# o1-labs/proof-systems

Hardware: AMD Instinct MI355X
Metric: MSM Mscalar/s at 2^20 (Vesta) (higher is better)
Workload: dtype u29x9 / u32x8 (255-bit Montgomery integers); 1 GPU; msm_2^20_vesta_srs; points_per_gpu=1048576, points_total=1048576, bases=SRS::<Vesta>::create, scalars=uniform 254-bit, seed 1234+rank, parallelism=point-range x1, world_size_seen=1

## Files before the change

### include/kimchi_hip.h

```cpp
#ifndef KIMCHI_HIP_H
#define KIMCHI_HIP_H

#include <stddef.h>
#include <stdint.h>

#ifdef __cplusplus
extern "C" {
#endif

#define KH_OK 0
#define KH_E_INVALID (-1)
#define KH_E_DEVICE (-2)
#define KH_E_NOTFOUND (-3)
#define KH_E_NOMEM (-4)

#define KH_CURVE_VESTA 0
#define KH_CURVE_PALLAS 1
#define KH_FIELD_FP 0
#define KH_FIELD_FQ 1
#define KH_BASIS_G (-1)

typedef struct kh_srs kh_srs_t;
typedef struct kh_sponge kh_sponge_t;

int kh_device_count(void);
int kh_init(int device_id);
int kh_set_device(int device_id);
int kh_get_device(void);
int kh_private_context_begin(void);
int kh_private_context_end(void);
int kh_private_context_active(void);
int kh_set_phase_timers(int on);
int kh_trim(void);
const char *kh_last_error(void);

int kh_srs_create(int curve, const uint64_t *g_xy , size_t n, kh_srs_t **out);
int kh_msm_set_wide_min_n(size_t n);
int kh_msm_set_sort_staging(unsigned entries, unsigned max_passes);
int kh_srs_set_wide_tables(kh_srs_t *srs, int on);
int kh_srs_has_wide_tables(const kh_srs_t *srs);
void kh_srs_free(kh_srs_t *srs);
size_t kh_srs_size(const kh_srs_t *srs);
int kh_srs_curve(const kh_srs_t *srs);
int kh_srs_device(const kh_srs_t *srs);

int kh_srs_generate(int curve, size_t start, size_t count, uint64_t *out_xy, int threads);
int kh_srs_h(int curve, uint64_t out_xy[8]);
int kh_group_map_to_group(int curve, const uint64_t t[4], uint64_t out_xy[8]);

int kh_srs_create_device(int curve, size_t depth, kh_srs_t **out);
int kh_srs_create_device_range(int curve, size_t start, size_t count, kh_srs_t **out);
int kh_srs_get_g(kh_srs_t *srs, size_t offset, size_t count, uint64_t *out_xy);

int kh_srs_set_lagrange(kh_srs_t *srs, unsigned log2_domain, unsigned chunk,
                        const uint64_t *xy, const uint8_t *inf, size_t n);
int kh_srs_compute_lagrange(kh_srs_t *srs, unsigned log2_domain);
int kh_srs_get_lagrange(kh_srs_t *srs, unsigned log2_domain, unsigned chunk,
                        uint64_t *out_xy, uint8_t *out_inf);
int kh_srs_lagrange_chunks(const kh_srs_t *srs, unsigned log2_domain);

int kh_msm(kh_srs_t *srs, int basis, unsigned chunk, size_t offset,
           const uint64_t *scalars, size_t n, int scalars_are_montgomery,
           uint64_t out_xy[8], uint8_t *out_is_inf);

int kh_msm_batch(kh_srs_t *srs, int basis, unsigned chunk, size_t offset,
                 const uint64_t *scalars, size_t n, size_t k, int scalars_are_montgomery,
                 uint64_t *out_xy , uint8_t *out_is_inf );

int kh_msm_points(int curve, const uint64_t *xy , const uint8_t *inf ,
                  const uint64_t *scalars, size_t n, int scalars_are_montgomery,
                  uint64_t out_xy[8], uint8_t *out_is_inf);

int kh_msm_points_batch(int curve, const uint64_t *xy, const uint8_t *inf, const uint64_t *scalars,
                        size_t n, size_t k, int scalars_are_montgomery,
                        uint64_t *out_xy , uint8_t *out_is_inf );

int kh_points_sum(int curve, const uint64_t *xy, const uint8_t *inf, size_t n, uint64_t out_xy[8], uint8_t *out_is_inf);
int kh_points_add(int curve, const uint64_t *a_xy, const uint8_t *a_inf, const uint64_t *b_xy, const uint8_t *b_inf, size_t n,
                  uint64_t *out_xy , uint8_t *out_is_inf );

int kh_msm_sharded(kh_srs_t *const *shards, size_t R, const uint64_t *scalars, size_t n, int scalars_are_montgomery,
                   uint64_t out_xy[8], uint8_t *out_is_inf);
int kh_msm_sharded_dev(kh_srs_t *const *shards, size_t R, const uint64_t *const *scalars_dev, const size_t *counts,
                       int scalars_are_montgomery, uint64_t out_xy[8], uint8_t *out_is_inf);

int kh_ipa_fold_scalars(int field, const uint64_t *lo, const uint64_t *hi, const uint64_t u[4], size_t n, uint64_t *out);
int kh_inner_product(int field, const uint64_t *a, const uint64_t *b, size_t n, uint64_t out[4]);
int kh_ipa_fold_points(int curve, const uint64_t *g_lo_xy, const uint64_t *g_hi_xy, const uint64_t u[4], size_t n,
                       uint64_t *out_xy, uint8_t *out_inf);
int kh_ipa_fold_points_endo(int curve, const uint64_t *g_lo_xy, const uint64_t *g_hi_xy, const uint64_t chal[2], size_t n,
                            uint64_t *out_xy, uint8_t *out_inf);
int kh_endos(int curve, uint64_t endo_q[4], uint64_t endo_r[4]);
int kh_scalar_challenge_to_field(int curve, const uint64_t chal[2], uint64_t out[4]);
// ... 450 lines not shown
```

### proof_systems_amd/csrc/api_internal.hpp

```cpp
#pragma once
#include <atomic>
#include <map>
#include <memory>

#include "common.hpp"
#include "host_ec.hpp"
#include "msm.hpp"

namespace kh {
struct LagrangeChunk { DevBuf pts; DevBuf inf; bool has_inf = false; size_t n = 0; int precomp_c = 0; };
}

namespace kh {
struct IpaWorkspace {
    int index = 0;
    bool live = false;
    std::thread::id owner;
    DevBuf a[2], b[2], coef[2], sc, partial, sg;
    hipEvent_t ev = nullptr;
    DevBuf rb_tab, rb_B, rb_part, rb_lists, rb_scratch;
    hipStream_t rb_stream = nullptr;
    hipEvent_t rb_go = nullptr, rb_snap = nullptr, rb_done = nullptr;
    uint32_t* rb_fail = nullptr;
    ~IpaWorkspace() {
        if (ev) (void)hipEventDestroy(ev);
        if (rb_go) (void)hipEventDestroy(rb_go);
        if (rb_snap) (void)hipEventDestroy(rb_snap);
        if (rb_done) (void)hipEventDestroy(rb_done);
        if (rb_stream) { (void)hipStreamSynchronize(rb_stream); (void)hipStreamDestroy(rb_stream); }
        if (rb_fail) (void)hipHostFree(rb_fail);
    }
};
}

struct kh_srs {
    int curve = 0;
    int device = -1;
    size_t n = 0;
    kh::DevBuf g;
    size_t g_stride = 0;
    int g_precomp_c = 0;
    kh::DevBuf g_wide; int g_wide_c = 0;
    std::shared_ptr<std::atomic<int>> jobs = std::make_shared<std::atomic<int>>(0);
    std::mutex wide_mu;
    std::unique_ptr<kh::IpaWorkspace> ipa_ws[KH_IPA_OPENINGS];
    uint64_t h[8];
    std::vector<khost::xyzz> h_table;
    std::vector<uint64_t> h_multiples;
    bool h_in_tables = false;
    std::mutex h_mu;
    std::mutex map_mu;
    std::mutex ipa_mu; std::condition_variable ipa_cv;
    std::map<unsigned, std::vector<std::unique_ptr<kh::LagrangeChunk>>> lagrange;
};
#define KH_ON_DEVICE_OF(srs) kh::DeviceScope dev_scope_((srs) ? (srs)->device : -1)

namespace kh {
int resolve_basis(kh_srs_t* srs, int basis, unsigned chunk, MsmBasis& out);
void xyzz_to_affine_batch(const khost::Crv& crv, const std::vector<khost::xyzz>& acc, uint64_t* out_xy, uint8_t* out_inf);
hipStream_t thread_copy_stream();
hipEvent_t thread_upload_event();
int acquire_slot(std::unique_lock<std::mutex>* lk, Context& C, bool side_first = false);
const char* slot_error(int si);
int wait_then_finish(std::unique_lock<std::mutex>& lk, Context& C, MsmSlot& S, uint64_t* out_xy, uint8_t* out_inf);
double last_wait_us();
void xfer_trim(int d);
struct PoolBlock {
    void* p = nullptr;
    ~PoolBlock() { if (p) (void)kh_dev_free(p); }
    template <class T> T* as() const { return (T*)p; }
};
struct WitnessPlace {
    const uint32_t* rows;
    size_t row0, row_stride;
    uint64_t* witness;
    size_t col_stride;
    __host__ __device__ size_t start_row(size_t i) const { return rows ? (size_t)rows[i] : row0 + i * row_stride; }
    __host__ __device__ size_t offset(size_t r, size_t c) const { return 4 * (c * col_stride + r); }
    __host__ __device__ uint64_t* cell(size_t r, size_t c) const { return witness + offset(r, c); }
};
static constexpr int WAVE_BLOCK = 64;
static constexpr size_t WAVE_BLOCK_MAX_N = (size_t)1 << 36;
inline dim3 blocks_of(size_t n, size_t per) { return dim3((unsigned)((n + per - 1) / per)); }
int poseidon_permute(Context& C, int field, uint64_t* states_dev, size_t n);
int poseidon_hash(Context& C, int field, const uint64_t* msgs_dev, size_t msg_len, size_t n, const uint64_t* init, uint64_t* digests_dev);
int poseidon_gate_rows(Context& C, int field, const uint64_t* states_dev, size_t n, const WitnessPlace& at, uint64_t* out_states_dev);
void poseidon_set_split_max_n(size_t n);
int complete_add_rows(Context& C, int field, const uint64_t* p1_dev, const uint64_t* p2_dev, size_t n, const WitnessPlace& at, uint64_t* out_dev);
int endomul_scalar_rows(Context& C, int field, const uint64_t* chals_dev, unsigned num_bits, size_t n, const WitnessPlace& at, const uint64_t* endo_scalar,
                        uint64_t* out_dev);
size_t chain_slice(bool is_endo, unsigned num_bits, size_t n);
size_t chain_scratch_bytes(bool is_endo, unsigned num_bits, size_t n);
int chain_rows(Context& C, int field, bool is_endo, const uint64_t* endo, const uint64_t* base_dev, const uint64_t* acc0_dev, const uint64_t* scalars_dev,
               unsigned num_bits, size_t n, const WitnessPlace& at, uint64_t* out_acc_dev, uint64_t* out_n_dev, uint32_t* flags_dev, unsigned bit,
// ... 100 lines not shown
```

### proof_systems_amd/csrc/common.hpp

```cpp
#pragma once
#include <hip/hip_runtime.h>
#include <stdarg.h>
#include <stdint.h>
#include <stdio.h>
#include <atomic>
#include <chrono>
#include <condition_variable>
#include <initializer_list>
#include <map>
#include <memory>
#include <mutex>
#include <set>
#include <string>
#include <thread>
#include <vector>

#include "../../include/kimchi_hip.h"
#include "msm_plan.hpp"

namespace kh {

void set_error(const char* fmt, ...);

#define KH_HIP(expr)                                                                         \
// ... 17 lines not shown
    void* p = nullptr;
    size_t cap = 0;
    DevBuf() = default;
    DevBuf(const DevBuf&) = delete;
    DevBuf& operator=(const DevBuf&) = delete;
    DevBuf(DevBuf&& o) noexcept : p(o.p), cap(o.cap) { o.p = nullptr; o.cap = 0; }
    DevBuf& operator=(DevBuf&& o) noexcept { if (this != &o) { release(); p = o.p; cap = o.cap; o.p = nullptr; o.cap = 0; } return *this; }
    ~DevBuf() { release(); }
    int reserve(size_t bytes) {
        if (bytes <= cap) return KH_OK;
        if (p) { hipError_t e = hipFree(p); (void)e; p = nullptr; cap = 0; }
        size_t want = bytes + bytes / 8;
        hipError_t e = hipMalloc(&p, want);
        if (e != hipSuccess) { set_error("hipMalloc(%zu) failed: %s", want, hipGetErrorString(e)); p = nullptr; return KH_E_NOMEM; }
        cap = want;
        return KH_OK;
    }
    void release() { if (p) { hipError_t e = hipFree(p); (void)e; } p = nullptr; cap = 0; }
    template <class T> T* as() const { return (T*)p; }
};

struct PhaseTimer {
    static constexpr int MAXP = 24;
    hipEvent_t k0 = nullptr, k1 = nullptr;
    const char* kname = nullptr;
    hipEvent_t ev[MAXP + 1];
    const char* names[MAXP];
    int n = 0;
    bool created = false;
    bool enabled = false;
    int init() {
        if (created) return KH_OK;
        for (int i = 0; i <= MAXP; i++) KH_HIP(hipEventCreate(&ev[i]));
        KH_HIP(hipEventCreate(&k0)); KH_HIP(hipEventCreate(&k1));
        created = true;
        return KH_OK;
    }
    void begin(hipStream_t s) { n = 0; kname = nullptr; if (enabled && created) (void)hipEventRecord(ev[0], s); }
    void mark(const char* name, hipStream_t s) {
        if (!enabled || !created || n >= MAXP) return;
        names[n] = name; n++;
        (void)hipEventRecord(ev[n], s);
    }
};

struct MsmBasis {
    const void* pts = nullptr;
    const uint8_t* inf = nullptr;
    size_t n = 0;
    int precomp_c = 0;
    size_t stride = 0;
    size_t batch_stride = 0;
    const void* wide_pts = nullptr;
    int wide_c = 0;
    bool glv = false;
};

struct MsmJob {
    MsmBasis basis;
    size_t offset = 0;
    const uint64_t* scalars = nullptr;
    size_t n = 0, k = 0;
    int mont = 0, curve = 0;
    MsmPlan plan;
    bool done_by_flag = false;
    bool spread_rerun = false;
};

struct MsmSlot {
    hipStream_t stream = nullptr;
    PhaseTimer timer;
    DevBuf ws_scalars, ws_digits, ws_hist, ws_cnt, ws_off, ws_ntask, ws_toff, ws_entries, ws_partial,
        ws_buckets, ws_seg, ws_out, ws_scan_tmp, ws_biglist, ws_points, ws_order, ws_chunks, ws_handed, ws_sync, ws_mid,
        ws_b29, ws_a1, ws_l2, ws_a2, ws_xlist;
    void* pinned = nullptr; size_t pinned_cap = 0;
    hipEvent_t done = nullptr;
    bool busy = false;
    std::thread::id owner;
    uint64_t ticket = 0;
    MsmJob job;
    std::shared_ptr<std::atomic<int>> handle_jobs;
    volatile uint32_t* host_abort = nullptr;
    volatile uint32_t* spread_abort = nullptr;
    bool flag_unavailable = false;
    bool pinned_coherent = false;
    volatile uint32_t* done_flag = nullptr;
    DevBuf ws_done;
    uint32_t done_expect = 0;
};
static constexpr int MSM_SLOTS = 4;

struct Context {
    std::mutex mu;
    std::condition_variable cv;
    int sync_inflight = 0;
    std::multiset<std::thread::id> blocked_owners;
    int device = -1;
    bool ready = false;
    hipStream_t stream = nullptr;
    bool main_dirty = false;
    hipEvent_t order_ev = nullptr;
    int num_cus = 256;
    size_t lds_per_cu = (size_t)160 << 10, lds_per_block = (size_t)64 << 10;
    bool fused_disabled = false;
    PhaseTimer timer;
    std::vector<std::pair<const char*, float>> last;
    MsmSlot slot[MSM_SLOTS];
// ... 45 lines not shown
```

### proof_systems_amd/csrc/msm.hip

```cpp
#include <hip/hip_ext.h>
#include <math.h>
#include "common.hpp"
#include "env.hpp"
#include "block_sum.cuh"
#include "coop.cuh"
#include "field29.cuh"
#include "host_ec.hpp"
#include "msm.hpp"
#include "msm_plan.hpp"
#include <condition_variable>
#include <functional>
#include <memory>
#include <thread>

namespace kh {

#define KH_HIGH_PRIO() __builtin_amdgcn_s_setprio(3)

class HostHelper {
    std::thread th_; std::mutex m_; std::condition_variable cv_, done_cv_;
    std::function<void()> job_; bool has_job_ = false, busy_ = false, stop_ = false;
    void loop() {
        std::unique_lock<std::mutex> lk(m_);
        for (;;) {
// ... 231 lines not shown
    }
    __syncthreads();
    size_t q; int Sq, sigma; geom_ids(g, s, w, j, q, Sq, sigma);
    u32* out = H + (q * Sq + sigma) * g.nb;
    for (u32 b = threadIdx.x; b < g.nb; b += blockDim.x) out[b] = h[b];
}
__global__ void k_key_totals(u32* __restrict__ H, u32 nb, int Sq, size_t nkeys, u32* __restrict__ cnt) {
    KH_HIGH_PRIO();
    size_t key = (size_t)blockIdx.x * blockDim.x + threadIdx.x;
    if (key >= nkeys) { if (key == nkeys) cnt[key] = 0; return; }
    size_t q = key / nb; u32 b = (u32)(key % nb);
    u32* p = H + q * Sq * nb + b;
    u32 run = 0;
    for (int s = 0; s < Sq; s++) { u32 v = p[(size_t)s * nb]; p[(size_t)s * nb] = run; run += v; }
    cnt[key] = run;
}
__global__ void k_scatter(const int32_t* __restrict__ digits, SortGeom g, const u32* __restrict__ H,
                          const u32* __restrict__ off, u32* __restrict__ entries) {
    KH_HIGH_PRIO();
    extern __shared__ u32 pos[];
    int s = blockIdx.x, w = blockIdx.y, j = blockIdx.z;
    size_t q; int Sq, sigma; geom_ids(g, s, w, j, q, Sq, sigma);
    const u32* hin = H + (q * Sq + sigma) * g.nb;
    const u32* o = off + q * g.nb;
    for (u32 b = threadIdx.x; b < g.nb; b += blockDim.x) pos[b] = o[b] + hin[b];
    __syncthreads();
    size_t lo = g.n * (size_t)s / g.S, hi = g.n * (size_t)(s + 1) / g.S;
    const int32_t* d = digits + ((size_t)j * g.W + w) * g.n;
    u32 pbase = (u32)(g.pt_offset + (g.precomp ? (size_t)w * g.pt_stride : 0) + (size_t)j * g.pt_batch);
    for (size_t i = lo + threadIdx.x; i < hi; i += blockDim.x) {
        int32_t v = d[i];
        if (v) {
            u32 b = (u32)(v < 0 ? -v : v) - 1u;
            u32 slot = atomicAdd(&pos[b], 1u);
            entries[slot] = (pbase + (u32)i) | (v < 0 ? 0x80000000u : 0u);
        }
    }
}
__device__ __forceinline__ u32 lds_inc_agg(u32* ctr, u32 key, bool active) {
    const u64 act = __ballot(active);
    if (!act) return 0;
    const int leader = __ffsll((long long)act) - 1;
    const u32 k0 = __shfl(key, leader, 64);
    if (__ballot(active && key == k0) == act) {
        const int lane = (int)(threadIdx.x & 63u);
        u32 b = 0;
        if (lane == leader) b = atomicAdd(&ctr[k0], (u32)__popcll(act));
        b = __shfl(b, leader, 64);
        return b + (u32)__popcll(act & ((1ull << lane) - 1ull));
    }
    return active ? atomicAdd(&ctr[key], 1u) : 0u;
}
__global__ void __launch_bounds__(PART_T)
k_part_hist(const int32_t* __restrict__ digits, u32 tot_e, u32 nblk, u32 shift, u32* __restrict__ PH) {
    KH_HIGH_PRIO();
    __shared__ u32 cnt[PART_P];
    const u32 blk = blockIdx.x, j = blockIdx.y, tid = threadIdx.x;
    if (tid < PART_P) cnt[tid] = 0;
    __syncthreads();
    const u32 e_lo = (u32)((u64)tot_e * blk / nblk), e_hi = (u32)((u64)tot_e * (blk + 1) / nblk);
    const int32_t* d = digits + (size_t)j * tot_e;
    for (u32 e0 = e_lo + tid; e0 < e_hi; e0 += 8 * PART_T) {
        int32_t v[8];
#pragma unroll
        for (int u = 0; u < 8; u++) { const u32 e = e0 + u * PART_T; v[u] = d[e < e_hi ? e : e_hi - 1]; if (e >= e_hi) v[u] = 0; }
#pragma unroll
        for (int u = 0; u < 8; u++) (void)lds_inc_agg(cnt, (((u32)(v[u] < 0 ? -v[u] : v[u]) - 1u) >> shift) & (PART_P - 1u), v[u] != 0);
    }
    __syncthreads();
    if (tid < PART_P) PH[((size_t)j * PART_P + tid) * nblk + blk] = cnt[tid];
    if (blk == 0 && j == 0 && tid == 0) PH[(size_t)gridDim.y * PART_P * nblk] = 0;
}
__global__ void __launch_bounds__(PART_T)
k_part_scatter(const int32_t* __restrict__ digits, u32 tot_e, u32 n, u32 nblk, const u32* __restrict__ PO, u32* __restrict__ mid) {
    KH_HIGH_PRIO();
    __shared__ u32 cur[PART_P];
    const u32 blk = blockIdx.x, j = blockIdx.y, tid = threadIdx.x;
    if (tid < PART_P) cur[tid] = PO[((size_t)j * PART_P + tid) * nblk + blk];
    __syncthreads();
    const u32 e_lo = (u32)((u64)tot_e * blk / nblk), e_hi = (u32)((u64)tot_e * (blk + 1) / nblk);
    const int32_t* d = digits + (size_t)j * tot_e;
    u32 w = (e_lo + tid) / n, i = (e_lo + tid) - w * n;
    for (u32 e0 = e_lo + tid; e0 < e_hi; e0 += 8 * PART_T) {
        int32_t v[8];
#pragma unroll
        for (int u = 0; u < 8; u++) { const u32 e = e0 + u * PART_T; v[u] = d[e < e_hi ? e : e_hi - 1]; if (e >= e_hi) v[u] = 0; }
#pragma unroll
        for (int u = 0; u < 8; u++) {
            const u32 b = (u32)(v[u] < 0 ? -v[u] : v[u]) - 1u;
            const u32 pos = lds_inc_agg(cur, b >> PART_LOW, v[u] != 0);
            if (v[u]) mid[pos] = ((b & ((1u << PART_LOW) - 1u)) << 25) | (v[u] < 0 ? 1u << 24 : 0u) | (w << 20) | i;
            i += PART_T;
            while (i >= n) { i -= n; w++; }
        }
    }
}
__global__ void __launch_bounds__(PART_T)
k_part_sort(const u32* __restrict__ mid, const u32* __restrict__ PO, u32 nblk, u32 nb, size_t pt_stride, size_t pt_offset, size_t pt_batch,
            u32 last_group, u32* __restrict__ off, u32* __restrict__ entries) {
    KH_HIGH_PRIO();
    __shared__ u32 hist[1u << PART_LOW], cur[1u << PART_LOW];
    const u32 pidx = blockIdx.x, j = blockIdx.y, tid = threadIdx.x;
    const size_t q = (size_t)j * PART_P + pidx;
    const u32 base = PO[q * nblk], end = PO[(q + 1) * nblk];
    if (tid < (1u << PART_LOW)) hist[tid] = 0;
    __syncthreads();
    for (u32 x0 = base + tid; x0 < end; x0 += 8 * PART_T) {
        u32 m[8];
#pragma unroll
        for (int u = 0; u < 8; u++) { const u32 x = x0 + u * PART_T; m[u] = mid[x < end ? x : end - 1]; }
#pragma unroll
        for (int u = 0; u < 8; u++) (void)lds_inc_agg(hist, m[u] >> 25, x0 + u * PART_T < end);
    }
    __syncthreads();
    if (tid < 64) {
        const u32 a = hist[2 * tid], b = hist[2 * tid + 1];
        u32 inc = a + b;
#pragma unroll
        for (int d = 1; d < 64; d <<= 1) { const u32 o = __shfl_up(inc, d, 64); if (tid >= (u32)d) inc += o; }
        const u32 ex = base + inc - (a + b);
// ... 236 lines not shown
    KH_TS(5);
    if (!grid_barrier(sync, 3 * G, abort_dev, abort_host, spin_limit)) return;
    KH_TS(6);
    const u32* o = off + (size_t)j * g.nb + b_lo;
    {
        u32 a[FUSED_C], hh[FUSED_C];
#pragma unroll
        for (int u = 0; u < FUSED_C; u++) { const u32 b = tid + u * FUSED_T, bc = b < g.sub ? b : 0u; a[u] = coh_load(o + bc); hh[u] = coh_load(hout + bc); }
        u32 total2;
        lane_sums(bsums + FUSED_B, G, blk, &base, &total2);
#pragma unroll
        for (int u = 0; u < FUSED_C; u++) { const u32 b = tid + u * FUSED_T; if (b < g.sub) lds[b] = a[u] + hh[u]; }
    }
    run = base + ex2;
#pragma unroll
    for (int i = 0; i < FUSED_KPT; i++) {
        const u32 key = key0 + i;
        if ((u32)i < g.kpt && key <= g.nkeys) toff[key] = run;
        run += nt[i];
    }
    __syncthreads();
    KH_TS(7);
    const u32 pb0 = (u32)(g.pt_offset + (size_t)j * g.pt_batch);
    const u32 e_first = 4 * (q_lo + tid);
    u32 w = e_first / g.n, i = e_first - w * g.n;
#pragma unroll
    for (int t = 0; t < FUSED_V; t++) asm volatile("" : "+v"(dv[t][0]), "+v"(dv[t][1]));
#pragma unroll
    for (int t = 0; t < FUSED_V; t++) {
#pragma unroll
        for (int l = 0; l < 4; l++) {
            const u32 c = (dv[t][l >> 1] >> (16 * (l & 1))) & 0xffffu, b = (c & 0x7fffu) - b_lo;
            if (c != 0xffffu && b < g.sub) {
                u32 ii = i + l, ww = w;
                if (ii >= g.n) { ii -= g.n; ww++; }
                const u32 slot = atomicAdd(&lds[b], 1u);
                entries[slot] = (pb0 + (u32)(ww * g.pt_stride) + ii) | ((c & 0x8000u) << 16);
            }
        }
        i += 4 * FUSED_T;
        while (i >= g.n) { i -= g.n; w++; }
    }
    __syncthreads();
    KH_TS(8);
    if (tid == 0) {
        const u32 out = __hip_atomic_fetch_add(sync + 1, 1u, __ATOMIC_RELAXED, __HIP_MEMORY_SCOPE_AGENT);
        if (out == G - 1) {
            __hip_atomic_store(sync, 0u, __ATOMIC_RELAXED, __HIP_MEMORY_SCOPE_AGENT);
            __hip_atomic_store(sync + 1, 0u, __ATOMIC_RELAXED, __HIP_MEMORY_SCOPE_AGENT);
        }
    }
}
__global__ void __launch_bounds__(PART_T)
k_part2_scatter(const int32_t* __restrict__ digits, u32 tot_e, u32 nblk, u32 low, const u32* __restrict__ PO, u32* __restrict__ mid, u32* __restrict__ xlist, u32* __restrict__ big) {
    KH_HIGH_PRIO();
    __shared__ u32 cur[PART_P];
    const u32 blk = blockIdx.x, j = blockIdx.y, tid = threadIdx.x;
    if (blk == 0 && j == 0 && tid == 0) { xlist[0] = 0; xlist[1] = 0; big[0] = 0; }
    if (tid < PART_P) cur[tid] = PO[((size_t)j * PART_P + tid) * nblk + blk];
    __syncthreads();
    const u32 e_lo = (u32)((u64)tot_e * blk / nblk), e_hi = (u32)((u64)tot_e * (blk + 1) / nblk);
    const int32_t* d = digits + (size_t)j * tot_e;
    for (u32 e0 = e_lo + tid; e0 < e_hi; e0 += 8 * PART_T) {
        int32_t v[8];
#pragma unroll
        for (int u = 0; u < 8; u++) { const u32 e = e0 + u * PART_T; v[u] = d[e < e_hi ? e : e_hi - 1]; if (e >= e_hi) v[u] = 0; }
#pragma unroll
        for (int u = 0; u < 8; u++) {
            const u32 b = (u32)(v[u] < 0 ? -v[u] : v[u]) - 1u;
            const u32 pos = lds_inc_agg(cur, b & (PART_P - 1u), v[u] != 0);
            if (v[u]) mid[pos] = ((b >> 8) << 17) | (v[u] < 0 ? 1u << 16 : 0u) | (e0 + u * PART_T - e_lo);
        }
    }
}
__global__ void __launch_bounds__(PART_T)
k_part2_sort(const u32* __restrict__ mid, const u32* __restrict__ PO, u32 nblk, u32 low, u32 nb, u32 tot_e, u32 n, size_t pt_stride, size_t pt_offset,
             size_t pt_batch, u32 last_group, size_t total_idx, WideTasks ta, u32* __restrict__ off, u32* __restrict__ entries,
             u32* __restrict__ toff, u32* __restrict__ order, u32* __restrict__ ptot, u32* __restrict__ xlist, u32* __restrict__ slist,
             uint8_t* __restrict__ buckets29, u32 og, u32 stage_cap, u32 max_pass, u32* __restrict__ big, u32 bigcap, u32 hot_nt) {
    KH_HIGH_PRIO();
    __shared__ u32 cur[1u << PART2_MAXLOW], pstart[1025], bi0[1024], bw0[1024], lh[MAX_K + 2], sh[PART_T / 64 + 1];
    __shared__ u32 xl_n, pfirst[PART2_MAXPASS], plast[PART2_MAXPASS];
    extern __shared__ u32 stage[];
    u32* const xl_key = stage; u32* const xl_nt = stage + (1u << PART2_MAXLOW); u32* const xl_base = stage + (2u << PART2_MAXLOW);
    const u32 pidx = blockIdx.x, j = blockIdx.y, tid = threadIdx.x;
    const size_t q = (size_t)j * PART_P + pidx;
    const u32 nparts = gridDim.x * gridDim.y;
    const u32 nbl = 1u << low;
    for (u32 i = tid; i <= nblk; i += PART_T) pstart[i] = PO[q * nblk + i];
    for (u32 i = tid; i < nblk; i += PART_T) {
        const u32 est = (u32)((u64)tot_e * i / nblk), w0 = est / n;
        bw0[i] = w0; bi0[i] = est - w0 * n;
    }
    for (u32 i = tid; i < nbl; i += PART_T) cur[i] = 0;
    for (u32 i = tid; i < MAX_K + 2; i += PART_T) lh[i] = 0;
    if (tid == 0) xl_n = 0;
    __syncthreads();
    const u32 base = pstart[0], end = pstart[nblk];
    for (u32 x0 = base + tid; x0 < end; x0 += 8 * PART_T) {
        u32 m[8];
#pragma unroll
        for (int u = 0; u < 8; u++) { const u32 x = x0 + u * PART_T; m[u] = mid[x < end ? x : end - 1]; }
#pragma unroll
        for (int u = 0; u < 8; u++) (void)lds_inc_agg(cur, m[u] >> 17, x0 + u * PART_T < end);
    }
    __syncthreads();
    {
        const u32 i0 = 2 * tid, a = i0 < nbl ? cur[i0] : 0u, b = i0 + 1 < nbl ? cur[i0 + 1] : 0u;
        u32 btot;
        const u32 ex = base + block_scan_1024(a + b, sh, &btot);
        __syncthreads();
        const size_t key0 = (size_t)j * nb + (size_t)pidx * nbl + i0;
        if (i0 < nbl) { off[key0] = ex; cur[i0] = ex; }
        if (i0 + 1 < nbl) { off[key0 + 1] = ex + a; cur[i0 + 1] = ex + a; }
        if (tid == 0 && pidx == PART_P - 1 && j == last_group) off[(size_t)(j + 1) * nb] = end;
        const u32 K = pick_K(PO[total_idx], ta.room, ta.kmin, ta.ktab, ta.nkeys);
        const u32 nta = (a + K - 1) / K, ntb = (b + K - 1) / K;
        const u32 la = nta ? (a + nta - 1) / nta : 0u, lb = ntb ? (b + ntb - 1) / ntb : 0u;
        const u32 tex = block_scan_1024(nta + ntb, sh, &btot);
        if (i0 < nbl) toff[key0] = tex;
        if (i0 + 1 < nbl) toff[key0 + 1] = tex + nta;
        if (tid == 0) ptot[q] = btot;
        if (i0 < nbl) atomicAdd(&lh[la], 1u);
        if (i0 + 1 < nbl) atomicAdd(&lh[lb], 1u);
        if (nta > 1) { const u32 sl = atomicAdd(&xl_n, 1u); xl_key[sl] = (u32)key0; xl_nt[sl] = nta; xl_base[sl] = atomicAdd(&xlist[0], nta - 1u); slist[atomicAdd(&xlist[1], 1u)] = (u32)key0; }
        if (ntb > 1) { const u32 sl = atomicAdd(&xl_n, 1u); xl_key[sl] = (u32)key0 + 1u; xl_nt[sl] = ntb; xl_base[sl] = atomicAdd(&xlist[0], ntb - 1u); slist[atomicAdd(&xlist[1], 1u)] = (u32)key0 + 1u; }
        if (nta > hot_nt) { const u32 sl = atomicAdd(&big[0], 1u); big[2 + sl] = (u32)key0; big[2 + bigcap + sl] = 0u; }
        if (ntb > hot_nt) { const u32 sl = atomicAdd(&big[0], 1u); big[2 + sl] = (u32)key0 + 1u; big[2 + bigcap + sl] = 0u; }
        if (i0 < nbl && a == 0) { uint4* rec = (uint4*)(buckets29 + ((size_t)j * nb + ((size_t)i0 << 8 | pidx)) * B29_BYTES); _Pragma("unroll") for (int t = 0; t < 9; t++) rec[t] = make_uint4(0u, 0u, 0u, 0u); }
        if (i0 + 1 < nbl && b == 0) { uint4* rec = (uint4*)(buckets29 + ((size_t)j * nb + ((size_t)(i0 + 1) << 8 | pidx)) * B29_BYTES); _Pragma("unroll") for (int t = 0; t < 9; t++) rec[t] = make_uint4(0u, 0u, 0u, 0u); }
        __syncthreads();
        const u32 L = MAX_K - (tid <= MAX_K ? tid : MAX_K), hv = tid <= MAX_K ? lh[L] : 0u;
        const u32 above = block_scan_1024(hv, sh, &btot);
        __syncthreads();
        if (tid <= MAX_K) lh[L] = above;
        __syncthreads();
        if (i0 < nbl) { const u32 r = atomicAdd(&lh[la], 1u); order[(size_t)(r / og) * nparts * og + q * og + (r % og)] = (u32)key0; }
        if (i0 + 1 < nbl) { const u32 r = atomicAdd(&lh[lb], 1u); order[(size_t)(r / og) * nparts * og + q * og + (r % og)] = (u32)key0 + 1u; }
        const u32 nx = xl_n;
        for (u32 it = 0; it < nx; it++) {
            const u32 key = xl_key[it], ntx = xl_nt[it], xb = xl_base[it];
            for (u32 jt = 1 + tid; jt < ntx; jt += PART_T) { xlist[2 + 2 * (size_t)(xb + jt - 1)] = key; xlist[3 + 2 * (size_t)(xb + jt - 1)] = jt; }
        }
    }
    __syncthreads();
    const u32 pb0 = (u32)(pt_offset + (size_t)j * pt_batch);
    const u32 lane = tid & 63u, wv = tid >> 6;
    const u32 S_eff = stage_cap > 2048u ? stage_cap - 1024u : 0u;
    const u32 npass = S_eff ? (end - base + S_eff - 1u) / S_eff : 0u;
    const bool staged = S_eff != 0u && npass >= 1u && npass <= max_pass;
    uint8_t* const bpass = (uint8_t*)(stage + stage_cap);
    if (staged) {
        if (tid < PART2_MAXPASS) { pfirst[tid] = 0xffffffffu; plast[tid] = 0u; }
        __syncthreads();
        for (u32 b = tid; b < nbl; b += PART_T) {
            const u32 o = cur[b], oe = b + 1 < nbl ? cur[b + 1] : end, pb = (o - base) / S_eff;
            bpass[b] = (uint8_t)pb;
            if (oe > o) { atomicMin(&pfirst[pb], o); atomicMax(&plast[pb], oe); }
        }
        __syncthreads();
    }
    for (u32 pass = 0; pass < (staged ? npass : 1u); pass++) {
        const u32 p0 = staged ? pfirst[pass] : 0u, p1 = staged ? plast[pass] : 0u;
        if (staged && p0 == 0xffffffffu) continue;
        for (u32 blk = wv; blk < nblk; blk += PART_T / 64) {
            const u32 rs = pstart[blk], re = pstart[blk + 1];
            const u32 w0 = bw0[blk], i0 = bi0[blk];
            for (u32 x0 = rs; x0 < re; x0 += 256) {
                u32 m[4];
#pragma unroll
                for (int u = 0; u < 4; u++) { const u32 x = x0 + u * 64 + lane; m[u] = mid[x < re ? x : re - 1]; }
#pragma unroll
                for (int u = 0; u < 4; u++) {
                    if (x0 + u * 64 >= re) break;
                    const u32 bk = m[u] >> 17;
                    const bool live = x0 + u * 64 + lane < re && (!staged || bpass[bk] == pass);
                    const u32 pos = lds_inc_agg(cur, bk, live);
                    if (live) {
                        u32 w = w0, i = i0 + (m[u] & 0xffffu);
                        while (i >= n) { i -= n; w++; }
                        const u32 val = (pb0 + (u32)(w * pt_stride) + i) | ((m[u] & (1u << 16)) << 15);
                        if (staged && pos - p0 < stage_cap) stage[pos - p0] = val;
                        else entries[pos] = val;
                    }
                }
            }
        }
        if (staged) {
            __syncthreads();
            const u32 cnt = p1 - p0 < stage_cap ? p1 - p0 : stage_cap;
            for (u32 k = tid; k < cnt; k += PART_T) entries[p0 + k] = stage[k];
            __syncthreads();
        }
    }
}
__global__ void __launch_bounds__(256)
k_wide_fixup(u32* __restrict__ toff, const u32* __restrict__ ptot, u32 nparts, u32 low, u32 nkeys, u32* __restrict__ handed, u32* __restrict__ big) {
    KH_HIGH_PRIO();
    __shared__ u32 sh[4];
    const u32 key = blockIdx.x * 256 + threadIdx.x, q = (blockIdx.x * 256) >> low;
    u32 v = 0;
    for (u32 t = threadIdx.x; t < q && t < nparts; t += 256) v += ptot[t];
#pragma unroll
    for (int d = 32; d >= 1; d >>= 1) v += __shfl_xor(v, d, 64);
    if ((threadIdx.x & 63u) == 0) sh[threadIdx.x >> 6] = v;
    __syncthreads();
    const u32 bs = sh[0] + sh[1] + sh[2] + sh[3];
    if (key < nkeys) toff[key] += bs;
    else if (key == nkeys) toff[key] = bs;
    if (key == 0) handed[0] = 0;
}
template <class BF>
__global__ void __launch_bounds__(256) __attribute__((amdgpu_num_vgpr(112), amdgpu_waves_per_eu(4, 4)))
k_accumulate29(const u32* __restrict__ entries, const u32* __restrict__ off, const u32* __restrict__ toff,
               const u32* __restrict__ roff, const u32* __restrict__ order,
               size_t nkeys, const uint8_t* __restrict__ pts, uint8_t* __restrict__ partial, u32* __restrict__ handed, const u32* __restrict__ abort_dev, u32 hi_prio) {
    if (hi_prio) __builtin_amdgcn_s_setprio(2);
    if (sort_gave_up(abort_dev)) return;
    const size_t t0 = (size_t)blockIdx.x * blockDim.x + threadIdx.x;
    u32 NT = roff[nkeys];
    if (t0 >= NT) return;
    size_t lo = 0, hi = nkeys;
    while (hi - lo > 1) {
        size_t mid = (lo + hi) >> 1;
        if (roff[mid] <= (u32)t0) lo = mid; else hi = mid;
    }
    size_t key = order ? order[lo] : lo;
    u32 jt = (u32)t0 - roff[lo];
    const size_t t = (size_t)toff[key] + jt;
    u32 o0 = off[key], cnt = off[key + 1] - o0, nt = toff[key + 1] - toff[key];
    u32 start = o0 + (u32)(((u64)jt * cnt) / nt);
    u32 end = o0 + (u32)(((u64)(jt + 1) * cnt) / nt);
    u32 e = entries[start];
    Aff<BF> p = Aff<BF>::load(pts + (size_t)(e & 0x7fffffffu) * 64);
    if (e >> 31) p.y = neg<BF>(p.y);
    typedef typename C29<BF>::T K29;
    Acc29<BF> acc;
    bool ok = true;
    u32 k = start + 1;
    if (k < end) {
        const Fe29<BF> x1 = pack29<BF, 5>(p.x), y1 = pack29<BF, 5>(p.y);
        e = entries[k];
        p = Aff<BF>::load(pts + (size_t)(e & 0x7fffffffu) * 64);
        if (e >> 31) p.y = neg<BF>(p.y);
        ok = aadd29<BF>(acc, x1, y1, pack29<BF, 5>(p.x), pack29<BF, 5>(p.y));
        k = ok ? k + 1 : end;
    } else {
        acc.x = to29<BF>(p.x); acc.y = to29<BF>(p.y);
#pragma unroll
        for (int i = 0; i < 9; i++) { acc.zz.v[i] = K29::one(i); acc.zzz.v[i] = K29::one(i); }
    }
    for (; k < end; k++) {
        e = entries[k];
        p = Aff<BF>::load(pts + (size_t)(e & 0x7fffffffu) * 64);
        if (e >> 31) p.y = neg<BF>(p.y);
        ok = madd29<BF, false>(acc, pack29<BF, 5>(p.x), pack29<BF, 5>(p.y));
        if (!ok) break;
    }
    Xyzz<BF> r;
    if (__builtin_expect(!ok, 0)) {
        e = entries[start];
        p = Aff<BF>::load(pts + (size_t)(e & 0x7fffffffu) * 64);
        if (e >> 31) p.y = neg<BF>(p.y);
        r = Xyzz<BF>::from_affine(p);
        for (u32 k = start + 1; k < end; k++) {
            e = entries[k];
            p = Aff<BF>::load(pts + (size_t)(e & 0x7fffffffu) * 64);
            r = madd<BF>(r, p, (e >> 31) != 0);
        }
    } else {
        r.x = from29<BF>(acc.x); r.y = from29<BF>(acc.y); r.zz = from29<BF>(acc.zz); r.zzz = from29<BF>(acc.zzz);
    }
    r.store(partial + t * 128);
}
__device__ __forceinline__ u32 wide_true_bucket(u32 key, u32 low) {
    const u32 nbl = 1u << low, grp = key >> (low + 8), kk = key & ((nbl << 8) - 1u);
    return (grp << (low + 8)) | ((kk & (nbl - 1u)) << 8) | (kk >> low);
}
template <class BF>
__device__ __forceinline__ bool wide_task29(u32 key, u32 jt, const u32* __restrict__ entries, const u32* __restrict__ off, const u32* __restrict__ toff,
                                            const uint8_t* __restrict__ pts, uint8_t* __restrict__ partial, uint8_t* __restrict__ buckets29, u32 low, u32* __restrict__ handed) {
    const u32 o0 = off[key], cnt = off[key + 1] - o0;
    if (cnt == 0) return true;
    const u32 t0 = toff[key], nt = toff[key + 1] - t0;
    u32 start = o0, end = o0 + cnt;
    if (nt != 1) { start = o0 + (u32)(((u64)jt * cnt) / nt); end = o0 + (u32)(((u64)(jt + 1) * cnt) / nt); }
    u32 e = entries[start];
    Aff<BF> p = Aff<BF>::load(pts + (size_t)(e & 0x7fffffffu) * 64);
    if (e >> 31) p.y = neg<BF>(p.y);
    typedef typename C29<BF>::T K29;
    Acc29<BF> acc;
    bool ok = true;
    u32 k = start + 1;
    if (k < end) {
        const Fe29<BF> x1 = pack29<BF, 5>(p.x), y1 = pack29<BF, 5>(p.y);
        e = entries[k];
        p = Aff<BF>::load(pts + (size_t)(e & 0x7fffffffu) * 64);
        if (e >> 31) p.y = neg<BF>(p.y);
        ok = aadd29<BF>(acc, x1, y1, pack29<BF, 5>(p.x), pack29<BF, 5>(p.y));
        k = ok ? k + 1 : end;
    } else {
        acc.x = to29<BF>(p.x); acc.y = to29<BF>(p.y);
#pragma unroll
        for (int i = 0; i < 9; i++) { acc.zz.v[i] = K29::one(i); acc.zzz.v[i] = K29::one(i); }
    }
    for (; k < end; k++) {
        e = entries[k];
        p = Aff<BF>::load(pts + (size_t)(e & 0x7fffffffu) * 64);
        if (e >> 31) p.y = neg<BF>(p.y);
        ok = madd29<BF, false>(acc, pack29<BF, 5>(p.x), pack29<BF, 5>(p.y));
        if (!ok) break;
    }
    if (!ok) { if (!handed) return false; const u32 slot = atomicAdd(&handed[0], 1u); handed[2 + 2 * slot] = key; handed[3 + 2 * slot] = jt; return true; }
    if (nt == 1) { store_b29<BF>(buckets29 + (size_t)wide_true_bucket(key, low) * B29_BYTES, acc); return true; }
    Xyzz<BF> r;
    r.x = from29<BF>(acc.x); r.y = from29<BF>(acc.y); r.zz = from29<BF>(acc.zz); r.zzz = from29<BF>(acc.zzz);
    r.store(partial + (size_t)(t0 + jt) * 128);
    return true;
}
template <class BF>
__device__ __forceinline__ void wide_task_exact(u32 key, u32 jt, const u32* __restrict__ entries, const u32* __restrict__ off, const u32* __restrict__ toff,
                                                const uint8_t* __restrict__ pts, uint8_t* __restrict__ partial, uint8_t* __restrict__ buckets29, u32 low) {
    const u32 o0 = off[key], cnt = off[key + 1] - o0, t0 = toff[key], nt = toff[key + 1] - t0;
    if (cnt == 0) return;
    const u32 start = o0 + (u32)(((u64)jt * cnt) / nt), end = o0 + (u32)(((u64)(jt + 1) * cnt) / nt);
    u32 e = entries[start];
    Aff<BF> p = Aff<BF>::load(pts + (size_t)(e & 0x7fffffffu) * 64);
    if (e >> 31) p.y = neg<BF>(p.y);
    Xyzz<BF> acc = Xyzz<BF>::from_affine(p);
    for (u32 k = start + 1; k < end; k++) {
        e = entries[k];
        p = Aff<BF>::load(pts + (size_t)(e & 0x7fffffffu) * 64);
        acc = madd<BF>(acc, p, (e >> 31) != 0);
    }
    if (nt == 1) {
        uint8_t* const rec = buckets29 + (size_t)wide_true_bucket(key, low) * B29_BYTES;
        if (acc.is_identity()) store_b29_identity<BF>(rec); else store_b29<BF>(rec, xyzz_to29<BF>(acc));
    } else acc.store(partial + (size_t)(t0 + jt) * 128);
}
template <class BF>
__global__ void __launch_bounds__(256) __attribute__((amdgpu_num_vgpr(112), amdgpu_waves_per_eu(4, 4)))
k_acc_wide29(const u32* __restrict__ entries, const u32* __restrict__ off, const u32* __restrict__ toff, const u32* __restrict__ order, u32 nkeys,
             const uint8_t* __restrict__ pts, uint8_t* __restrict__ partial, uint8_t* __restrict__ buckets29, u32 low, u32* __restrict__ handed) {
    const u32 g = blockIdx.x * blockDim.x + threadIdx.x;
    if (g < nkeys) (void)wide_task29<BF>(order[g], 0u, entries, off, toff, pts, partial, buckets29, low, handed);
}
template <class BF>
__global__ void __launch_bounds__(256)
k_acc_wide_rest(const u32* __restrict__ entries, const u32* __restrict__ off, const u32* __restrict__ toff, const u32* __restrict__ xlist, const u32* __restrict__ handed,
                const uint8_t* __restrict__ pts, uint8_t* __restrict__ partial, uint8_t* __restrict__ buckets29, u32 low) {
    KH_HIGH_PRIO();
    const u32 nx = xlist[0], nh = handed[0];
    for (u32 it = blockIdx.x * blockDim.x + threadIdx.x; it < nx; it += gridDim.x * blockDim.x) {
        const u32 key = xlist[2 + 2 * it], jt = xlist[3 + 2 * it];
        if (!wide_task29<BF>(key, jt, entries, off, toff, pts, partial, buckets29, low, nullptr))
            wide_task_exact<BF>(key, jt, entries, off, toff, pts, partial, buckets29, low);
    }
    for (u32 it = blockIdx.x * blockDim.x + threadIdx.x; it < nh; it += gridDim.x * blockDim.x)
        wide_task_exact<BF>(handed[2 + 2 * it], handed[3 + 2 * it], entries, off, toff, pts, partial, buckets29, low);
}
__device__ __forceinline__ size_t hot_key(u32 slot) { return 2 + (size_t)slot; }
__device__ __forceinline__ size_t hot_cbase(size_t cap, u32 slot) { return 2 + cap + slot; }
__device__ __forceinline__ size_t item_key(size_t cap, u32 it) { return 2 + 2 * cap + it; }
__device__ __forceinline__ size_t item_chunk(size_t cap, u32 it) { return 2 + 3 * cap + it; }
__device__ __forceinline__ void list_hot_bucket(u32* __restrict__ big, size_t cap, u32 key, u32 nt) {
    u32 nch = (nt + CHUNK - 1) / CHUNK;
    u32 slot = atomicAdd(&big[0], 1u);
    u32 cbase = atomicAdd(&big[1], nch);
    big[hot_key(slot)] = key; big[hot_cbase(cap, slot)] = cbase;
    for (u32 j = 0; j < nch; j++) { big[item_key(cap, cbase + j)] = key; big[item_chunk(cap, cbase + j)] = j; }
}
template <class BF>
__global__ void __launch_bounds__(256)
k_bucket_sum(const u32* __restrict__ toff, size_t nkeys, const uint8_t* __restrict__ partial,
             uint8_t* __restrict__ buckets, u32* __restrict__ big, size_t cap, u32 SMALL_NT, const u32* __restrict__ abort_dev) {
    KH_HIGH_PRIO();
    if (sort_gave_up(abort_dev)) return;
    size_t key = (size_t)blockIdx.x * blockDim.x + threadIdx.x;
    if (key >= nkeys) return;
    u32 t0 = toff[key], nt = toff[key + 1] - t0;
    Xyzz<BF> acc = Xyzz<BF>::identity();
    if (nt > SMALL_NT) {
        list_hot_bucket(big, cap, (u32)key, nt);
    } else if (nt > 0) {
        acc = Xyzz<BF>::load(partial + (size_t)t0 * 128);
        for (u32 k = 1; k < nt; k++) acc = add<BF>(acc, Xyzz<BF>::load(partial + (size_t)(t0 + k) * 128));
    }
    acc.store(buckets + key * 128);
}
template <class BF>
__global__ void __launch_bounds__(64)
k_bucket_chunk(const u32* __restrict__ toff, const uint8_t* __restrict__ partial, const u32* __restrict__ big, size_t cap,
               uint8_t* __restrict__ chunk_out, const u32* __restrict__ abort_dev) {
    KH_HIGH_PRIO();
    if (sort_gave_up(abort_dev)) return;
    u32 nitems = big[1];
    const u32 quad = threadIdx.x >> 2;
    for (u32 it = blockIdx.x; it < nitems; it += gridDim.x) {
        u32 key = big[item_key(cap, it)], j = big[item_chunk(cap, it)];
        u32 t0 = toff[key], nt = toff[key + 1] - t0;
        u32 lo = j * CHUNK, hi = lo + CHUNK < nt ? lo + CHUNK : nt;
        const Fe<BF> acc = quad_chunk_sum<BF>(partial + (size_t)t0 * 128, lo + quad, hi, 16);
        if (threadIdx.x < 4) quad_store<BF>(chunk_out + (size_t)it * 128, acc);
    }
}
template <class BF>
__global__ void __launch_bounds__(256)
k_bucket_big(const u32* __restrict__ toff, const uint8_t* __restrict__ chunk_out, uint8_t* __restrict__ buckets,
             const u32* __restrict__ big, size_t cap, const u32* __restrict__ abort_dev) {
    KH_HIGH_PRIO();
    if (sort_gave_up(abort_dev)) return;
    __shared__ u32 sh[4 * 32];
// ... 169 lines not shown
__global__ void __launch_bounds__(128)
k_marginal_fin_q(const uint8_t* __restrict__ marg, MargGeom g, uint8_t* __restrict__ out, u32* __restrict__ done_ws, u32* __restrict__ done_flag) {
    KH_HIGH_PRIO();
    __shared__ u32 sh[32 * 32];
    const u32 j = blockIdx.x; const size_t q = blockIdx.y;
    const u32 v = threadIdx.x >> 2, role = threadIdx.x & 3u, f = g.wd[j];
    Fe<BF> r = Fe<BF>::zero();
    if (v < (1u << f)) r = quad_load<BF>(marg + ((q * 3 + j) * 32 + v) * 128);
    auto put = [&](const Fe<BF>& x) {
#pragma unroll
        for (int k = 0; k < 8; k++) sh[(v * 4 + role) * 8 + k] = x.v[k];
    };
    auto get = [&](u32 from) {
        Fe<BF> o = Fe<BF>::zero();
        if (from < 32) {
#pragma unroll
            for (int k = 0; k < 8; k++) o.v[k] = sh[(from * 4 + role) * 8 + k];
        }
        return o;
    };
    for (u32 d = 1; d < 32; d <<= 1) {
        put(r); __syncthreads();
        const Fe<BF> o = get(v + d);
        __syncthreads();
        r = quad_add<BF>(r, o);
    }
    if (v == 0 && j != 0) r = Fe<BF>::zero();
    for (u32 d = 16; d >= 1; d >>= 1) {
        put(r); __syncthreads();
        const Fe<BF> o = v < d ? get(v + d) : Fe<BF>::zero();
        __syncthreads();
        r = quad_add<BF>(r, o);
    }
    if (threadIdx.x < 4) quad_store<BF>(out + (q * 3 + j) * 128, r);
    if (done_ws) {
        __threadfence_system();
        __syncthreads();
        if (threadIdx.x == 0) {
            const u32 blocks = gridDim.x * gridDim.y;
            if (__hip_atomic_fetch_add(done_ws, 1u, __ATOMIC_ACQ_REL, __HIP_MEMORY_SCOPE_AGENT) == blocks - 1) {
                __hip_atomic_store(done_ws, 0u, __ATOMIC_RELAXED, __HIP_MEMORY_SCOPE_AGENT);
                const u32 e = done_ws[1] + 1;
                done_ws[1] = e;
                __threadfence_system();
                __hip_atomic_store(done_flag, e, __ATOMIC_RELEASE, __HIP_MEMORY_SCOPE_SYSTEM);
            }
        }
    }
}

template <class BF>
__global__ void __launch_bounds__(256)
k_bucket_sum_wide(const u32* __restrict__ toff, const u32* __restrict__ xlist, const u32* __restrict__ slist, const uint8_t* __restrict__ partial,
                  uint8_t* __restrict__ buckets29, u32 low, u32 SMALL_NT, u32* __restrict__ big, u32 cap, uint8_t* __restrict__ chunk_out) {
    KH_HIGH_PRIO();
    __shared__ __attribute__((aligned(16))) uint8_t total[4 * 128];
    const u32 count = xlist[1], nhot = big[0];
    for (u32 it = blockIdx.x * blockDim.x + threadIdx.x; it < count; it += gridDim.x * blockDim.x) {
        const u32 key = slist[it];
        const u32 t0 = toff[key], nt = toff[key + 1] - t0;
        if (nt > SMALL_NT) continue;
        Xyzz<BF> acc = Xyzz<BF>::load(partial + (size_t)t0 * 128);
        for (u32 k = 1; k < nt; k++) acc = add<BF>(acc, Xyzz<BF>::load(partial + (size_t)(t0 + k) * 128));
        uint8_t* const rec = buckets29 + (size_t)wide_true_bucket(key, low) * B29_BYTES;
        if (acc.is_identity()) store_b29_identity<BF>(rec); else store_b29<BF>(rec, xyzz_to29<BF>(acc));
    }
    if (nhot == 0) return;
    const u32 wave = threadIdx.x >> 6, lane = threadIdx.x & 63u, quad = lane >> 2;
    const u32 gw = blockIdx.x * (blockDim.x >> 6) + wave, GW = gridDim.x * (blockDim.x >> 6);
    u32 cbase = 0;
    for (u32 h = 0; h < nhot; h++) {
        const u32 key = big[2 + h];
        const u32 t0 = toff[key], nt = toff[key + 1] - t0, nch = (nt + CHUNK - 1) / CHUNK;
        for (u32 c = (gw + GW - cbase % GW) % GW; c < nch; c += GW) {
            const u32 lo = c * CHUNK, hi = lo + CHUNK < nt ? lo + CHUNK : nt;
            const Fe<BF> acc = quad_chunk_sum<BF>(partial + (size_t)t0 * 128, lo + quad, hi, 16);
            if (lane < 4) quad_store<BF>(chunk_out + (size_t)(cbase + c) * 128, acc);
            __threadfence();
            u32 arrived = 0;
            if (lane == 0) arrived = __hip_atomic_fetch_add(&big[2 + cap + h], 1u, __ATOMIC_ACQ_REL, __HIP_MEMORY_SCOPE_AGENT) + 1u;
            arrived = __shfl(arrived, 0, 64);
            if (arrived == nch) {
                __threadfence();
                const Fe<BF> o = quad_chunk_sum<BF>(chunk_out + (size_t)cbase * 128, quad, nch, 16);
                if (lane < 4) quad_store<BF>(total + 128 * wave, o);
                __builtin_amdgcn_wave_barrier();
                if (lane == 0) {
                    const Xyzz<BF> v = Xyzz<BF>::load(total + 128 * wave);
                    uint8_t* const rec = buckets29 + (size_t)wide_true_bucket(key, low) * B29_BYTES;
                    if (v.is_identity()) store_b29_identity<BF>(rec); else store_b29<BF>(rec, xyzz_to29<BF>(v));
                }
                __builtin_amdgcn_wave_barrier();
            }
        }
        cbase += nch;
    }
}
template <class F>
__device__ __forceinline__ bool is_marker29(const Acc29<F>& a) { return a.zz.v[0] == 0xffffffffu; }
template <class BF>
__device__ __forceinline__ void wide_sum29(const uint8_t* __restrict__ in, size_t stride, u32 n, uint8_t* __restrict__ o) {
    Acc29<BF> acc;
    bool have = false, ok = true;
#pragma unroll 1
    for (u32 i = 0; i < n; i++) {
        const Acc29<BF> b = load_b29<BF>(in + (size_t)i * stride);
        if (is_identity29<BF>(b)) continue;
        if (!have) { acc = b; have = true; ok = !is_marker29<BF>(b); }
        else ok = !is_marker29<BF>(b) && add29<BF>(acc, b);
        if (!ok) break;
    }
    if (!ok) { acc.zz.v[0] = 0xffffffffu; store_b29<BF>(o, acc); return; }
    if (have) store_b29<BF>(o, acc); else store_b29_identity<BF>(o);
}
template <class BF>
__global__ void __launch_bounds__(256)
k_wide_a1(const uint8_t* __restrict__ buckets29, WideGeom g, u32 ngroups, uint8_t* __restrict__ out29) {
    KH_HIGH_PRIO();
    const u32 per = g.nb >> g.rlog, items = 2u * per;
    const u32 gid = blockIdx.x * blockDim.x + threadIdx.x;
    if (gid >= items * ngroups) return;
    const u32 q = gid / items, u = gid - q * items;
    u32 out = u;
    if (u >= per) { const u32 v = u - per, b = v & ((1u << g.lo) - 1u), sc = v >> g.lo; out = per + b * ((1u << g.hi) >> g.rlog) + sc; }
    u32 t0, ts;
    wide_a1_item(g, out, t0, ts);
    wide_sum29<BF>(buckets29 + ((size_t)q * g.nb + t0) * B29_BYTES, (size_t)ts * B29_BYTES, 1u << g.rlog, out29 + ((size_t)q * items + out) * B29_BYTES);
}
template <class BF>
__global__ void __launch_bounds__(256)
k_wide_l2(const uint8_t* __restrict__ in29, u32 flog, u32 nrec, uint8_t* __restrict__ out29) {
    KH_HIGH_PRIO();
    const u32 gid = blockIdx.x * blockDim.x + threadIdx.x;
    if (gid >= nrec) return;
    wide_sum29<BF>(in29 + ((size_t)gid << flog) * B29_BYTES, B29_BYTES, 1u << flog, out29 + (size_t)gid * B29_BYTES);
}
template <class BF>
__device__ __attribute__((noinline)) Xyzz<BF> wide_chunk_exact(const uint8_t* __restrict__ buckets29g, WideGeom g, u32 out) {
    u32 t0, ts;
    wide_a1_item(g, out, t0, ts);
    Xyzz<BF> acc = Xyzz<BF>::identity();
    const u32 r = 1u << g.rlog;
    for (u32 i = 0; i < r; i++) {
        const Acc29<BF> b = load_b29<BF>(buckets29g + ((size_t)t0 + (size_t)i * ts) * B29_BYTES);
        if (!is_identity29<BF>(b)) acc = add<BF>(acc, xyzz_from29<BF>(b));
    }
    return acc;
}
template <class BF>
__device__ __attribute__((noinline)) Xyzz<BF> wide_run_exact(const uint8_t* __restrict__ chunks29g, const uint8_t* __restrict__ buckets29g, WideGeom g, u32 run) {
    Xyzz<BF> acc = Xyzz<BF>::identity();
    const u32 f = 1u << g.flog, c0 = run << g.flog;
    for (u32 i = 0; i < f; i++) {
        const Acc29<BF> b = load_b29<BF>(chunks29g + (size_t)(c0 + i) * B29_BYTES);
        if (is_marker29<BF>(b)) acc = add<BF>(acc, wide_chunk_exact<BF>(buckets29g, g, c0 + i));
        else if (!is_identity29<BF>(b)) acc = add<BF>(acc, xyzz_from29<BF>(b));
    }
    return acc;
}
template <class BF>
__global__ void __launch_bounds__(64)
k_wide_a2(const uint8_t* __restrict__ runs29, const uint8_t* __restrict__ chunks29, const uint8_t* __restrict__ buckets29, WideGeom g, uint8_t* __restrict__ outw) {
    KH_HIGH_PRIO();
    __shared__ u32 stage[32][16];
    const u32 q = blockIdx.y, lane = threadIdx.x, role = lane & 3u, quad = lane >> 2;
    const u32 per = g.nb >> g.rlog, per2 = per >> g.flog;
    const u32 r0 = blockIdx.x * 16u, plane = r0 >= per2 ? 1u : 0u;
    const u32 s = ((1u << (plane ? g.hi : g.lo)) >> g.rlog) >> g.flog;
    uint8_t* const og = outw + ((size_t)q * 2 + plane) * (1u << g.lo) * 128;
    if (lane < 16) {
        const u32 run = r0 + lane;
        const Acc29<BF> b = load_b29<BF>(runs29 + ((size_t)q * 2 * per2 + run) * B29_BYTES);
        Xyzz<BF> a = Xyzz<BF>::identity();
        if (__builtin_expect(is_marker29<BF>(b), 0)) a = wide_run_exact<BF>(chunks29 + (size_t)q * 2 * per * B29_BYTES, buckets29 + (size_t)q * g.nb * B29_BYTES, g, run);
        else if (!is_identity29<BF>(b)) a = xyzz_from29<BF>(b);
#pragma unroll
        for (int k = 0; k < 8; k++) { stage[k][lane] = a.x.v[k]; stage[8 + k][lane] = a.y.v[k]; stage[16 + k][lane] = a.zz.v[k]; stage[24 + k][lane] = a.zzz.v[k]; }
    }
    __syncthreads();
    Fe<BF> acc;
#pragma unroll
    for (int k = 0; k < 8; k++) acc.v[k] = stage[role * 8 + k][quad];
    for (u32 d = s >> 1; d >= 1; d >>= 1) acc = quad_add<BF>(acc, quad_shfl_down<BF>(acc, (int)d));
    if ((quad & (s - 1u)) == 0u) {
        const u32 m = (r0 - plane * per2 + quad) / s;
        if (plane || m) quad_store<BF>(og + (size_t)(m - (plane ? 0u : 1u)) * 128, acc);
    }
    if (plane == 0 && lane < 4)
        for (u32 p = (1u << g.hi) - 1u + blockIdx.x; p < (1u << g.lo); p += per2 / 16u) quad_store<BF>(og + (size_t)p * 128, Fe<BF>::zero());
}

template <class BF>
__global__ void __launch_bounds__(256)
k_precompute(uint8_t* __restrict__ tables, const uint8_t* __restrict__ inf, size_t n, int c, int W, uint8_t* __restrict__ scratch) {
    size_t i = (size_t)blockIdx.x * blockDim.x + threadIdx.x;
    if (i >= n) return;
    if (inf && inf[i]) {
        for (int w = 1; w < W; w++) { Fe<BF> z = Fe<BF>::zero(); z.store(tables + ((size_t)w * n + i) * 64); z.store(tables + ((size_t)w * n + i) * 64 + 32); }
        return;
    }
    Xyzz<BF> P = Xyzz<BF>::from_affine(Aff<BF>::load(tables + i * 64));
    Fe<BF> prod = Fe<BF>::one();
    for (int w = 1; w < W; w++) {
        for (int k = 0; k < c; k++) P = dbl<BF>(P);
        P.store(scratch + ((size_t)(w - 1) * n + i) * 128);
        prod = mul<BF>(prod, P.zzz);
        prod.store(tables + ((size_t)w * n + i) * 64);
    }
    Fe<BF> iv = inv<BF>(prod);
    for (int w = W - 1; w >= 1; w--) {
        Xyzz<BF> Q = Xyzz<BF>::load(scratch + ((size_t)(w - 1) * n + i) * 128);
        Fe<BF> izzz = iv;
        if (w > 1) izzz = mul<BF>(iv, Fe<BF>::load(tables + ((size_t)(w - 1) * n + i) * 64));
        iv = mul<BF>(iv, Q.zzz);
        Fe<BF> izz = sqr<BF>(mul<BF>(izzz, Q.zz));
        Fe<BF> x = mul<BF>(Q.x, izz), y = mul<BF>(Q.y, izzz);
        x.store(tables + ((size_t)w * n + i) * 64);
        y.store(tables + ((size_t)w * n + i) * 64 + 32);
    }
}

struct VestaCfg { typedef FqParams Base; typedef FpParams Scalar; };
struct PallasCfg { typedef FpParams Base; typedef FqParams Scalar; };

static std::atomic<size_t>& wide_min_n_cell() {
    static std::atomic<size_t> v{(size_t)env_int("KH_WIDE_MIN_N", 1 << 19)};
    return v;
}
static std::atomic<u32>& sort_staging_cell(int i) {
    static std::atomic<u32> v[2] = {{(u32)env_int("KH_PART2_STAGE", 28672)}, {(u32)env_int("KH_PART2_MAXPASS", 2)}};
    return v[i];
}
void msm_set_sort_staging(unsigned entries, unsigned max_passes) { sort_staging_cell(0).store(entries); sort_staging_cell(1).store(max_passes); }
size_t msm_wide_min_n() { const size_t v = wide_min_n_cell().load(); return v ? v : ~(size_t)0; }
void msm_set_wide_min_n(size_t n) { wide_min_n_cell().store(n); }
static int msm_reserve(Context& Ctx, MsmSlot& C, const MsmPlan& P, bool& flag_on) {
    hipStream_t s = C.stream;
    const size_t nkeys = P.nkeys, M = P.M, max_tasks = P.max_tasks, ngroups = P.ngroups;
    int rc;
    if ((rc = C.ws_digits.reserve(M * sizeof(int32_t)))) return rc;
    if ((rc = C.ws_hist.reserve(nkeys * P.Sq * sizeof(u32)))) return rc;
    if ((rc = C.ws_cnt.reserve((nkeys + 2) * sizeof(u32)))) return rc;
    if ((rc = C.ws_off.reserve((nkeys + 2) * sizeof(u32)))) return rc;
    if ((rc = C.ws_ntask.reserve((nkeys + 2) * sizeof(u32)))) return rc;
    if ((rc = C.ws_toff.reserve((nkeys + 2) * sizeof(u32)))) return rc;
    if ((rc = C.ws_entries.reserve((M + 1) * sizeof(u32)))) return rc;
    if ((rc = C.ws_partial.reserve(max_tasks * 128))) return rc;
    if ((rc = C.ws_handed.reserve((max_tasks + 2) * sizeof(u32)))) return rc;
    if ((rc = C.ws_buckets.reserve(nkeys * 128))) return rc;
    if ((rc = C.ws_biglist.reserve((2 + 4 * P.bigcap) * sizeof(u32)))) return rc;
    if ((rc = C.ws_chunks.reserve(P.bigcap * 128))) return rc;
    if ((rc = C.ws_order.reserve((2 * (MAX_K + 1) + 3 * (nkeys + 2)) * sizeof(u32)))) return rc;
    if (P.wide) {
        if ((rc = C.ws_xlist.reserve((3 * max_tasks + 8) * sizeof(u32)))) return rc;
        if ((rc = C.ws_handed.reserve((2 * max_tasks + 4) * sizeof(u32)))) return rc;
        if ((rc = C.ws_b29.reserve(nkeys * B29_BYTES))) return rc;
        if ((rc = C.ws_a1.reserve(ngroups * 2 * (size_t)(P.nb >> P.wg.rlog) * B29_BYTES))) return rc;
        if ((rc = C.ws_l2.reserve(ngroups * 2 * (size_t)(P.nb >> (P.wg.rlog + P.wg.flog)) * B29_BYTES))) return rc;
        if ((rc = C.ws_a2.reserve(ngroups * 2 * ((size_t)1 << P.wg.lo) * 128))) return rc;
    }
    if ((rc = C.ws_seg.reserve(std::max(ngroups * (size_t)(P.nseg + P.nblk1), P.nout * (size_t)32) * 128))) return rc;
    if ((rc = C.ws_out.reserve(P.nout * 128))) return rc;
    if (C.pinned_cap < P.nout * 128) {
        if (C.pinned) (void)hipHostFree(C.pinned);
        C.pinned = nullptr; C.pinned_cap = 0;
        C.pinned_coherent = hipHostMalloc(&C.pinned, P.nout * 128 + 4096, hipHostMallocCoherent | hipHostMallocMapped) == hipSuccess;
        if (!C.pinned_coherent) { (void)hipGetLastError(); C.pinned = nullptr; KH_HIP(hipHostMalloc(&C.pinned, P.nout * 128 + 4096, hipHostMallocDefault)); }
        C.pinned_cap = P.nout * 128 + 4096;
    }
    if (Ctx.once("msm_attr")) {
        KH_HIP(hipFuncSetAttribute((const void*)k_hist, hipFuncAttributeMaxDynamicSharedMemorySize, 131072));
        KH_HIP(hipFuncSetAttribute((const void*)k_scatter, hipFuncAttributeMaxDynamicSharedMemorySize, 131072));
        KH_HIP(hipFuncSetAttribute((const void*)k_sort_fused, hipFuncAttributeMaxDynamicSharedMemorySize, 131072));
    }
    if (P.sort == SORT_PARTITIONED) {
        if ((rc = C.ws_hist.reserve((P.part_size + 1) * sizeof(u32)))) return rc;
        if ((rc = C.ws_cnt.reserve((P.part_size + 1) * sizeof(u32)))) return rc;
        if ((rc = C.ws_mid.reserve(M * sizeof(u32)))) return rc;
    }
    if (P.sort == SORT_FUSED) {
        if ((rc = C.ws_hist.reserve((size_t)P.fg.k * P.fg.bpg * P.nb * sizeof(u32)))) return rc;
        if (!C.ws_sync.p) {
            if ((rc = C.ws_sync.reserve((2 + 2 * FUSED_B + 32 + 2) * sizeof(u32)))) return rc;
            KH_HIP(hipMemsetAsync(C.ws_sync.p, 0, (2 + 2 * FUSED_B + 32 + 2) * sizeof(u32), s));
        }
        if (!C.host_abort) {
            void* hp = nullptr;
            KH_HIP(hipHostMalloc(&hp, 64, hipHostMallocCoherent | hipHostMallocMapped));
// ... 59 lines not shown
        return;
    }
    if (T.kind == TAIL_MARGINALS_H)
        hipLaunchKernelGGL((k_marginals_h<BF>), dim3(32, 3, ngroups), dim3(256), 0, s, buckets, T.mg, seg);
    else if (T.kind == TAIL_MARGINALS_Q)
        hipLaunchKernelGGL((k_marginals_q<BF>), dim3(32, 3, ngroups), dim3(256), 0, s, buckets, T.mg, seg);
    else
        hipLaunchKernelGGL((k_marginals<BF>), dim3(32, 3, ngroups), dim3(64), 0, s, buckets, T.mg, seg);
    if (T.fin_quad)
        hipLaunchKernelGGL((k_marginal_fin_q<BF>), dim3(3, ngroups), dim3(128), 0, s, seg, T.mg, out, done_ws, done_flag);
    else
        hipLaunchKernelGGL((k_marginal_fin<BF>), dim3(3, ngroups), dim3(64), 0, s, seg, T.mg, out);
}

struct SortViews { u32 *len_hist, *cursor, *order, *rnt, *roff, *slist; };
static SortViews sort_views(const MsmSlot& C, const MsmPlan& P) {
    SortViews v;
    v.len_hist = C.ws_order.as<u32>();
    v.cursor = v.len_hist + (MAX_K + 1);
    v.order = v.cursor + (MAX_K + 1);
    v.rnt = v.order + (P.nkeys + 2);
    v.roff = v.rnt + (P.nkeys + 2);
    v.slist = C.ws_xlist.as<u32>() + P.slist_off;
    return v;
}
template <class CFG>
static int msm_launch_sort(MsmSlot& C, const uint8_t* inf, const u64* scalars_dev, int mont, const MsmShape& sh, const MsmPlan& P, u32*& order, u32*& roff) {
    typedef typename CFG::Scalar SF;
    hipStream_t s = C.stream;
    const size_t n = sh.n, k = sh.k, nkeys = P.nkeys;
    const bool wide = P.wide, fused = P.sort == SORT_FUSED;
    int rc;
    if (P.glv)
    hipLaunchKernelGGL((k_digits_glv<SF>), dim3((unsigned)((n + 255) / 256), (unsigned)k), dim3(256), 0, s,
                       scalars_dev, inf, sh.offset, sh.batch_stride, n, mont, P.c, P.W, C.ws_digits.as<int32_t>());
    else
    hipLaunchKernelGGL((k_digits<SF>), dim3((unsigned)((n + 255) / 256), (unsigned)k), dim3(256), 0, s,
                       scalars_dev, inf, sh.offset, sh.batch_stride, n, mont, P.c, P.W, C.ws_digits.as<int32_t>(), (size_t)0, n);
    C.timer.mark("digits", s);
    const SortViews v = sort_views(C, P);
    u32 *const len_hist = v.len_hist, *const cursor = v.cursor, *const rnt = v.rnt, *const slist = v.slist;
    order = v.order; roff = v.roff;
    if (fused) {
        static const unsigned long long fused_spin_ticks = 100ull * (unsigned long long)env_int("KH_FUSED_SPIN_US", 20000);
        order = nullptr; roff = C.ws_toff.as<u32>();
        u32* sy = C.ws_sync.as<u32>();
        hipLaunchKernelGGL(k_sort_fused, dim3(P.fg.bpg * P.fg.k * P.fg.split), dim3(FUSED_T), (size_t)P.fg.sub * sizeof(u32), s, C.ws_digits.as<int32_t>(), P.fg,
                           C.ws_hist.as<u32>(), C.ws_off.as<u32>(), C.ws_toff.as<u32>(), C.ws_entries.as<u32>(), C.ws_handed.as<u32>(),
                           C.ws_biglist.as<u32>(), sy, sy + 2, C.host_abort, fused_spin_ticks);
        C.timer.mark("sort", s);
    } else if (P.sort == SORT_PARTITIONED) {
        const u32 tot_e = (u32)P.tot_e, part_nblk = P.part_nblk, part_low = P.part_low;
        const dim3 pgrid(part_nblk, (unsigned)k);
        hipLaunchKernelGGL(k_part_hist, pgrid, dim3(PART_T), 0, s, C.ws_digits.as<int32_t>(), tot_e, part_nblk, wide ? 0u : part_low, C.ws_hist.as<u32>());
        C.timer.mark("histogram", s);
        if ((rc = exclusive_scan_u32(C.ws_hist.as<u32>(), C.ws_cnt.as<u32>(), P.part_size + 1, C.ws_scan_tmp, s))) return rc;
        C.timer.mark("scan", s);
        if (wide) {
            hipLaunchKernelGGL(k_part2_scatter, pgrid, dim3(PART_T), 0, s, C.ws_digits.as<int32_t>(), tot_e, part_nblk, part_low, C.ws_cnt.as<u32>(), C.ws_mid.as<u32>(), C.ws_xlist.as<u32>(), C.ws_biglist.as<u32>());
            const WideTasks wt{P.room, P.kmin, (u32)nkeys, P.ktab};
            u32* const ptot = C.ws_ntask.as<u32>();
            hipLaunchKernelGGL(k_part2_sort, dim3(PART_P, (unsigned)k), dim3(PART_T), P.part2_lds, s, C.ws_mid.as<u32>(), C.ws_cnt.as<u32>(), part_nblk, part_low, P.nb, tot_e, (u32)n,
                               P.g.pt_stride, sh.offset, sh.batch_stride, (u32)(k - 1), P.part_size, wt, C.ws_off.as<u32>(), C.ws_entries.as<u32>(),
                               C.ws_toff.as<u32>(), order, ptot, C.ws_xlist.as<u32>(), slist, C.ws_b29.as<uint8_t>(), wide_og, P.stage_now, P.part2_maxpass, C.ws_biglist.as<u32>(), (u32)P.bigcap, WIDE_HOT_NT);
            hipLaunchKernelGGL(k_wide_fixup, dim3((unsigned)(nkeys / 256 + 1)), dim3(256), 0, s, C.ws_toff.as<u32>(), ptot, (u32)(k * PART_P), part_low, (u32)nkeys,
                               C.ws_handed.as<u32>(), C.ws_biglist.as<u32>());
        } else {
        hipLaunchKernelGGL(k_part_scatter, pgrid, dim3(PART_T), 0, s, C.ws_digits.as<int32_t>(), tot_e, (u32)n, part_nblk, C.ws_cnt.as<u32>(), C.ws_mid.as<u32>());
        hipLaunchKernelGGL(k_part_sort, dim3(PART_P, (unsigned)k), dim3(PART_T), 0, s, C.ws_mid.as<u32>(), C.ws_cnt.as<u32>(), part_nblk, P.nb,
                           P.g.pt_stride, sh.offset, sh.batch_stride, (u32)(k - 1), C.ws_off.as<u32>(), C.ws_entries.as<u32>());
        }
        C.timer.mark("scatter", s);
    } else {
        size_t lds = (size_t)P.nb * sizeof(u32);
        dim3 sgrid((unsigned)P.S, (unsigned)P.W, (unsigned)k);
        hipLaunchKernelGGL(k_hist, sgrid, dim3(1024), lds, s, C.ws_digits.as<int32_t>(), P.g, C.ws_hist.as<u32>());
        hipLaunchKernelGGL(k_key_totals, dim3((unsigned)((nkeys + 1 + 255) / 256)), dim3(256), 0, s,
                           C.ws_hist.as<u32>(), P.nb, P.Sq, nkeys, C.ws_cnt.as<u32>());
        C.timer.mark("histogram", s);
        if ((rc = exclusive_scan_u32(C.ws_cnt.as<u32>(), C.ws_off.as<u32>(), nkeys + 1, C.ws_scan_tmp, s))) return rc;
        C.timer.mark("scan", s);
        hipLaunchKernelGGL(k_scatter, sgrid, dim3(1024), lds, s, C.ws_digits.as<int32_t>(), P.g, C.ws_hist.as<u32>(),
                           C.ws_off.as<u32>(), C.ws_entries.as<u32>());
        C.timer.mark("scatter", s);
    }
    if (!fused && !wide) {
        hipLaunchKernelGGL(k_task_reset, dim3(1), dim3(320), 0, s, len_hist, C.ws_biglist.as<u32>());
        hipLaunchKernelGGL(k_ntask, dim3((unsigned)((nkeys + 1 + 1023) / 1024)), dim3(1024), 0, s, C.ws_off.as<u32>(), nkeys, P.room, P.kmin, P.ktab, C.ws_ntask.as<u32>(), len_hist, C.ws_handed.as<u32>());
        if ((rc = exclusive_scan_u32(C.ws_ntask.as<u32>(), C.ws_toff.as<u32>(), nkeys + 1, C.ws_scan_tmp, s))) return rc;
        if (P.M >= ((size_t)1 << 22)) {
            hipLaunchKernelGGL(k_len_starts, dim3(1), dim3(320), 0, s, len_hist, cursor);
            hipLaunchKernelGGL(k_len_rank, dim3((unsigned)((nkeys + 1 + 1023) / 1024)), dim3(1024), 0, s, C.ws_off.as<u32>(), C.ws_ntask.as<u32>(), nkeys, cursor, order, rnt);
            if ((rc = exclusive_scan_u32(rnt, roff, nkeys + 1, C.ws_scan_tmp, s))) return rc;
        } else {
            order = nullptr; roff = C.ws_toff.as<u32>();
        }
        C.timer.mark("tasks", s);
    }
    return KH_OK;
}

template <class CFG>
static int msm_launch(MsmSlot& C, const MsmBasis& basis, const u64* scalars_dev, int mont, const MsmShape& sh, const MsmPlan& P, bool flag_on) {
    typedef typename CFG::Base BF;
    hipStream_t s = C.stream;
    const size_t nkeys = P.nkeys, ngroups = P.ngroups;
    const bool wide = P.wide, fused = P.sort == SORT_FUSED;
    const void* const tab_pts = wide ? basis.wide_pts : basis.pts;
    int rc;
    C.timer.begin(s);
    u32 *order = nullptr, *roff = nullptr;
    if ((rc = msm_launch_sort<CFG>(C, basis.inf, scalars_dev, mont, sh, P, order, roff))) return rc;
    u32* const slist = sort_views(C, P).slist;
    const u32* abort_dev = fused ? C.ws_sync.as<u32>() + 2 + 2 * FUSED_B + 32 : nullptr;
    uint8_t* const b29 = wide ? C.ws_b29.as<uint8_t>() : nullptr;
    if (wide) {
        launch_timed(C.timer, "k_acc_wide29", k_acc_wide29<BF>, dim3(P.acc_blocks), dim3(256), P.wide_acc_lds, s, C.ws_entries.as<u32>(), C.ws_off.as<u32>(),
                     C.ws_toff.as<u32>(), order, (u32)nkeys, (const uint8_t*)tab_pts, C.ws_partial.as<uint8_t>(), b29, P.part_low, C.ws_handed.as<u32>());
        const unsigned xgrid = P.M / nkeys >= 64 ? 2048u : WIDE_XB;
        hipLaunchKernelGGL((k_acc_wide_rest<BF>), dim3(xgrid), dim3(256), 0, s, C.ws_entries.as<u32>(), C.ws_off.as<u32>(), C.ws_toff.as<u32>(), C.ws_xlist.as<u32>(),
                           C.ws_handed.as<u32>(), (const uint8_t*)tab_pts, C.ws_partial.as<uint8_t>(), b29, P.part_low);
    } else
        launch_timed(C.timer, "k_accumulate29", k_accumulate29<BF>, dim3(P.acc_blocks), dim3(256), 0, s, C.ws_entries.as<u32>(), C.ws_off.as<u32>(),
                     C.ws_toff.as<u32>(), roff, order, nkeys, (const uint8_t*)tab_pts, C.ws_partial.as<uint8_t>(), C.ws_handed.as<u32>(), abort_dev, P.acc_prio);
    C.timer.mark("accumulate", s);
    if (wide)
        hipLaunchKernelGGL((k_bucket_sum_wide<BF>), dim3(256), dim3(256), 0, s, C.ws_toff.as<u32>(), C.ws_xlist.as<u32>(), slist,
                           C.ws_partial.as<uint8_t>(), b29, P.part_low, WIDE_HOT_NT, C.ws_biglist.as<u32>(), (u32)P.bigcap, C.ws_chunks.as<uint8_t>());
    else
        launch_bucket_sums<BF>(s, P.quad_sum, P.quad_sum ? (P.spread ? SPREAD_MAX_NT : 16u) : (nkeys <= 16384 ? 4u : 16u), P.spread ? (u32*)C.spread_abort : nullptr,
                               C.ws_toff.as<u32>(), nkeys, C.ws_partial.as<uint8_t>(), C.ws_buckets.as<uint8_t>(), C.ws_biglist.as<u32>(), P.bigcap,
                               C.ws_chunks.as<uint8_t>(), abort_dev);
    C.timer.mark("bucket_sum", s);
    u32* const done_ws = flag_on ? C.ws_done.as<u32>() : nullptr; u32* const done_flag = flag_on ? (u32*)C.done_flag : nullptr;
    if (flag_on) C.done_expect++;
    const MargGeom& mg = P.mg;
    if (wide) {
        hipLaunchKernelGGL((k_wide_a1<BF>), dim3((P.wide_items + 255) / 256), dim3(256), 0, s, b29, P.wg, (u32)ngroups, C.ws_a1.as<uint8_t>());
        C.timer.mark("reduce_a1", s);
        hipLaunchKernelGGL((k_wide_l2<BF>), dim3((P.wide_runs + 63) / 64), dim3(64), 0, s, C.ws_a1.as<uint8_t>(), P.wg.flog, P.wide_runs, C.ws_l2.as<uint8_t>());
        hipLaunchKernelGGL((k_wide_a2<BF>), dim3(P.wide_runs / (u32)ngroups / 16u, (unsigned)ngroups), dim3(64), 0, s, C.ws_l2.as<uint8_t>(), C.ws_a1.as<uint8_t>(), b29, P.wg,
                           C.ws_a2.as<uint8_t>());
        hipLaunchKernelGGL((k_marginals_q<BF>), dim3(32, 3, (unsigned)P.tail_groups), dim3(256), 0, s, C.ws_a2.as<uint8_t>(), mg, C.ws_seg.as<uint8_t>());
        hipLaunchKernelGGL((k_marginal_fin_q<BF>), dim3(3, (unsigned)P.tail_groups), dim3(128), 0, s, C.ws_seg.as<uint8_t>(), mg, (uint8_t*)C.pinned, done_ws, done_flag);
    } else {
        NarrowTail T;
        T.kind = !P.planes ? TAIL_SEGMENTS : ((mg.nb >> mg.wd[0]) >= 256 ? TAIL_MARGINALS_H : (P.few_groups ? TAIL_MARGINALS_Q : TAIL_MARGINALS));
        T.fin_quad = P.direct_out; T.mg = mg; T.nb = P.nb; T.m = P.m; T.nseg = P.nseg; T.nblk1 = P.nblk1; T.ngroups = ngroups;
        launch_narrow_tail<BF>(s, T, C.ws_buckets.as<uint8_t>(), C.ws_seg.as<uint8_t>(), P.direct_out ? (uint8_t*)C.pinned : C.ws_out.as<uint8_t>(), done_ws, done_flag);
    }
    C.timer.mark("reduce", s);
    KH_HIP(hipGetLastError());
    if (!P.direct_out) KH_HIP(hipMemcpyAsync(C.pinned, C.ws_out.p, P.nout * 128, hipMemcpyDeviceToHost, s));
    KH_HIP(hipEventRecord(C.done, s));
    return KH_OK;
}

int msm_enqueue(Context& C, MsmSlot& S, int curve, const MsmBasis& basis, size_t offset, const uint64_t* scalars_dev, size_t n, size_t k, int mont,
                int flags) {
    MsmJob job;
    job.basis = basis; job.offset = offset; job.scalars = scalars_dev; job.n = n; job.k = k; job.mont = mont; job.curve = curve;
    if (n == 0 || k == 0) {
        S.busy = true; S.owner = std::this_thread::get_id(); S.ticket = C.next_ticket++;
        S.job = job;
        KH_HIP(hipEventRecord(S.done, S.stream));
        return KH_OK;
    }
    static const bool fused_off = env_flag("KH_NO_FUSED_SORT", false), flag_off = env_flag("KH_NO_DONE_FLAG", false), fin_quad = !env_flag("KH_NO_FIN_QUAD", false);
    MsmShape sh;
    sh.n = n; sh.k = k; sh.offset = offset; sh.flags = flags;
    sh.precomp_c = basis.precomp_c; sh.has_wide = basis.wide_pts != nullptr; sh.wide_c = basis.wide_c; sh.glv = basis.glv;
    sh.stride = basis.stride; sh.basis_n = basis.n; sh.batch_stride = basis.batch_stride;
    sh.num_cus = C.num_cus; sh.lds_per_cu = C.lds_per_cu; sh.lds_per_block = C.lds_per_block;
    sh.wide_min_n = msm_wide_min_n(); sh.stage_entries = sort_staging_cell(0).load(); sh.stage_maxpass = sort_staging_cell(1).load();
    sh.fused_off = fused_off || C.fused_disabled; sh.flag_off = flag_off; sh.fin_quad = fin_quad;
    const char* why = nullptr;
    KH_REQUIRE(msm_plan(sh, job.plan, &why) == 0, "%s (n=%zu k=%zu)", why, n, k);
    bool flag_on = false;
    int rc = msm_reserve(C, S, job.plan, flag_on);
    if (rc) return rc;
    rc = curve == KH_CURVE_VESTA ? msm_launch<VestaCfg>(S, basis, scalars_dev, mont, sh, job.plan, flag_on)
                                 : msm_launch<PallasCfg>(S, basis, scalars_dev, mont, sh, job.plan, flag_on);
    if (rc) return rc;
    job.done_by_flag = job.plan.direct_out && flag_on;
    S.busy = true; S.owner = std::this_thread::get_id(); S.ticket = C.next_ticket++;
    S.job = job;
    return KH_OK;
}

static int msm_rerun(Context& C, MsmSlot& S) {
    const MsmJob j = S.job;
    const uint64_t ticket = S.ticket; const auto owner = S.owner;
    int rc = msm_enqueue(C, S, j.curve, j.basis, j.offset, j.scalars, j.n, j.k, j.mont);
    S.ticket = ticket; S.owner = owner; C.next_ticket--;
    if (rc) { S.busy = false; return rc; }
    KH_HIP(hipEventSynchronize(S.done));
    return KH_OK;
}

int msm_finish(Context& C, MsmSlot& S, uint64_t* out_xy, uint8_t* out_inf, bool flag_seen) {
    if (!(flag_seen && S.job.done_by_flag && S.timer.n == 0)) KH_HIP(hipEventSynchronize(S.done));
    if (S.job.plan.sort == SORT_FUSED && S.host_abort && *S.host_abort) {
        *S.host_abort = 0;
        if (!C.fused_disabled) fprintf(stderr, "libkimchi_hip: k_sort_fused could not get its blocks co-resident (shared GPU?): using the multi-launch sort from now on\n");
        C.fused_disabled = true;
        counter(CNT_FUSED_RETRY)++;
        KH_HIP(hipMemsetAsync(S.ws_sync.p, 0, (2 + 2 * FUSED_B + 32 + 2) * sizeof(u32), S.stream));
        if (int rc = msm_rerun(C, S)) return rc;
    }
    if (S.job.plan.spread && S.spread_abort && *S.spread_abort) {
        *S.spread_abort = 0;
        counter(CNT_SPREAD_RETRY)++;
        if (int rc = msm_rerun(C, S)) return rc;
        S.job.spread_rerun = true;
    }
    S.busy = false;
    static const bool fused_dbg = env_flag("KH_FUSED_DEBUG", false);
    if (fused_dbg && S.ws_sync.p) {
        unsigned long long ts[12]; (void)hipMemcpy(ts, S.ws_sync.as<u32>() + 2 + 2 * FUSED_B, sizeof(ts), hipMemcpyDeviceToHost);
        fprintf(stderr, "k_sort_fused phases (us):"); for (int i = 1; i < 9; i++) fprintf(stderr, " %.1f", (double)(ts[i] - ts[i - 1]) / 100.0);
        fprintf(stderr, " | p3: %.1f %.1f %.1f %.1f\n", (double)(ts[9] - ts[4]) / 100.0, (double)(ts[10] - ts[9]) / 100.0, (double)(ts[11] - ts[10]) / 100.0, (double)(ts[5] - ts[11]) / 100.0);
    }
    collect_timings(C, S.timer);
    const MsmJob& J = S.job;
// ... 13 lines not shown
        if (Pp->wide) {
            for (int g2 = 0; g2 < 2; g2++) {
                const khost::xyzz* r3 = res + (j * 2 + g2) * 3;
                khost::xyzz f = r3[2];
                for (int t = 0; t < (int)Pp->mg.wd[1]; t++) f = crv.dbl(f);
                f = crv.add(f, r3[1]);
                for (int t = 0; t < (int)Pp->mg.wd[0]; t++) f = crv.dbl(f);
                f = crv.add(f, r3[0]);
                if (g2 == 0) { for (int t = 0; t < (int)Pp->wg.lo; t++) f = crv.dbl(f); total = f; }
                else total = crv.add(total, f);
            }
        } else if (Pp->precomp && Pp->planes) {
            total = res[j * 3 + 2];
            for (int t = 0; t < (int)Pp->mg.wd[1]; t++) total = crv.dbl(total);
            total = crv.add(total, res[j * 3 + 1]);
            for (int t = 0; t < (int)Pp->mg.wd[0]; t++) total = crv.dbl(total);
            total = crv.add(total, res[j * 3]);
        } else if (Pp->precomp) total = res[j];
        else {
            total = crv.identity();
            for (int w = Pp->W - 1; w >= 0; w--) {
                for (int t = 0; t < Pp->c; t++) total = crv.dbl(total);
                total = crv.add(total, res[j * Pp->W + w]);
            }
        }
    };
    if ((!P.precomp && J.k >= 2) || (P.planes && J.k >= 16)) {
        const size_t half = J.k / 2, kk = J.k;
        HostHelper& hh = host_helper(&C);
        hh.run([finish_one, half, kk] { for (size_t j = half; j < kk; j++) finish_one(j); });
        for (size_t j = 0; j < half; j++) finish_one(j);
        hh.wait();
    } else {
        for (size_t j = 0; j < J.k; j++) finish_one(j);
    }
    khost::Crv crv(J.curve); const khost::Fld& F = crv.F;
    static thread_local std::vector<khost::fe> pre;
    pre.resize(J.k + 1);
    pre[0] = F.f.one;
    for (size_t j = 0; j < J.k; j++) pre[j + 1] = crv.is_identity(tot[j]) ? pre[j] : F.mul(pre[j], tot[j].zzz);
    khost::fe inv = F.inv(pre[J.k]);
    for (size_t j = J.k; j-- > 0;) {
        if (crv.is_identity(tot[j])) { memset(out_xy + 8 * j, 0, 64); out_inf[j] = 1; continue; }
        const khost::fe izzz = F.mul(inv, pre[j]);
        inv = F.mul(inv, tot[j].zzz);
        const khost::fe izz = F.sqr(F.mul(izzz, tot[j].zz));
        const khost::fe x = F.mul(tot[j].x, izz), y = F.mul(tot[j].y, izzz);
        memcpy(out_xy + 8 * j, &x, 32); memcpy(out_xy + 8 * j + 4, &y, 32);
        out_inf[j] = 0;
    }
    return KH_OK;
}

int msm_precompute(Context& C, int curve, void* tables, const uint8_t* inf, size_t n, int c) {
    const int W = windows_of(c);
    DevBuf& scratch = C.scratch("precompute");
    int rc = scratch.reserve((size_t)(W - 1) * n * 128); if (rc) return rc;
    dim3 grid((unsigned)((n + 255) / 256));
    KH_CURVE_LAUNCH(curve, k_precompute<F>, grid, dim3(256), 0, C.stream, (uint8_t*)tables, inf, n, c, W, scratch.as<uint8_t>());
    KH_HIP(hipStreamSynchronize(C.stream));
    if (scratch.cap > ((size_t)1 << 30)) scratch.release();
    return KH_OK;
}

template <class F>
__global__ void k_debug_field(int op, const u64* a, const u64* b, u64* out, size_t n) {
    size_t i = (size_t)blockIdx.x * blockDim.x + threadIdx.x;
    if (i >= n) return;
    Fe<F> x = Fe<F>::load(a + 4 * i), y = Fe<F>::zero(), r;
    if (b) y = Fe<F>::load(b + 4 * i);
    switch (op) {
        case 0: r = mul<F>(x, y); break;
        case 1: r = add<F>(x, y); break;
        case 2: r = sub<F>(x, y); break;
        case 3: r = to_mont<F>(x); break;
        case 4: r = from_mont<F>(x); break;
        case 5: r = sqr<F>(x); break;
        case 7: r = from29<F>(mul29<F>(to29<F>(x), to29<F>(y))); break;
        case 8: r = from29<F>(sqr29<F>(to29<F>(x))); break;
        case 9: r = unpack29<F>(pack29<F, 0>(x)); break;
        case 10: r = from29<F>(mul29<F>(pack29<F, 5>(x), to29<F>(y))); break;
        default: r = neg<F>(x); break;
    }
    r.store(out + 4 * i);
}
template <class F>
__global__ void k_debug_field29(int op, int spread, const u32* a, const u32* b, const u32* c, u32* out, size_t n) {
    const size_t i = (size_t)blockIdx.x * blockDim.x + threadIdx.x;
    if (i >= n) return;
    typedef typename C29<F>::T K;
    Fe29<F> x, y, z, r;
#pragma unroll
    for (int k = 0; k < 9; k++) { x.v[k] = a[9 * i + k]; y.v[k] = op == 0 ? b[9 * i + k] : 0u; z.v[k] = c[9 * i + k]; }
    if (op == 0) r = spread == 0 ? mulsub29<F, K::s71>(x, y, z) : (spread == 1 ? mulsub29<F, K::s51>(x, y, z) : mulsub29<F, K::s44>(x, y, z));
    else r = spread == 0 ? sqrsub29<F, K::s71>(x, z) : (spread == 1 ? sqrsub29<F, K::s51>(x, z) : sqrsub29<F, K::s44>(x, z));
#pragma unroll
    for (int k = 0; k < 9; k++) out[9 * i + k] = r.v[k];
}
int debug_field29_op(Context& C, int field, int op, int spread, const u32* a, const u32* b, const u32* c, u32* out, size_t n) {
    dim3 grid((unsigned)((n + 255) / 256));
    KH_FIELD_LAUNCH(field, k_debug_field29<F>, grid, dim3(256), 0, C.stream, op, spread, a, b, c, out, n);
    return KH_OK;
}
int debug_field_op(Context& C, int field, int op, const u64* a, const u64* b, u64* out, size_t n) {
    dim3 grid((unsigned)((n + 255) / 256));
    KH_FIELD_LAUNCH(field, k_debug_field<F>, grid, dim3(256), 0, C.stream, op, a, b, out, n);
    return KH_OK;
}
template <class F>
__global__ void k_debug_point(int op, const u64* p, const uint8_t* pinf, const u64* q, const uint8_t* qinf, uint8_t* out, size_t n) {
    size_t i = (size_t)blockIdx.x * blockDim.x + threadIdx.x;
    if (i >= n) return;
// ... 185 lines not shown
```

### proof_systems_amd/csrc/msm.hpp

```cpp
#pragma once
#include "common.hpp"
#include "host_ec.hpp"
#include "gate_batch.hpp"
#include "witness_lookup.hpp"

namespace kh {

int msm_precompute(Context& C, int curve, void* tables, const uint8_t* inf, size_t n, int c);
int rebase_points(hipStream_t s, int curve, const uint64_t* coef, size_t Q, const void* tables, size_t stride, size_t N, void* B, void* part, void* lists,
                  hipEvent_t after_plan = nullptr);
int rebase_tables(hipStream_t s, int curve, const void* part, size_t N, const void* extra_affine_host, size_t extra, int c, void* scratch, void* tables, uint32_t* fail,
                  const uint64_t* glv_beta = nullptr);
int msm_debug_glv_split(hipStream_t s, int field, const uint64_t* scalars_dev, size_t n, uint32_t* out_dev);
const uint32_t* msm_glv_lambda(int scalar_field);
size_t rebase_bucket_bytes(size_t N);
size_t rebase_part_bytes(size_t N);
size_t rebase_list_bytes(size_t Q);
static constexpr int MSM_PRECOMP_C = 16;
static constexpr int MSM_WIDE_C = 20;
void msm_set_wide_min_n(size_t n);
void msm_set_sort_staging(unsigned entries, unsigned max_passes);
size_t msm_wide_min_n();
static constexpr size_t MSM_PRECOMP_MIN_N = 1024;
int msm_enqueue(Context& C, MsmSlot& S, int curve, const MsmBasis& basis, size_t offset, const uint64_t* scalars_dev, size_t n, size_t k, int mont,
                int flags = 0);
int msm_finish(Context& C, MsmSlot& S, uint64_t* out_xy, uint8_t* out_inf, bool flag_seen = false);
int debug_field_op(Context& C, int field, int op, const uint64_t* a, const uint64_t* b, uint64_t* out, size_t n);
int debug_field29_op(Context& C, int field, int op, int spread, const uint32_t* a, const uint32_t* b, const uint32_t* c, uint32_t* out, size_t n);
int debug_point_op(Context& C, int curve, int op, const uint64_t* p, const uint8_t* pinf, const uint64_t* q, const uint8_t* qinf, uint8_t* out, size_t n);
int debug_bucket_tail_sizes(int tail, int fin, unsigned c_or_nb, unsigned m, size_t groups, size_t* in_records, size_t* seg_records, size_t* out_records);
int debug_bucket_tail(Context& C, int curve, int tail, int fin, unsigned c_or_nb, unsigned m, size_t groups, const uint8_t* buckets, uint8_t* seg, uint8_t* out);
size_t debug_bucket_sums_cap(size_t nkeys, size_t ntasks);
int debug_bucket_sums(Context& C, int curve, int kind, size_t nkeys, const uint32_t* toff, const uint8_t* partial, uint8_t* buckets, uint32_t* big, size_t bigcap,
                      uint8_t* chunks);
int debug_msm_sort_plan(Context& C, const kh_msm_sort_args_t& a, MsmShape& sh, MsmPlan& P, kh_msm_sort_echo_t* echo);
int debug_msm_sort_run(Context& C, MsmSlot& S, const kh_msm_sort_args_t& a, const MsmShape& sh, const MsmPlan& P, const kh_msm_sort_echo_t& echo, const kh_msm_sort_out_t& out);

int ntt_build_twiddles(Context& C, int field, unsigned logn, int inverse, uint64_t* tab);
void ntt_trim(Context& C);
int ipa_fold_scalars(Context& C, int field, const uint64_t* lo, const uint64_t* hi, const uint64_t u[4], size_t n, uint64_t* out);
int ipa_inner_product(Context& C, int field, const uint64_t* a, const uint64_t* b, size_t n, uint64_t out[4]);
int ipa_fold_points_endo(Context& C, int curve, const uint64_t* g_lo, const uint64_t* g_hi, const uint64_t chal[2], size_t n, uint64_t* out_xy, uint8_t* out_inf);
int ipa_round_step(hipStream_t s, int field, int has_fold, const uint64_t* a, const uint64_t* b, const uint64_t* coef, size_t n, size_t cur2, size_t ncoef,
                   const uint64_t u[4], const uint64_t uinv[4], uint64_t* a2, uint64_t* b2, uint64_t* coef2,
                   const uint64_t rand_l[4], const uint64_t rand_r[4], uint64_t* sc, uint64_t* partial, unsigned* counter, unsigned extra, unsigned uslot);
int ipa_round_fold(hipStream_t s, int field, const uint64_t* a, const uint64_t* b, const uint64_t* coef, size_t Nj, size_t ncoef,
                   const uint64_t u[4], const uint64_t uinv[4], uint64_t* a2, uint64_t* b2, uint64_t* coef2);
int ipa_sg_split(hipStream_t s, int field, const uint64_t* coef, size_t n, int has_fold, const uint64_t u[4], uint64_t* out);
int bpoly_run(hipStream_t s, int field, const uint64_t* chals_dev, unsigned rounds, size_t k, const uint64_t* rs_dev, uint64_t* out_dev);
int poly_lincomb(Context& C, int field, const uint64_t* const* segs_dev, const size_t* lens, const uint64_t* scales, size_t m, uint64_t* out_dev, size_t out_len);
int poly_b_init(Context& C, int field, const uint64_t* elm, const uint64_t* scales, size_t k, size_t n, uint64_t* out_dev);
int poly_eval_chunks(Context& C, int field, const uint64_t* const* polys_dev, const size_t* lens, const size_t* num_chunks, size_t m, size_t chunk,
                     const uint64_t* points, size_t npts, uint64_t* out);
int poly_div_vanishing(Context& C, int field, const uint64_t* f_dev, size_t len, size_t n, uint64_t* q_dev, uint64_t* r_dev);
int poly_coset_ntt(Context& C, int field, const uint64_t* coeffs_dev, unsigned log2_n, const uint64_t shift[4], uint64_t* out_dev, size_t batch);
int poly_scan(Context& C, int field, int op, int rev, uint64_t* data_dev, size_t n);
int poly_batch_inversion(Context& C, int field, uint64_t* v_dev, size_t n);
int poly_divide_by_linear(Context& C, int field, const uint64_t* f_dev, size_t len, const uint64_t a[4], uint64_t* q_dev, uint64_t rem[4], uint64_t* rem_dev = nullptr);
int poly_check_equal(Context& C, const uint64_t* v_dev, size_t n, const uint64_t* expect, uint32_t* flags_dev, unsigned bit);
int poly_index_columns(Context& C, int field, const uint8_t* selcol_dev, const uint32_t* wires_dev, const uint64_t* coeffs_dev, size_t n_gates,
                       size_t n, size_t zk_rows, const uint64_t* shifts, size_t ncol, uint64_t* d1_dev);
int lookup_selector_columns(Context& C, int field, const uint8_t* code_dev, size_t n_gates, size_t n, const int* patterns, size_t npat, uint64_t* out_dev);
int lookup_table_columns(Context& C, int field, const uint64_t* segs_dev, const uint64_t* seg_starts , size_t nseg, const uint64_t* data_dev, size_t n, size_t width,
                         uint64_t* tcols_dev, uint64_t* ids_dev, uint64_t* rtsel_dev, size_t rt_offset, size_t rt_len, size_t zk_rows);
int lookup_atom_denominators(Context& C, int field, const uint64_t* x8_dev, size_t n, size_t zk_rows, const uint64_t a[4], const uint64_t omega[4],
                             uint64_t* atoms_dev);
int lookup_atom_finish(Context& C, int field, size_t n, size_t zk_rows, const uint64_t zh8[32], const uint64_t lim0[4], const uint64_t limf[4],
                       uint64_t* atoms_dev);
size_t lookup_sorted_scratch_words(size_t L);
size_t lookup_sorted_status_offset(size_t L);
int lookup_sorted_run(Context& C, const uint64_t* table_dev, size_t L, const uint64_t* values_dev, size_t value_stride, size_t mpr, uint64_t* out_dev,
                      size_t out_stride, uint32_t* scratch_dev);
int gate_count();
// ... 30 lines not shown
```

### proof_systems_amd/csrc/msm_api.cpp

```cpp
#include <stdlib.h>
#include <algorithm>
#include <chrono>

#include "api_internal.hpp"
#include "env.hpp"

using namespace kh;

static int free_slot(Context& C) {
    for (int i = 0; i < MSM_SLOTS; i++) if (!C.slot[i].busy) return i;
    return -1;
}
int kh::acquire_slot(std::unique_lock<std::mutex>* lk, Context& C, bool side_first) {
    const auto me = std::this_thread::get_id();
    auto t_start = std::chrono::steady_clock::now();
    uint64_t seen = ~(uint64_t)0;
    for (;;) {
        uint64_t sig = C.next_ticket;
        for (int i = 0; i < MSM_SLOTS; i++) sig = sig * 1315423911ull + (C.slot[i].busy ? C.slot[i].ticket + 1 : 0);
        if (sig != seen) { seen = sig; t_start = std::chrono::steady_clock::now(); }
        int si = -1;
        if (side_first) for (int i = MSM_SLOTS - 1; i >= 1; i--) if (!C.slot[i].busy) { si = i; break; }
        if (si < 0) si = free_slot(C);
        if (si >= 0 || !lk) return si;
// ... 132 lines not shown
    auto& groups = coalesce_groups(C);
    for (auto& g : groups)
        if (!g->closed && g->members.size() < COALESCE_MAX && g->srs == srs && g->basis == basis && g->chunk == chunk && g->offset == offset && g->n == n && g->mont == mont) {
            std::shared_ptr<CoalesceGroup> grp = g;
            grp->members.push_back({scalars, out_xy, out_inf});
            grp->cv.notify_all();
            grp->cv.wait(lk, [&] { return grp->done; });
            if (grp->rc) set_error("%s", grp->err.c_str());
            return grp->rc;
        }
    std::shared_ptr<CoalesceGroup> grp(new CoalesceGroup);
    grp->srs = srs; grp->basis = basis; grp->chunk = chunk; grp->offset = offset; grp->n = n; grp->mont = mont;
    grp->members.push_back({scalars, out_xy, out_inf});
    groups.push_back(grp);
    if (burst) {
        const auto deadline = now + std::chrono::microseconds(400);
        size_t seen = 1;
        for (;;) {
            grp->cv.wait_for(lk, std::chrono::microseconds(40));
            if (grp->members.size() == seen || grp->members.size() >= COALESCE_MAX || std::chrono::steady_clock::now() >= deadline) break;
            seen = grp->members.size();
        }
    }
    grp->closed = true;
    groups.erase(std::find(groups.begin(), groups.end(), grp));
    const size_t kk = grp->members.size();
    std::vector<uint64_t> res(8 * kk); std::vector<uint8_t> rinf(kk);
    auto run = [&]() -> int {
        MsmBasis b; int r;
        int si = acquire_slot(&lk, C);
        KH_REQUIRE(si >= 0, "%s", slot_error(si));
        MsmSlot& S = C.slot[si];
        if ((r = resolve_counted(srs, basis, chunk, b, S))) return r;
        HandleJobGuard counted{S};
        if ((r = S.ws_scalars.reserve(kk * n * 32))) return r;
        for (size_t j = 0; j < kk; j++)
            KH_HIP(hipMemcpyAsync((char*)S.ws_scalars.p + j * n * 32, grp->members[j].scalars, n * 32, hipMemcpyHostToDevice, S.stream));
        if ((r = msm_enqueue(C, S, srs->curve, b, offset, S.ws_scalars.as<uint64_t>(), n, kk, mont))) return r;
        counted.keep = true;
        return wait_then_finish(lk, C, S, res.data(), rinf.data());
    };
    rc = run();
    if (rc == KH_OK)
        for (size_t j = 0; j < kk; j++) { memcpy(grp->members[j].out_xy, &res[8 * j], 64); *grp->members[j].out_inf = rinf[j]; }
    else grp->err = kh_last_error();
    grp->rc = rc; grp->done = true;
    grp->cv.notify_all();
    return rc;
}

extern "C" {

int kh_msm_set_wide_min_n(size_t n) { msm_set_wide_min_n(n); return KH_OK; }
int kh_msm_set_sort_staging(unsigned entries, unsigned max_passes) {
    if (max_passes > 8) { set_error("kh_msm_set_sort_staging: at most 8 passes (got %u)", max_passes); return KH_E_INVALID; }
    msm_set_sort_staging(entries, max_passes); return KH_OK;
}
int kh_msm_submit(kh_srs_t* srs, int basis, unsigned chunk, size_t offset, const uint64_t* scalars_dev, size_t n, size_t k,
                  int scalars_are_montgomery, uint64_t* ticket) {
    KH_ON_DEVICE_OF(srs);
    KH_REQUIRE(ticket, "null ticket pointer");
    KH_REQUIRE(scalars_dev || n == 0 || k == 0, "null scalars");
    int rc = ensure_init(); if (rc) return rc;
    Context& C = ctx();
    std::unique_lock<std::mutex> lk(C.mu);
    int si = -1;
    if ((rc = msm_submit_locked(C, srs, basis, chunk, offset, scalars_dev, true, n, k, scalars_are_montgomery, &si, &lk))) return rc;
    *ticket = C.slot[si].ticket | ((uint64_t)C.device << 56);
    return KH_OK;
}
int kh_msm_submit_host(kh_srs_t* srs, int basis, unsigned chunk, size_t offset, const uint64_t* scalars, size_t n, size_t k,
                       int scalars_are_montgomery, uint64_t* ticket) {
    KH_ON_DEVICE_OF(srs);
    KH_REQUIRE(ticket, "null ticket pointer");
    KH_REQUIRE(scalars || n == 0 || k == 0, "null scalars");
    int rc = ensure_init(); if (rc) return rc;
    Context& C = ctx();
    std::unique_lock<std::mutex> lk(C.mu);
    int si = -1;
    rc = msm_submit_locked(C, srs, basis, chunk, offset, scalars, false, n, k, scalars_are_montgomery, &si, &lk, true);
    if (rc) { lk.unlock(); hipStream_t cs0 = thread_copy_stream(); if (cs0) (void)hipStreamSynchronize(cs0); return rc; }
    *ticket = C.slot[si].ticket | ((uint64_t)C.device << 56);
    lk.unlock();
    hipStream_t cs = thread_copy_stream();
    if (cs) KH_HIP(hipStreamSynchronize(cs));
    return KH_OK;
}
int kh_msm_wait(uint64_t ticket, uint64_t* out_xy, uint8_t* out_is_inf) {
    KH_REQUIRE(out_xy && out_is_inf, "null output pointer");
    kh::DeviceScope dev_scope_((int)(ticket >> 56));
    int rc = ensure_init(); if (rc) return rc;
    Context& C = ctx();
    std::unique_lock<std::mutex> lk(C.mu);
    const uint64_t seq = ticket & (((uint64_t)1 << 56) - 1);
    for (int i = 0; i < MSM_SLOTS; i++)
        if (C.slot[i].busy && C.slot[i].ticket == seq) return wait_then_finish(lk, C, C.slot[i], out_xy, out_is_inf);
    set_error("unknown or already waited MSM ticket %llu", (unsigned long long)ticket);
    return KH_E_INVALID;
}

int kh_msm_sharded_dev(kh_srs_t* const* shards, size_t R, const uint64_t* const* scalars_dev, const size_t* counts, int scalars_are_montgomery,
                       uint64_t out_xy[8], uint8_t* out_is_inf) {
    KH_REQUIRE(shards && scalars_dev && counts && out_xy && out_is_inf && R > 0, "kh_msm_sharded_dev: null argument");
    KH_REQUIRE(R <= 64, "at most 64 shards (got %zu)", R);
    for (size_t r = 0; r < R; r++) {
        KH_REQUIRE(shards[r], "shard %zu is null", r);
// ... 175 lines not shown
```

### proof_systems_amd/csrc/msm_plan.hpp

```cpp
#pragma once
#include <math.h>
#include <stddef.h>
#include <stdint.h>
#include <algorithm>
#include <map>
#include <mutex>
#include <utility>
#include <vector>

namespace kh {

typedef uint32_t u32;

static constexpr int MSM_SPREAD_SCALARS = 2;
static constexpr int MSM_LATENCY = 4;
constexpr int windows_of(int c) { return (256 + c - 1) / c; }
static constexpr int PART_T = 1024, PART_P = 256, PART_LOW = 7;
static constexpr u32 PART2_MAXLOW = 11, PART2_MAXPASS = 8;
static constexpr u32 MAX_K = 256;
static constexpr int FUSED_T = 1024, FUSED_KPT = 2, FUSED_G = 16, FUSED_B = 64;
static constexpr int FUSED_V = 17, FUSED_C = 16;
static constexpr u32 WIDE_XB = 32, WIDE_HOT_NT = 16;
static constexpr u32 CHUNK = 128;
static constexpr u32 SUM_PER_T = 2, SUM_BLK = 256 * SUM_PER_T;
static constexpr size_t B29_BYTES = 144;
static constexpr u32 SPREAD_MAX_NT = 256;
static constexpr u32 wide_og = 16, wide_acc_blocks = 3, wide_rlog = 4;
static_assert((wide_og & (wide_og - 1)) == 0 && wide_og <= (1u << (17 - 9)) && wide_rlog >= 1 && wide_rlog + 2 <= 17 / 2, "wide-path constants");

struct SortGeom {
    size_t n;
    u32 nb;
    int S;
    int W;
    int precomp;
    size_t pt_stride;
    size_t pt_offset;
    size_t pt_batch;
};
struct KTab { uint8_t k[48]; };
struct FusedGeom {
    u32 n, nb, W, k, bpg, split, sub, kpt, nkeys, room, kmin;
    KTab ktab;
    size_t pt_stride, pt_offset, pt_batch;
};
struct WideTasks { u32 room, kmin, nkeys; KTab ktab; };
struct MargGeom { u32 nb; u32 sh[3]; u32 wd[3]; };
struct WideGeom { u32 nb, lo, hi, rlog, flog; };

#if defined(__HIPCC__)
#define KH_PLAN_FN __host__ __device__ inline __attribute__((always_inline))
#else
#define KH_PLAN_FN inline
#endif
KH_PLAN_FN u32 marginal_bucket(const MargGeom& g, u32 j, u32 v, u32 e) {
    const u32 s = g.sh[j], f = g.wd[j];
    return ((e >> s) << (s + f)) | (v << s) | (e & ((1u << s) - 1u));
}
inline MargGeom marginal_geometry(u32 bits) {
    const u32 f0 = (bits + 2) / 3, f1 = (bits - f0 + 1) / 2, f2 = bits - f0 - f1;
    MargGeom mg;
    mg.nb = 1u << bits; mg.sh[0] = 0; mg.wd[0] = f0; mg.sh[1] = f0; mg.wd[1] = f1; mg.sh[2] = f0 + f1; mg.wd[2] = f2;
    return mg;
}
inline size_t hot_list_cap(size_t nkeys, size_t max_tasks) { return nkeys + max_tasks / CHUNK + 2; }
KH_PLAN_FN void wide_a1_item(const WideGeom& g, u32 out, u32& t0, u32& tstride) {
    const u32 per = g.nb >> g.rlog;
    if (out < per) { t0 = out << g.rlog; tstride = 1u; return; }
    const u32 cpm = (1u << g.hi) >> g.rlog, v = out - per, b = v / cpm, s = v - b * cpm;
    t0 = ((s << g.rlog) << g.lo) + b; tstride = 1u << g.lo;
}

struct MsmShape {
    size_t n = 0, k = 0, offset = 0;
    int flags = 0;
    int precomp_c = 0;
    bool has_wide = false; int wide_c = 0;
    bool glv = false;
    size_t stride = 0, basis_n = 0, batch_stride = 0;
    int num_cus = 256;
    size_t lds_per_cu = (size_t)160 << 10, lds_per_block = (size_t)64 << 10;
    size_t wide_min_n = ~(size_t)0;
    u32 stage_entries = 0, stage_maxpass = 0;
    bool fused_off = false;
    bool flag_off = false;
    bool fin_quad = true;
};

enum MsmSort { SORT_PLAIN = 0, SORT_FUSED, SORT_PARTITIONED };

struct MsmPlan {
    bool wide = false, glv = false;
    int precomp = 0, c = 0, W = 0;
    u32 nb = 0;
    int S = 0, Sq = 0;
    size_t ngroups = 0;
    size_t nkeys = 0, M = 0, tot_e = 0;
    bool few_groups = false, quad_sum = false, spread = false;
    u32 room = 0, kmin = 0; KTab ktab{};
    size_t max_tasks = 0, bigcap = 0, slist_off = 0;
    u32 acc_prio = 0;
    MsmSort sort = SORT_PLAIN;
    SortGeom g{};
    FusedGeom fg{};
    u32 part_low = 0, part_nblk = 0; size_t part_size = 0;
    WideGeom wg{};
    size_t wide_acc_lds = 0;
    u32 stage_now = 0, part2_maxpass = 0; size_t part2_lds = 0;
    u32 acc_blocks = 0, wide_items = 0, wide_runs = 0;
    u32 m = 0, nseg = 0, nblk1 = 0, planes = 0;
    MargGeom mg{};
    size_t tail_groups = 0, nout = 0;
    bool direct_out = false;
    bool want_flag = false;
};

inline int msm_pick_window(size_t n) {
    int lg = 0; while (((size_t)1 << (lg + 1)) <= n) lg++;
    int c = lg - 3;
    if (c < 4) c = 4;
    if (c > 16) c = 16;
    return c;
}

inline KTab task_length_table(size_t nkeys, u32 cus) {
    static std::mutex mu;
    static std::map<std::pair<size_t, u32>, KTab> cache;
    std::lock_guard<std::mutex> lk(mu);
    auto it = cache.find({nkeys, cus});
    if (it != cache.end()) return it->second;
    KTab t{};
    for (int idx = 0; idx < 48; idx++) {
        const double m = pow(2.0, (idx - 8) / 4.0);
        std::vector<double> p(1, exp(-m));
        for (int c = 1; c < (int)(m + 12 * sqrt(m) + 24); c++) p.push_back(p.back() * m / c);
        auto tasks_per_bucket = [&](int K) { double s = 0; for (size_t c = 1; c < p.size(); c++) s += p[c] * (double)((c + K - 1) / K); return s; };
        if (ceil(ceil((double)nkeys * tasks_per_bucket(8) / 256.0) / cus) > 6) { t.k[idx] = 0; continue; }
        double best = 1e300; int bk = 8;
        for (int K = 4; K <= 32; K++) {
            const double tpb = tasks_per_bucket(K);
            const double blocks = ceil((double)nkeys * tpb / 256.0);
            const double len = std::min<double>(K, m + 2.3 * sqrt(m));
            const double cost = ceil(blocks / cus) * len + 2.0 * tpb;
            if (cost < best - 1e-9) { best = cost; bk = K; }
        }
        t.k[idx] = (uint8_t)bk;
    }
    cache[{nkeys, cus}] = t;
    return t;
}

inline int msm_plan(const MsmShape& sh, MsmPlan& P, const char** why) {
    const size_t n = sh.n, k = sh.k;
    P = MsmPlan{};
    const bool wide = P.wide = sh.has_wide && sh.wide_c > 16 && sh.wide_c - 9 <= (int)PART2_MAXLOW && n >= sh.wide_min_n && k <= 4 &&
                               (size_t)windows_of(sh.wide_c) * n <= ((size_t)1 << 26);
    const int c = P.c = wide ? sh.wide_c : (sh.precomp_c ? sh.precomp_c : msm_pick_window(n));
    P.glv = sh.glv && !wide && sh.precomp_c != 0;
    const int W = P.W = P.glv ? 2 * ((128 + c - 1) / c) : windows_of(c);
    const u32 nb = P.nb = 1u << (c - 1);
    const int precomp = P.precomp = (wide || sh.precomp_c) ? 1 : 0;
    int S = (int)(n / 32768); if (S < 1) S = 1; if (S > 16) S = 16;
    { int want = (int)(512 / ((size_t)W * k)); if (want < 1) want = 1; if (S > want) S = want; }
    P.S = S;
    const size_t tab_stride = sh.stride ? sh.stride : sh.basis_n;
    P.g = SortGeom{n, nb, S, W, precomp, tab_stride, sh.offset, sh.batch_stride};
    const size_t ngroups = P.ngroups = precomp ? k : k * (size_t)W;
    P.few_groups = ngroups <= 8;
    P.quad_sum = !wide && precomp && P.few_groups;
    P.spread = P.quad_sum && (sh.flags & MSM_SPREAD_SCALARS) != 0;
    P.acc_prio = (sh.flags & MSM_LATENCY) ? 1u : 0u;
    P.Sq = precomp ? W * S : S;
    const size_t nkeys = P.nkeys = ngroups * nb;
    const size_t M = P.M = n * (size_t)W * k;
    P.tot_e = (size_t)W * n;
    const size_t cap = (size_t)sh.num_cus * 256 * 4;
    size_t room_sz = cap / 4;
    if (nkeys < cap / 2) room_sz = cap - cap / 16 - nkeys / 2;
    P.room = (u32)room_sz;
    P.kmin = 8;
    P.ktab = precomp ? task_length_table(nkeys, (u32)sh.num_cus) : KTab{};
    const size_t max_tasks = P.max_tasks = M / 4 + nkeys + 1;
    if (!(M < ((size_t)1 << 31) && (tab_stride * (size_t)(precomp ? W : 1) + sh.batch_stride * k) < ((size_t)1 << 31))) {
        *why = "MSM too large for 31-bit entry indices";
        return 1;
    }
    P.bigcap = hot_list_cap(nkeys, max_tasks);
    P.slist_off = 2 + 2 * max_tasks;
    P.acc_blocks = wide ? (u32)(nkeys / 256) : (u32)((max_tasks + 255) / 256);
    P.wide_acc_lds = (sh.lds_per_cu / (wide_acc_blocks + 1) + 1024) & ~(size_t)1023;
    if (P.wide_acc_lds > sh.lds_per_block) P.wide_acc_lds = sh.lds_per_block & ~(size_t)1023;
    if (wide) {
        WideGeom& wg = P.wg;
        wg.nb = nb; wg.lo = (u32)c / 2; wg.hi = (u32)(c - 1) - wg.lo; wg.rlog = wide_rlog;
        wg.flog = wg.lo > wg.rlog + 5 ? wg.lo - wg.rlog - 4 : 1;
        P.wide_items = 2u * (nb >> wg.rlog) * (u32)ngroups;
        P.wide_runs = 2u * (nb >> (wg.rlog + wg.flog)) * (u32)ngroups;
    }
    u32 m = 1;
    while (m < 16 && (ngroups * (size_t)nb) / m > 65536) m <<= 1;
    if (!precomp && m < 4) m = 4;
    if (nb < m) m = nb;
    P.m = m;
    P.nseg = nb / m;
    P.nblk1 = (P.nseg + SUM_BLK - 1) / SUM_BLK;
    P.planes = wide ? 3u : ((precomp && ngroups <= 4096 && c >= 7 && c <= 16) ? 3u : 0u);
    if (P.planes) P.mg = marginal_geometry(wide ? P.wg.lo : (u32)c - 1);
    P.tail_groups = wide ? 2 * ngroups : ngroups;
    P.nout = P.planes ? P.tail_groups * P.planes : ngroups;
    bool fused = precomp && !wide && !sh.fused_off && k <= 4 && M < ((size_t)1 << 22) && nb >= 2048 && sh.num_cus >= 128;
    if (fused) {
        FusedGeom& fg = P.fg;
        fg.n = (u32)n; fg.nb = nb; fg.W = (u32)W; fg.k = (u32)k; fg.bpg = (u32)std::min<size_t>(FUSED_G, FUSED_B / (2 * k)); fg.nkeys = (u32)nkeys;
        fg.split = 2; fg.sub = nb / fg.split;
        fg.room = P.room; fg.kmin = P.kmin; fg.ktab = P.ktab; fg.pt_stride = tab_stride; fg.pt_offset = sh.offset; fg.pt_batch = sh.batch_stride;
        const size_t threads = (size_t)fg.bpg * k * fg.split * FUSED_T;
        fg.kpt = (u32)((nkeys + 1 + threads - 1) / threads);
        const size_t tot4 = P.tot_e / 4, chunk4 = (tot4 + fg.bpg - 1) / fg.bpg + 1;
        if (fg.kpt > (u32)FUSED_KPT || n < 4 || P.tot_e % 4 || chunk4 > (size_t)FUSED_V * FUSED_T || fg.sub > (u32)FUSED_C * FUSED_T) { fused = false; fg = FusedGeom{}; }
    }
    const bool part = wide || (precomp && !fused && nb == ((u32)PART_P << PART_LOW) && n <= ((size_t)1 << 20) && W <= 16 && M >= ((size_t)1 << 21));
    P.sort = fused ? SORT_FUSED : (part ? SORT_PARTITIONED : SORT_PLAIN);
    P.part_low = wide ? (u32)c - 9 : (u32)PART_LOW;
    P.part_nblk = wide ? (u32)std::max<size_t>(std::max<size_t>(1, std::min<size_t>(256, 512 / k)), (P.tot_e + 65535) / 65536)
                       : (part ? (u32)std::max<size_t>(1, std::min<size_t>(256, 512 / k)) : 0);
    P.part_size = (size_t)k * PART_P * P.part_nblk;
    if (wide) {
        P.part2_maxpass = std::min<u32>(PART2_MAXPASS, sh.stage_maxpass);
        u32 stage_now = std::min<u32>(sh.stage_entries, (131072u - (1u << PART2_MAXLOW)) / 4u);
        if (stage_now <= 2048u || P.tot_e / PART_P > (size_t)P.part2_maxpass * (stage_now - 1024u)) stage_now = 0;
        const u32 stage_words = std::max<u32>(stage_now, 3u << PART2_MAXLOW);
        P.stage_now = stage_now;
        P.part2_lds = (size_t)stage_words * 4 + (stage_now ? ((size_t)1 << PART2_MAXLOW) : 0);
    }
    P.direct_out = wide || (P.planes && (P.few_groups || sh.fin_quad));
    P.want_flag = !sh.flag_off && (wide || P.planes);
    return 0;
}

}
```

### proof_systems_amd/csrc/srs.cpp

```cpp
#include <stdlib.h>

#include "api_internal.hpp"
#include "srs_file.hpp"

using namespace kh;

int kh::resolve_basis(kh_srs_t* srs, int basis, unsigned chunk, MsmBasis& out) {
    KH_REQUIRE(srs != nullptr, "null SRS handle");
    if (basis == KH_BASIS_G) {
        KH_REQUIRE(chunk == 0, "chunk must be 0 for the monomial basis");
        out.pts = srs->g.p; out.inf = nullptr; out.n = srs->n; out.stride = srs->g_stride; out.precomp_c = srs->g_precomp_c;
        out.wide_pts = srs->g_wide_c ? srs->g_wide.p : nullptr; out.wide_c = srs->g_wide_c;
        return KH_OK;
    }
    std::lock_guard<std::mutex> ml(srs->map_mu);
    auto it = srs->lagrange.find((unsigned)basis);
    if (it == srs->lagrange.end() || chunk >= it->second.size() || !it->second[chunk]) {
        set_error("Lagrange basis for domain 2^%d chunk %u is not registered on this SRS", basis, chunk);
        return KH_E_NOTFOUND;
    }
    LagrangeChunk& L = *it->second[chunk];
    out.pts = L.pts.p; out.inf = L.has_inf ? L.inf.as<uint8_t>() : nullptr; out.n = L.n; out.precomp_c = L.precomp_c;
    return KH_OK;
}

void kh::xyzz_to_affine_batch(const khost::Crv& crv, const std::vector<khost::xyzz>& acc, uint64_t* out_xy, uint8_t* out_inf) {
    const khost::Fld& F = crv.F;
    const size_t k = acc.size();
    std::vector<khost::fe> pre(k + 1);
    pre[0] = F.f.one;
    for (size_t j = 0; j < k; j++) pre[j + 1] = crv.is_identity(acc[j]) ? pre[j] : F.mul(pre[j], acc[j].zzz);
    khost::fe inv = F.inv(pre[k]);
    for (size_t j = k; j-- > 0;) {
        if (crv.is_identity(acc[j])) { memset(out_xy + 8 * j, 0, 64); out_inf[j] = 1; continue; }
        const khost::fe izzz = F.mul(inv, pre[j]);
        inv = F.mul(inv, acc[j].zzz);
        const khost::fe izz = F.sqr(F.mul(izzz, acc[j].zz));
        const khost::fe x = F.mul(acc[j].x, izz), y = F.mul(acc[j].y, izzz);
        memcpy(out_xy + 8 * j, &x, 32); memcpy(out_xy + 8 * j + 4, &y, 32);
        out_inf[j] = 0;
    }
}

static int build_wide_tables(Context& C, kh_srs* s, bool required) {
    if (s->g_wide_c) return KH_OK;
    if (!s->g_precomp_c || (!required && s->n < msm_wide_min_n())) return KH_OK;
    int rc = s->g_wide.reserve(s->g_stride * 64 * (size_t)windows_of(MSM_WIDE_C));
    if (!rc) {
        hipError_t e = hipMemcpyAsync(s->g_wide.p, s->g.p, s->g_stride * 64, hipMemcpyDeviceToDevice, C.stream);
        if (e != hipSuccess) { set_error("hipMemcpyAsync failed: %s", hipGetErrorString(e)); rc = KH_E_DEVICE; }
    }
    if (!rc) rc = msm_precompute(C, s->curve, s->g_wide.p, nullptr, s->g_stride, MSM_WIDE_C);
    if (rc) {
        (void)hipStreamSynchronize(C.stream);
        s->g_wide.release(); s->g_wide_c = 0;
        if (required || rc != KH_E_NOMEM) return rc;
        (void)hipGetLastError();
        set_error("");
        return KH_OK;
    }
    s->g_wide_c = MSM_WIDE_C;
    return KH_OK;
}
static int table_width(size_t n) { return n >= MSM_PRECOMP_MIN_N ? MSM_PRECOMP_C : 0; }
static size_t table_bytes(size_t n, size_t stride) { return stride * 64 * (table_width(n) ? windows_of(table_width(n)) : 1); }
static int build_tables(Context& C, int curve, void* tables, const uint8_t* inf, size_t n, size_t stride, int* c_built) {
    const int c = table_width(n);
    if (c) { int rc = msm_precompute(C, curve, tables, inf, stride, c); if (rc) return rc; }
    *c_built = c;
    return KH_OK;
}
template <class Fill>
static int srs_create(int curve, size_t n, kh_srs_t** out, Fill fill) {
    int rc = ensure_init(); if (rc) return rc;
    std::unique_ptr<kh_srs> s(new kh_srs);
    s->curve = curve; s->n = n;
    Context& C = ctx();
    s->device = C.device;
    std::lock_guard<std::mutex> lk(C.mu);
    s->g_stride = n + 1 + KH_IPA_OPENINGS;
    if ((rc = s->g.reserve(table_bytes(n, s->g_stride)))) return rc;
    if ((rc = fill(C, s->g.p))) return rc;
    for (size_t i = n; i < s->g_stride; i++)
        KH_HIP(hipMemcpyAsync((char*)s->g.p + i * 64, s->g.p, 64, hipMemcpyDeviceToDevice, C.stream));
    if ((rc = build_tables(C, curve, s->g.p, nullptr, n, s->g_stride, &s->g_precomp_c))) return rc;
    if ((rc = build_wide_tables(C, s.get(), false))) return rc;
    KH_HIP(hipStreamSynchronize(C.stream));
    if ((rc = kh_srs_h(curve, s->h))) return rc;
    *out = s.release();
    return KH_OK;
}

extern "C" {

int kh_srs_has_wide_tables(const kh_srs_t* srs) { return srs && srs->g_wide_c ? 1 : 0; }
int kh_srs_set_wide_tables(kh_srs_t* srs, int on) {
    KH_ON_DEVICE_OF(srs);
    KH_REQUIRE(srs != nullptr, "null SRS handle");
    int rc = ensure_init(); if (rc) return rc;
    Context& C = ctx();
    std::lock_guard<std::mutex> lk(C.mu);
    if (on) {
        KH_REQUIRE(srs->g_precomp_c, "kh_srs_set_wide_tables: the handle has no window tables (fewer than %d points)", (int)MSM_PRECOMP_MIN_N);
        std::lock_guard<std::mutex> wl(srs->wide_mu);
        if (srs->g_wide_c) return KH_OK;
        if ((rc = build_wide_tables(C, srs, true))) return rc;
        const int built = srs->g_wide_c;
        srs->g_wide_c = 0;
        const hipError_t e = hipStreamSynchronize(C.stream);
        if (e != hipSuccess) { srs->g_wide.release(); KH_HIP(e); }
        srs->g_wide_c = built;
        return KH_OK;
    }
    std::lock_guard<std::mutex> wl(srs->wide_mu);
    KH_REQUIRE(srs->jobs->load() == 0, "kh_srs_set_wide_tables: an MSM is in flight (kh_msm_wait first)");
    srs->g_wide_c = 0;
    srs->g_wide.release();
    return KH_OK;
}
int kh_srs_create(int curve, const uint64_t* g_xy, size_t n, kh_srs_t** out) {
    KH_REQUIRE(out && g_xy && n > 0, "kh_srs_create: null argument or n == 0");
    KH_REQUIRE(curve == KH_CURVE_VESTA || curve == KH_CURVE_PALLAS, "unknown curve id %d", curve);
    return srs_create(curve, n, out, [&](Context&, void* g) -> int { KH_HIP(hipMemcpy(g, g_xy, n * 64, hipMemcpyHostToDevice)); return KH_OK; });
}
int kh_srs_create_device(int curve, size_t depth, kh_srs_t** out) { return kh_srs_create_device_range(curve, 0, depth, out); }
int kh_srs_create_device_range(int curve, size_t start, size_t depth, kh_srs_t** out) {
    KH_REQUIRE(out && depth > 0, "kh_srs_create_device: null argument or depth == 0");
    KH_REQUIRE(curve == KH_CURVE_VESTA || curve == KH_CURVE_PALLAS, "unknown curve id %d", curve);
    KH_REQUIRE(start + depth <= ((size_t)1 << 32), "SRS index must fit u32 (ipa.rs:758)");
    return srs_create(curve, depth, out, [&](Context& C, void* g) { return srs_generate_device(C, curve, start, depth, g); });
}
int kh_srs_create_compressed(int curve, const uint8_t* g_bytes, size_t n, const uint8_t* h_bytes, kh_srs_t** out) {
    KH_REQUIRE(out && g_bytes && n > 0, "kh_srs_create_compressed: null argument or n == 0");
    KH_REQUIRE(curve == KH_CURVE_VESTA || curve == KH_CURVE_PALLAS, "unknown curve id %d", curve);
    KH_REQUIRE(n < ((size_t)1 << 32), "kh_srs_create_compressed: %zu records, the limit is 2^32 - 1", n);
    const size_t m = n + (h_bytes ? 1 : 0);
    uint64_t h_xy[8];
    kh_srs_t* srs = nullptr;
    int rc = srs_create(curve, n, &srs, [&](Context& C, void* g) -> int {
        DevBuf &rec = C.scratch("point_codec_bytes"), &inf = C.scratch("point_codec_inf"), &st = C.scratch("point_codec_status");
        int r;
        if ((r = rec.reserve(m * KH_POINT_BYTES)) || (r = inf.reserve(m)) || (r = st.reserve(m))) return r;
        KH_HIP(hipMemcpyAsync(rec.p, g_bytes, n * KH_POINT_BYTES, hipMemcpyHostToDevice, C.stream));
        if (h_bytes) KH_HIP(hipMemcpyAsync(rec.as<uint8_t>() + n * KH_POINT_BYTES, h_bytes, KH_POINT_BYTES, hipMemcpyHostToDevice, C.stream));
        if ((r = points_decompress_launch(C, curve, rec.as<uint8_t>(), m, (uint64_t*)g, inf.as<uint8_t>(), st.as<uint8_t>(), nullptr, 0))) return r;
        std::vector<uint8_t> status(m);
        KH_HIP(hipMemcpyAsync(status.data(), st.p, m, hipMemcpyDeviceToHost, C.stream));
        if (h_bytes) KH_HIP(hipMemcpyAsync(h_xy, (const char*)g + n * 64, 64, hipMemcpyDeviceToHost, C.stream));
        KH_HIP(hipStreamSynchronize(C.stream));
        for (size_t i = 0; i < m; i++) {
            if (status[i] == KH_POINT_OK) continue;
            if (i < n) set_error("kh_srs_create_compressed: record %zu is %s: a basis point must be a point", i, point_status_name(status[i]));
            else set_error("kh_srs_create_compressed: the record of the blinding base is %s", point_status_name(status[i]));
            return KH_E_INVALID;
        }
        return KH_OK;
    });
    if (rc) return rc;
    if (h_bytes && (rc = kh_srs_set_blinding_base(srs, h_xy))) { kh_srs_free(srs); return rc; }
// ... 205 lines not shown
```

### proof_systems_amd/khip.py

```python
from __future__ import annotations

import ctypes as C
import os

import numpy as np

from . import _abi

_HERE = os.path.dirname(os.path.abspath(__file__))
LIB_PATH = os.environ.get("KH_LIB") or os.path.join(_HERE, "libkimchi_hip.so")

if not os.path.exists(LIB_PATH):
    raise ImportError(f"{LIB_PATH} is missing: run `python -c 'import __graft_entry__ as g; g.build()'` "
                      "(hipcc --offload-arch=gfx950); there is no CPU fallback")
try:
    _PROTOTYPES, _STRUCTS, _CONSTANTS = _abi.parse()
except OSError as e:
    raise ImportError(f"{_abi.HEADER} is missing: the binding is declared from it ({e})") from e

_lib = C.CDLL(LIB_PATH)

SYMBOLS = list(_PROTOTYPES)

def __getattr__(name: str):
    try:
        return _CONSTANTS["KH_" + name]
    except KeyError:
        raise AttributeError(f"module {__name__!r} has no attribute {name!r}") from None


VESTA, PALLAS = _CONSTANTS["KH_CURVE_VESTA"], _CONSTANTS["KH_CURVE_PALLAS"]
FP, FQ = _CONSTANTS["KH_FIELD_FP"], _CONSTANTS["KH_FIELD_FQ"]
BASIS_G = _CONSTANTS["KH_BASIS_G"]
PROVE_CHECK = _CONSTANTS["KH_PROVE_CHECK"]
WITNESS_GATES, WITNESS_WIRES, WITNESS_LOOKUPS = _CONSTANTS["KH_WITNESS_GATES"], _CONSTANTS["KH_WITNESS_WIRES"], _CONSTANTS["KH_WITNESS_LOOKUPS"]


def _sections(prefix: str):
    return {name[len(prefix):].lower(): value for name, value in _CONSTANTS.items() if name.startswith(prefix)}


_BY_VALUE = {"int": C.c_int, "unsigned": C.c_uint, "size_t": C.c_size_t, "uint64_t": C.c_uint64, "uint32_t": C.c_uint32, "uint8_t": C.c_uint8,
             "double": C.c_double, "float": C.c_float}
_STRUCTURES = {}


def _ctype(ctype: str, name: str = ""):
    toks = ctype.replace("*", " * ").split()
    depth = toks.count("*")
    base, = [t for t in toks if t not in ("const", "*")]
    if depth and (name.endswith("_dev") or base == "void" or (base.startswith("kh_") and base not in _STRUCTURES)):
        t, depth = C.c_void_p, depth - 1
    elif depth and base == "char":
        t, depth = C.c_char_p, depth - 1
    else:
        t = None if base == "void" else _STRUCTURES.get(base) or _BY_VALUE[base]
    for _ in range(depth):
        t = C.POINTER(t)
    return t


def _structure(name: str, fields):
    members = []
    for field, ctype, dims in fields:
        t = _ctype(ctype)
        for d in reversed(dims):
            t = t * d
        members.append((field, t))
    return type("".join(w.capitalize() for w in name[3:-2].split("_")) + "C", (C.Structure,), {"__doc__": name, "_fields_": members})


for _name, _fields in _STRUCTS.items():
    _STRUCTURES[_name] = _structure(_name, _fields)
LookupTableC, RuntimeTableCfgC = _STRUCTURES["kh_lookup_table_t"], _STRUCTURES["kh_runtime_table_cfg_t"]
WitnessReportC, WitnessLookupC = _STRUCTURES["kh_witness_report_t"], _STRUCTURES["kh_witness_lookup_t"]
SectionC, VerifyItemC, VerifyTraceC = _STRUCTURES["kh_section_t"], _STRUCTURES["kh_verify_item_t"], _STRUCTURES["kh_verify_trace_t"]

for _name, (_ret, _params) in _PROTOTYPES.items():
    _fn = getattr(_lib, _name, None)
    if _fn is not None:
        _fn.restype = _ctype(_ret)
        _fn.argtypes = [_ctype(_t, _p) for _t, _p in _params]

U64P = C.POINTER(C.c_uint64)
U8P = C.POINTER(C.c_uint8)

# ... 22 lines not shown
    return a if shape is None else a.reshape(shape)


def raw():
    return _lib


def device_count() -> int:
    return _lib.kh_device_count()


def init(device: int = -1, timers: bool = True):
    _check(_lib.kh_init(device))
    if timers:
        _check(_lib.kh_set_phase_timers(1))


def set_device(device: int):
    _check(_lib.kh_set_device(device))


def get_device() -> int:
    return _lib.kh_get_device()


def trim():
    _check(_lib.kh_trim())


def set_phase_timers(on: bool):
    _check(_lib.kh_set_phase_timers(int(bool(on))))


def set_sort_staging(entries: int = 28672, max_passes: int = 2):
    _check(_lib.kh_msm_set_sort_staging(entries, max_passes))


def glv_split(scalar_field: int, scalars):
    a = np.ascontiguousarray(scalars, dtype=np.uint64)
    n = a.shape[0]
    out = np.zeros((n, 10), np.uint32)
    _check(_lib.kh_debug_glv_split(scalar_field, _p64(a), n, out.ctypes.data_as(C.POINTER(C.c_uint32))))
    res = []
    for row in out:
        m1 = sum(int(row[t]) << (32 * t) for t in range(4)); m2 = sum(int(row[4 + t]) << (32 * t) for t in range(4))
        res.append((-m1 if row[8] else m1, -m2 if row[9] else m2))
    return res


def set_wide_min_n(n: int):
    _check(_lib.kh_msm_set_wide_min_n(n))


POINT_BYTES = _CONSTANTS["KH_POINT_BYTES"]
POINT_OK, POINT_INFINITY, POINT_BAD_FLAGS, POINT_NOT_CANONICAL, POINT_NOT_ON_CURVE = (_CONSTANTS["KH_POINT_" + _n] for _n in (
    "OK", "INFINITY", "BAD_FLAGS", "NOT_CANONICAL", "NOT_ON_CURVE"))


def _records(b):
    if isinstance(b, (bytes, bytearray, memoryview)):
        b = np.frombuffer(bytes(b), dtype=np.uint8)
    elif isinstance(b, (list, tuple)):
        b = np.frombuffer(b"".join(bytes(r) for r in b), dtype=np.uint8)
    return np.ascontiguousarray(b, dtype=np.uint8).reshape(-1, POINT_BYTES)


def points_compress(curve: int, xy, inf=None):
    xy = _c64(xy, (-1, 8))
    if inf is not None:
        inf = np.ascontiguousarray(inf, dtype=np.uint8).reshape(-1)
    out = np.zeros((xy.shape[0], POINT_BYTES), dtype=np.uint8)
    _check(_lib.kh_points_compress(curve, _p64(xy), _p8(inf), xy.shape[0], _p8(out)))
    return out


def points_decompress_raw(curve: int, records):
    rec = _records(records)
    n = rec.shape[0]
    xy = np.zeros((n, 8), dtype=np.uint64); inf = np.zeros(n, dtype=np.uint8); status = np.zeros(n, dtype=np.uint8)
    first = C.c_size_t(n)
    rc = _lib.kh_points_decompress(curve, _p8(rec), n, _p64(xy), _p8(inf), _p8(status), C.byref(first))
    return rc, xy, inf, status, (first.value if first.value < n else None)


def points_decompress(curve: int, records):
    rc, xy, inf, _status, _first = points_decompress_raw(curve, records)
    _check(rc)
    return xy, inf


def points_compress_dev(curve: int, xy, inf, n: int, out):
    _check(_lib.kh_points_compress_dev(curve, _ptr(xy), _ptr(inf), n, _ptr(out)))


def points_decompress_dev(curve: int, records, n: int, out_xy, out_inf, status=None, flags=None, bit: int = 0):
    _check(_lib.kh_points_decompress_dev(curve, _ptr(records), n, _ptr(out_xy), _ptr(out_inf), _ptr(status), _ptr(flags), bit))


class Srs:

    def __init__(self, curve: int, g_xy=None, depth: int = 0, start: int = 0):
        self.curve = curve
        self._h = C.c_void_p()
        if g_xy is None:
            self.n = depth
            _check(_lib.kh_srs_create_device_range(curve, start, depth, C.byref(self._h)))
# ... 6 lines not shown
    def create(cls, curve: int, depth: int, start: int = 0):
        return cls(curve, None, depth, start)

    @classmethod
    def _adopt(cls, curve: int, handle):
        self = cls.__new__(cls)
        self.curve, self._h, self.n = curve, handle, int(_lib.kh_srs_size(handle))
        return self

    @classmethod
    def from_compressed(cls, curve: int, g_bytes, h_bytes=None):
        g = _records(g_bytes)
        h = _records(h_bytes) if h_bytes is not None else None
        handle = C.c_void_p()
        _check(_lib.kh_srs_create_compressed(curve, _p8(g), g.shape[0], _p8(h), C.byref(handle)))
        return cls._adopt(curve, handle)

    @classmethod
    def from_file_bytes(cls, curve: int, data: bytes, limit: int = 0):
        buf = np.frombuffer(bytes(data) + b"\0", dtype=np.uint8)
        handle = C.c_void_p()
        _check(_lib.kh_srs_create_from_file(curve, buf.ctypes.data_as(U8P), buf.size - 1, limit, C.byref(handle)))
        return cls._adopt(curve, handle)

    def to_file_bytes(self) -> bytes:
        out = np.zeros(int(_lib.kh_srs_file_bytes(self.n)), dtype=np.uint8)
        _check(_lib.kh_srs_write_file(self._h, _p8(out), out.size))
        return out.tobytes()

    def get_g(self, offset: int = 0, count: int = None):
        count = self.n - offset if count is None else count
        out = np.zeros((count, 8), dtype=np.uint64)
        _check(_lib.kh_srs_get_g(self._h, offset, count, _p64(out)))
        return out

    def get_g_compressed(self, offset: int = 0, count: int = None):
        count = self.n - offset if count is None else count
        out = np.zeros((count, POINT_BYTES), dtype=np.uint8)
        _check(_lib.kh_srs_get_g_compressed(self._h, offset, count, _p8(out)))
        return out

    def debug_rebase_points(self, coef):
        c = _c64(coef, (-1, 4))
        N = self.n // c.shape[0]
        out = np.zeros((N, 8), dtype=np.uint64); fail = C.c_uint32(0)
        _check(_lib.kh_debug_rebase_points(self._h, _p64(c), c.shape[0], _p64(out), C.byref(fail)))
        if fail.value:
            raise KhError("rebase: an output is the point at infinity")
        return out

    def has_wide_tables(self) -> bool:
        return bool(_lib.kh_srs_has_wide_tables(self._h))

    def set_wide_tables(self, on: bool):
        _check(_lib.kh_srs_set_wide_tables(self._h, int(on)))

    def close(self):
        if self._h:
            _lib.kh_srs_free(self._h)
            self._h = C.c_void_p()

    def __del__(self):
        try:
            self.close()
        except Exception:
            pass

    def set_lagrange(self, log2_domain: int, xy, inf=None, chunk: int = 0):
        xy = _c64(xy, (-1, 8))
        if inf is not None:
            inf = np.ascontiguousarray(inf, dtype=np.uint8)
        _check(_lib.kh_srs_set_lagrange(self._h, log2_domain, chunk, _p64(xy), _p8(inf), xy.shape[0]))

    def compute_lagrange(self, log2_domain: int):
        _check(_lib.kh_srs_compute_lagrange(self._h, log2_domain))

    def get_lagrange(self, log2_domain: int, chunk: int = 0):
        n = 1 << log2_domain
        xy = np.zeros((n, 8), dtype=np.uint64)
        inf = np.zeros(n, dtype=np.uint8)
        _check(_lib.kh_srs_get_lagrange(self._h, log2_domain, chunk, _p64(xy), _p8(inf)))
        return xy, inf

    def lagrange_chunks(self, log2_domain: int) -> int:
        return _lib.kh_srs_lagrange_chunks(self._h, log2_domain)

    def max_poly_size(self) -> int:
        return self.n

    def blinding_commitment(self):
        out = np.zeros(8, dtype=np.uint64)
        _check(_lib.kh_srs_get_blinding_base(self._h, _p64(out)))
        return out

    def set_blinding_base(self, h_xy):
        h = _c64(h_xy, (8,))
        _check(_lib.kh_srs_set_blinding_base(self._h, _p64(h)))

    def commit_non_hiding(self, coeffs, num_chunks: int):
        c = _c64(coeffs, (-1, 4))
        cap = max(num_chunks, -(-c.shape[0] // self.n), 1)
        out = np.zeros((cap, 8), dtype=np.uint64)
        inf = np.zeros(cap, dtype=np.uint8)
        cnt = C.c_size_t(0)
        _check(_lib.kh_commit_non_hiding(self._h, _p64(c), c.shape[0], num_chunks, _p64(out), _p8(inf), C.byref(cnt)))
        return out[:cnt.value], inf[:cnt.value]

    def commit_evaluations_non_hiding(self, log2_domain: int, evals):
# ... 1429 lines not shown
```

### rust/kimchi-hip-sys/src/lib.rs

```rust
#![allow(non_camel_case_types, clippy::too_many_arguments, clippy::missing_safety_doc)]

use core::ffi::{c_char, c_int, c_uint, c_void};

#[repr(C)]
pub struct kh_srs_t {
    _private: [u8; 0],
}
#[repr(C)]
pub struct kh_ipa_t {
    _private: [u8; 0],
}
#[repr(C)]
pub struct kh_sponge_t {
    _private: [u8; 0],
}
#[repr(C)]
pub struct kh_prover_index_t {
    _private: [u8; 0],
}
#[repr(C)]
pub struct kh_proof_t {
    _private: [u8; 0],
}
#[repr(C)]
// ... 132 lines not shown
    pub slot: c_int,
    pub ncells: c_int,
    pub cols: [c_int; 3],
    pub table_id: [u64; 4],
    pub entry: [[u64; 4]; 3],
    pub lookups_missing: usize,
}
#[repr(C)]
#[derive(Clone, Copy)]
pub struct kh_section_t {
    pub limbs: *const u64,
    pub flags: *const u8,
    pub count: usize,
}
#[repr(C)]
#[derive(Clone, Copy)]
pub struct kh_verify_item_t {
    pub index: *const kh_verifier_index_t,
    pub proof: *const kh_proof_t,
    pub public_inputs: *const u64,
    pub n_public: usize,
    pub prev_chals: *const u64,
    pub prev_rounds: *const c_uint,
    pub prev_comm_xy: *const u64,
    pub prev_comm_inf: *const u8,
    pub prev_comm_chunks: *const usize,
    pub n_prev: usize,
}
#[repr(C)]
#[derive(Clone, Copy)]
pub struct kh_verify_trace_t {
    pub challenges: [[u64; 4]; 7],
    pub constant_term: [u64; 4],
    pub ft_eval0: [u64; 4],
    pub combined_inner_product: [u64; 4],
}
#[repr(C)]
#[derive(Clone, Copy)]
pub struct kh_wire_section_t {
    pub bytes: *const u8,
    pub count: usize,
}

pub const KH_OK: c_int = 0;
pub const KH_E_INVALID: c_int = -1;
pub const KH_E_DEVICE: c_int = -2;
pub const KH_E_NOTFOUND: c_int = -3;
pub const KH_E_NOMEM: c_int = -4;
pub const KH_CURVE_VESTA: c_int = 0;
pub const KH_CURVE_PALLAS: c_int = 1;
pub const KH_FIELD_FP: c_int = 0;
pub const KH_FIELD_FQ: c_int = 1;
pub const KH_BASIS_G: c_int = -1;
pub const KH_REF_NONE: c_int = -2;
pub const KH_REF_ARENA: c_int = -1;
pub const KH_STEP_NO_FLAG: c_int = 255;
pub const KH_IPA_OPENINGS: c_int = 4;
pub const KH_E_BLINDERS: c_int = -5;
pub const KH_MSM_SLOTS: c_int = 4;
pub const KH_E_SORT_GAVE_UP: c_int = -6;
pub const KH_COMM_ID_BYTES: c_int = 128;
pub const KH_PROVE_CHECK: c_int = 1;
pub const KH_PROVE_ALL_GATES: c_int = 2;
pub const KH_PROVE_EAGER_CHECK: c_int = 8;
pub const KH_PROVE_SHARED_CONTEXT: c_int = 4;
pub const KH_PROOF_W_COMM: c_int = 0;
pub const KH_PROOF_Z_COMM: c_int = 1;
pub const KH_PROOF_T_COMM: c_int = 2;
pub const KH_PROOF_PUBLIC_COMM: c_int = 3;
pub const KH_PROOF_EVALS: c_int = 4;
pub const KH_PROOF_PUBLIC_EVALS: c_int = 5;
pub const KH_PROOF_FT_EVAL1: c_int = 6;
pub const KH_PROOF_LR: c_int = 7;
pub const KH_PROOF_DELTA: c_int = 8;
pub const KH_PROOF_Z1_Z2: c_int = 9;
pub const KH_PROOF_SG: c_int = 10;
pub const KH_PROOF_CHALLENGES: c_int = 11;
pub const KH_PROOF_LOOKUP_SORTED_COMM: c_int = 12;
pub const KH_PROOF_LOOKUP_AGGREG_COMM: c_int = 13;
pub const KH_PROOF_LOOKUP_RUNTIME_COMM: c_int = 14;
pub const KH_GATE_ZERO: c_int = -1;
pub const KH_VINDEX_SIGMA_COMM: c_int = 0;
pub const KH_VINDEX_COEFFICIENTS_COMM: c_int = 1;
pub const KH_VINDEX_GENERIC_COMM: c_int = 2;
pub const KH_VINDEX_SELECTOR_COMM: c_int = 3;
pub const KH_VINDEX_OPTIONAL_COMM: c_int = 4;
pub const KH_VINDEX_SHIFTS: c_int = 5;
pub const KH_VINDEX_DIGEST: c_int = 6;
pub const KH_GATE_LOOKUP: c_int = -2;
pub const KH_VINDEX_LOOKUP_TABLE_COMM: c_int = 7;
pub const KH_VINDEX_LOOKUP_TABLE_IDS_COMM: c_int = 8;
pub const KH_VINDEX_LOOKUP_SELECTOR_COMM: c_int = 9;
pub const KH_VINDEX_LOOKUP_RUNTIME_SELECTOR_COMM: c_int = 10;
pub const KH_VINDEX_LOOKUP_INFO: c_int = 11;
pub const KH_LOOKUP_COL_SELECTOR_D1: c_int = 0;
pub const KH_LOOKUP_COL_SELECTOR_C: c_int = 1;
pub const KH_LOOKUP_COL_SELECTOR_D8: c_int = 2;
pub const KH_LOOKUP_COL_TABLE_D1: c_int = 3;
pub const KH_LOOKUP_COL_TABLE_IDS_D1: c_int = 4;
pub const KH_LOOKUP_COL_ATOM_D8: c_int = 5;
pub const KH_LOOKUP_COL_RUNTIME_SELECTOR: c_int = 6;
pub const KH_WITNESS_GATES: c_int = 1;
pub const KH_WITNESS_WIRES: c_int = 2;
pub const KH_WITNESS_LOOKUPS: c_int = 4;
pub const KH_WITNESS_OK: c_int = 0;
pub const KH_WITNESS_DISCONNECTED: c_int = 1;
// ... 8 lines not shown
pub const KH_SPONGE_FQ: c_int = 0;
pub const KH_SPONGE_FR: c_int = 1;
pub const KH_TOK_CONST: c_int = 0;
pub const KH_TOK_CELL: c_int = 1;
pub const KH_TOK_DUP: c_int = 2;
pub const KH_TOK_POW: c_int = 3;
pub const KH_TOK_ADD: c_int = 4;
pub const KH_TOK_MUL: c_int = 5;
pub const KH_TOK_SUB: c_int = 6;
pub const KH_TOK_STORE: c_int = 7;
pub const KH_TOK_LOAD: c_int = 8;
pub const KH_CELL_FIELD: c_int = 0;
pub const KH_CELL_INT256: c_int = 1;
pub const KH_CELL_INT128: c_int = 2;
pub const KH_CELL_LIMB88: c_int = 3;
pub const KH_CELL_U64: c_int = 4;
pub const KH_STEP_GATHER: c_int = 0;
pub const KH_STEP_SCATTER: c_int = 1;
pub const KH_STEP_GENERIC: c_int = 2;
pub const KH_STEP_POSEIDON: c_int = 3;
pub const KH_STEP_COMPLETE_ADD: c_int = 4;
pub const KH_STEP_VARBASEMUL: c_int = 5;
pub const KH_STEP_ENDOMUL: c_int = 6;
pub const KH_STEP_ENDOMUL_SCALAR: c_int = 7;
pub const KH_STEP_RANGE_CHECK: c_int = 8;
pub const KH_STEP_XOR: c_int = 9;
pub const KH_STEP_ROT64: c_int = 10;
pub const KH_STEP_FF_ADD: c_int = 11;
pub const KH_STEP_FF_MUL: c_int = 12;
pub const KH_STEP_LOOKUP: c_int = 14;
pub const KH_STEP_INVERSE: c_int = 15;
pub const KH_STEP_SQRT: c_int = 16;
pub const KH_STEP_BITS: c_int = 17;
pub const KH_SCAN_ADD: c_int = 0;
pub const KH_SCAN_MUL: c_int = 1;

#[link(name = "kimchi_hip")]
extern "C" {
    pub fn kh_device_count() -> c_int;
    pub fn kh_init(device_id: c_int) -> c_int;
    pub fn kh_set_device(device_id: c_int) -> c_int;
    pub fn kh_get_device() -> c_int;
    pub fn kh_private_context_begin() -> c_int;
    pub fn kh_private_context_end() -> c_int;
    pub fn kh_private_context_active() -> c_int;
    pub fn kh_set_phase_timers(on: c_int) -> c_int;
    pub fn kh_trim() -> c_int;
    pub fn kh_last_error() -> *const c_char;
    pub fn kh_srs_create(curve: c_int, g_xy: *const u64, n: usize, out: *mut *mut kh_srs_t) -> c_int;
    pub fn kh_msm_set_wide_min_n(n: usize) -> c_int;
    pub fn kh_msm_set_sort_staging(entries: c_uint, max_passes: c_uint) -> c_int;
    pub fn kh_srs_set_wide_tables(srs: *mut kh_srs_t, on: c_int) -> c_int;
    pub fn kh_srs_has_wide_tables(srs: *const kh_srs_t) -> c_int;
    pub fn kh_srs_free(srs: *mut kh_srs_t);
    pub fn kh_srs_size(srs: *const kh_srs_t) -> usize;
    pub fn kh_srs_curve(srs: *const kh_srs_t) -> c_int;
    pub fn kh_srs_device(srs: *const kh_srs_t) -> c_int;
    pub fn kh_srs_generate(curve: c_int, start: usize, count: usize, out_xy: *mut u64, threads: c_int) -> c_int;
    pub fn kh_srs_h(curve: c_int, out_xy: *mut u64) -> c_int;
    pub fn kh_group_map_to_group(curve: c_int, t: *const u64, out_xy: *mut u64) -> c_int;
    pub fn kh_srs_create_device(curve: c_int, depth: usize, out: *mut *mut kh_srs_t) -> c_int;
    pub fn kh_srs_create_device_range(curve: c_int, start: usize, count: usize, out: *mut *mut kh_srs_t) -> c_int;
    pub fn kh_srs_get_g(srs: *mut kh_srs_t, offset: usize, count: usize, out_xy: *mut u64) -> c_int;
    pub fn kh_srs_set_lagrange(srs: *mut kh_srs_t, log2_domain: c_uint, chunk: c_uint, xy: *const u64, inf: *const u8, n: usize) -> c_int;
    pub fn kh_srs_compute_lagrange(srs: *mut kh_srs_t, log2_domain: c_uint) -> c_int;
    pub fn kh_srs_get_lagrange(srs: *mut kh_srs_t, log2_domain: c_uint, chunk: c_uint, out_xy: *mut u64, out_inf: *mut u8) -> c_int;
    pub fn kh_srs_lagrange_chunks(srs: *const kh_srs_t, log2_domain: c_uint) -> c_int;
    pub fn kh_msm(srs: *mut kh_srs_t, basis: c_int, chunk: c_uint, offset: usize, scalars: *const u64, n: usize, scalars_are_montgomery: c_int, out_xy: *mut u64, out_is_inf: *mut u8) -> c_int;
    pub fn kh_msm_batch(srs: *mut kh_srs_t, basis: c_int, chunk: c_uint, offset: usize, scalars: *const u64, n: usize, k: usize, scalars_are_montgomery: c_int, out_xy: *mut u64, out_is_inf: *mut u8) -> c_int;
    pub fn kh_msm_points(curve: c_int, xy: *const u64, inf: *const u8, scalars: *const u64, n: usize, scalars_are_montgomery: c_int, out_xy: *mut u64, out_is_inf: *mut u8) -> c_int;
    pub fn kh_msm_points_batch(curve: c_int, xy: *const u64, inf: *const u8, scalars: *const u64, n: usize, k: usize, scalars_are_montgomery: c_int, out_xy: *mut u64, out_is_inf: *mut u8) -> c_int;
    pub fn kh_points_sum(curve: c_int, xy: *const u64, inf: *const u8, n: usize, out_xy: *mut u64, out_is_inf: *mut u8) -> c_int;
    pub fn kh_points_add(curve: c_int, a_xy: *const u64, a_inf: *const u8, b_xy: *const u64, b_inf: *const u8, n: usize, out_xy: *mut u64, out_is_inf: *mut u8) -> c_int;
    pub fn kh_msm_sharded(shards: *const *mut kh_srs_t, R: usize, scalars: *const u64, n: usize, scalars_are_montgomery: c_int, out_xy: *mut u64, out_is_inf: *mut u8) -> c_int;
    pub fn kh_msm_sharded_dev(shards: *const *mut kh_srs_t, R: usize, scalars_dev: *const *const u64, counts: *const usize, scalars_are_montgomery: c_int, out_xy: *mut u64, out_is_inf: *mut u8) -> c_int;
    pub fn kh_ipa_fold_scalars(field: c_int, lo: *const u64, hi: *const u64, u: *const u64, n: usize, out: *mut u64) -> c_int;
    pub fn kh_inner_product(field: c_int, a: *const u64, b: *const u64, n: usize, out: *mut u64) -> c_int;
    pub fn kh_ipa_fold_points(curve: c_int, g_lo_xy: *const u64, g_hi_xy: *const u64, u: *const u64, n: usize, out_xy: *mut u64, out_inf: *mut u8) -> c_int;
    pub fn kh_ipa_fold_points_endo(curve: c_int, g_lo_xy: *const u64, g_hi_xy: *const u64, chal: *const u64, n: usize, out_xy: *mut u64, out_inf: *mut u8) -> c_int;
    pub fn kh_endos(curve: c_int, endo_q: *mut u64, endo_r: *mut u64) -> c_int;
    pub fn kh_scalar_challenge_to_field(curve: c_int, chal: *const u64, out: *mut u64) -> c_int;
    pub fn kh_combine_polys_dev(field: c_int, polys_dev: *const *const u64, lens: *const usize, num_chunks: *const usize, m: usize, polyscale: *const u64, srs_length: usize, out_dev: *mut u64, out_len: *mut usize) -> c_int;
    pub fn kh_poly_lincomb_dev(field: c_int, polys_dev: *const *const u64, lens: *const usize, scalars: *const u64, m: usize, out_dev: *mut u64, out_len: usize) -> c_int;
    pub fn kh_b_init_dev(field: c_int, elm: *const u64, k: usize, evalscale: *const u64, padded_len: usize, out_dev: *mut u64) -> c_int;
    pub fn kh_evaluate_chunks_dev(field: c_int, coeffs_dev: *const u64, len: usize, chunk_size: usize, num_chunks: usize, points: *const u64, npts: usize, out: *mut u64) -> c_int;
    pub fn kh_evaluate_chunks_batch_dev(field: c_int, polys_dev: *const *const u64, lens: *const usize, num_chunks: *const usize, m: usize, chunk_size: usize, points: *const u64, npts: usize, out: *mut u64) -> c_int;
    pub fn kh_divide_by_vanishing_poly_dev(field: c_int, f_dev: *const u64, len: usize, log2_n: c_uint, q_dev: *mut u64, r_dev: *mut u64) -> c_int;
    pub fn kh_expr_evaluations_dev(field: c_int, tokens: *const u32, ntok: usize, cols_dev: *const *const u64, col_len: *const usize, ncols: usize, constants: *const u64, nconsts: usize, rows: usize, stride: c_uint, next_shift: c_uint, accumulate: c_int, out_dev: *mut u64) -> c_int;
    pub fn kh_gate_count() -> c_int;
    pub fn kh_gate_name(gate: c_int) -> *const c_char;
    pub fn kh_gate_num_constants(gate: c_int) -> c_int;
    pub fn kh_gate_constants(field: c_int, gate: c_int, alpha: *const u64, endo: *const u64, params: *const u64, nparams: usize, out: *mut u64) -> c_int;
    pub fn kh_gate_evaluations_dev(field: c_int, gate: c_int, cols_dev: *const *const u64, col_len: usize, constants: *const u64, nconsts: usize, rows: usize, stride: c_uint, next_shift: c_uint, accumulate: c_int, out_dev: *mut u64) -> c_int;
    pub fn kh_poseidon_gate_coefficients(field: c_int, out: *mut u64) -> c_int;
    pub fn kh_poseidon_permute_dev(field: c_int, states_dev: *mut u64, n: usize) -> c_int;
    pub fn kh_poseidon_hash_dev(field: c_int, msgs_dev: *const u64, msg_len: usize, n: usize, init: *const u64, digests_dev: *mut u64) -> c_int;
    pub fn kh_poseidon_gate_witness_dev(field: c_int, states_dev: *const u64, n: usize, rows: *const u32, row0: usize, row_stride: usize, witness_dev: *mut u64, col_stride: usize, col_len: usize, out_states_dev: *mut u64) -> c_int;
    pub fn kh_poseidon_set_split_max_n(n: usize) -> c_int;
    pub fn kh_complete_add_witness_dev(field: c_int, p1_dev: *const u64, p2_dev: *const u64, n: usize, rows: *const u32, row0: usize, row_stride: usize, witness_dev: *mut u64, col_stride: usize, col_len: usize, out_dev: *mut u64) -> c_int;
    pub fn kh_varbasemul_witness_dev(field: c_int, base_dev: *const u64, acc0_dev: *const u64, scalars_dev: *const u64, num_bits: c_uint, n: usize, rows: *const u32, row0: usize, row_stride: usize, witness_dev: *mut u64, col_stride: usize, col_len: usize, out_acc_dev: *mut u64, out_n_dev: *mut u64, flags_dev: *mut u32, bit: c_uint) -> c_int;
    pub fn kh_endomul_witness_dev(field: c_int, endo: *const u64, base_dev: *const u64, acc0_dev: *const u64, chals_dev: *const u64, num_bits: c_uint, n: usize, rows: *const u32, row0: usize, row_stride: usize, witness_dev: *mut u64, col_stride: usize, col_len: usize, out_acc_dev: *mut u64, out_n_dev: *mut u64, flags_dev: *mut u32, bit: c_uint) -> c_int;
    pub fn kh_curve_witness_set_slice_elements(elements: usize) -> c_int;
    pub fn kh_endomul_scalar_witness_dev(field: c_int, chals_dev: *const u64, num_bits: c_uint, n: usize, rows: *const u32, row0: usize, row_stride: usize, witness_dev: *mut u64, col_stride: usize, col_len: usize, endo_scalar: *const u64, out_dev: *mut u64) -> c_int;
    pub fn kh_foreign_field_gate_coefficients(field: c_int, modulus: *const u64, out: *mut u64) -> c_int;
    pub fn kh_range_check_witness_dev(field: c_int, limbs_dev: *const u64, n: usize, compact: c_int, rows: *const u32, row0: usize, row_stride: usize, witness_dev: *mut u64, col_stride: usize, col_len: usize, flags_dev: *mut u32, bit: c_uint) -> c_int;
    pub fn kh_xor_witness_dev(field: c_int, in1_dev: *const u64, in2_dev: *const u64, bits: c_uint, n: usize, rows: *const u32, row0: usize, row_stride: usize, witness_dev: *mut u64, col_stride: usize, col_len: usize, out_dev: *mut u64, flags_dev: *mut u32, bit: c_uint) -> c_int;
// ... 138 lines not shown
```

Before: 1105 Mscalar/s.

## Add shifted wide precompute tables to shrink the bucket count in wide-window MSM

Adds a shifted wide-table kind in which each window's table also stores point multiples for several shift values. Digits are split into a shift index and a reduced bucket, so fewer buckets are populated and the shift index selects the table row. Partitioning, sorting, accumulation and bucket indexing are changed to map keys to true bucket records, skip holes, and launch smaller blocks when there are few keys. This is meant to cut the bucket-reduction and accumulation work, in exchange for a table several times larger, extra digit decoding, and a fallback to plain tables when memory runs short.

Result: slower. 649.8 Mscalar/s (-41.2%).

```diff
diff --git a/include/kimchi_hip.h b/include/kimchi_hip.h
--- a/include/kimchi_hip.h
+++ b/include/kimchi_hip.h
@@ -37,8 +37,12 @@
 int kh_srs_create(int curve, const uint64_t *g_xy , size_t n, kh_srs_t **out);
 int kh_msm_set_wide_min_n(size_t n);
 int kh_msm_set_sort_staging(unsigned entries, unsigned max_passes);
-int kh_srs_set_wide_tables(kh_srs_t *srs, int on);
+#define KH_WIDE_PLAIN 1
+#define KH_WIDE_SHIFTED 2
+int kh_srs_set_wide_tables(kh_srs_t *srs, int on );
 int kh_srs_has_wide_tables(const kh_srs_t *srs);
+int kh_srs_wide_tables_kind(const kh_srs_t *srs);
+int kh_msm_set_wide_table_limit(size_t bytes);
 void kh_srs_free(kh_srs_t *srs);
 size_t kh_srs_size(const kh_srs_t *srs);
 int kh_srs_curve(const kh_srs_t *srs);
diff --git a/proof_systems_amd/csrc/api_internal.hpp b/proof_systems_amd/csrc/api_internal.hpp
--- a/proof_systems_amd/csrc/api_internal.hpp
+++ b/proof_systems_amd/csrc/api_internal.hpp
@@ -40,6 +40,7 @@
     kh::DevBuf g;
     size_t g_stride = 0;
     int g_precomp_c = 0;
+    int g_wide_kind = 0;
     kh::DevBuf g_wide; int g_wide_c = 0;
     std::shared_ptr<std::atomic<int>> jobs = std::make_shared<std::atomic<int>>(0);
     std::mutex wide_mu;
diff --git a/proof_systems_amd/csrc/common.hpp b/proof_systems_amd/csrc/common.hpp
--- a/proof_systems_amd/csrc/common.hpp
+++ b/proof_systems_amd/csrc/common.hpp
@@ -93,7 +93,7 @@
     size_t stride = 0;
     size_t batch_stride = 0;
     const void* wide_pts = nullptr;
-    int wide_c = 0;
+    int wide_c = 0, wide_kind = 0;
     bool glv = false;
 };
 
diff --git a/proof_systems_amd/csrc/msm.hip b/proof_systems_amd/csrc/msm.hip
--- a/proof_systems_amd/csrc/msm.hip
+++ b/proof_systems_amd/csrc/msm.hip
@@ -307,7 +307,7 @@
     return active ? atomicAdd(&ctr[key], 1u) : 0u;
 }
 __global__ void __launch_bounds__(PART_T)
-k_part_hist(const int32_t* __restrict__ digits, u32 tot_e, u32 nblk, u32 shift, u32* __restrict__ PH) {
+k_part_hist(const int32_t* __restrict__ digits, u32 tot_e, u32 nblk, u32 shift, int wide_kind, u32* __restrict__ PH) {
     KH_HIGH_PRIO();
     __shared__ u32 cnt[PART_P];
     const u32 blk = blockIdx.x, j = blockIdx.y, tid = threadIdx.x;
@@ -320,7 +320,11 @@
 #pragma unroll
         for (int u = 0; u < 8; u++) { const u32 e = e0 + u * PART_T; v[u] = d[e < e_hi ? e : e_hi - 1]; if (e >= e_hi) v[u] = 0; }
 #pragma unroll
-        for (int u = 0; u < 8; u++) (void)lds_inc_agg(cnt, (((u32)(v[u] < 0 ? -v[u] : v[u]) - 1u) >> shift) & (PART_P - 1u), v[u] != 0);
+        for (int u = 0; u < 8; u++) {
+            u32 b = (u32)(v[u] < 0 ? -v[u] : v[u]) - 1u;
+            if (wide_kind == WIDE_SHIFTED) { u32 j, dp; wide_shift_digit(b + 1u, j, dp); b = (dp - 1u) >> 1; }
+            (void)lds_inc_agg(cnt, (b >> shift) & (PART_P - 1u), v[u] != 0);
+        }
     }
     __syncthreads();
     if (tid < PART_P) PH[((size_t)j * PART_P + tid) * nblk + blk] = cnt[tid];
@@ -663,7 +667,7 @@
     }
 }
 __global__ void __launch_bounds__(PART_T)
-k_part2_scatter(const int32_t* __restrict__ digits, u32 tot_e, u32 nblk, u32 low, const u32* __restrict__ PO, u32* __restrict__ mid, u32* __restrict__ xlist, u32* __restrict__ big) {
+k_part2_scatter(const int32_t* __restrict__ digits, u32 tot_e, u32 nblk, u32 low, int wide_kind, const u32* __restrict__ PO, u32* __restrict__ mid, u32* __restrict__ xlist, u32* __restrict__ big) {
     KH_HIGH_PRIO();
     __shared__ u32 cur[PART_P];
     const u32 blk = blockIdx.x, j = blockIdx.y, tid = threadIdx.x;
@@ -678,9 +682,11 @@
         for (int u = 0; u < 8; u++) { const u32 e = e0 + u * PART_T; v[u] = d[e < e_hi ? e : e_hi - 1]; if (e >= e_hi) v[u] = 0; }
 #pragma unroll
         for (int u = 0; u < 8; u++) {
-            const u32 b = (u32)(v[u] < 0 ? -v[u] : v[u]) - 1u;
-            const u32 pos = lds_inc_agg(cur, b & (PART_P - 1u), v[u] != 0);
-            if (v[u]) mid[pos] = ((b >> 8) << 17) | (v[u] < 0 ? 1u << 16 : 0u) | (e0 + u * PART_T - e_lo);
+            u32 j = 0, dp = (u32)(v[u] < 0 ? -v[u] : v[u]);
+            if (wide_kind == WIDE_SHIFTED) wide_shift_digit(dp, j, dp);
+            const u32 key = wide_key_of_bucket(wide_kind, low, dp - 1u);
+            const u32 pos = lds_inc_agg(cur, (key >> low) & (PART_P - 1u), v[u] != 0);
+            if (v[u]) mid[pos] = (j << 28) | ((key & ((1u << low) - 1u)) << 17) | (v[u] < 0 ? 1u << 16 : 0u) | (e0 + u * PART_T - e_lo);
         }
     }
 }
@@ -688,7 +694,7 @@
 k_part2_sort(const u32* __restrict__ mid, const u32* __restrict__ PO, u32 nblk, u32 low, u32 nb, u32 tot_e, u32 n, size_t pt_stride, size_t pt_offset,
              size_t pt_batch, u32 last_group, size_t total_idx, WideTasks ta, u32* __restrict__ off, u32* __restrict__ entries,
              u32* __restrict__ toff, u32* __restrict__ order, u32* __restrict__ ptot, u32* __restrict__ xlist, u32* __restrict__ slist,
-             uint8_t* __restrict__ buckets29, u32 og, u32 stage_cap, u32 max_pass, u32* __restrict__ big, u32 bigcap, u32 hot_nt) {
+             uint8_t* __restrict__ buckets29, u32 og, u32 stage_cap, u32 max_pass, u32* __restrict__ big, u32 bigcap, u32 hot_nt, int wide_kind, u32 hf, u32 tab_log) {
     KH_HIGH_PRIO();
     __shared__ u32 cur[1u << PART2_MAXLOW], pstart[1025], bi0[1024], bw0[1024], lh[MAX_K + 2], sh[PART_T / 64 + 1];
     __shared__ u32 xl_n, pfirst[PART2_MAXPASS], plast[PART2_MAXPASS];
@@ -713,11 +719,12 @@
 #pragma unroll
         for (int u = 0; u < 8; u++) { const u32 x = x0 + u * PART_T; m[u] = mid[x < end ? x : end - 1]; }
 #pragma unroll
-        for (int u = 0; u < 8; u++) (void)lds_inc_agg(cur, m[u] >> 17, x0 + u * PART_T < end);
+        for (int u = 0; u < 8; u++) (void)lds_inc_agg(cur, (m[u] >> 17) & (nbl - 1u), x0 + u * PART_T < end);
     }
     __syncthreads();
     {
         const u32 i0 = 2 * tid, a = i0 < nbl ? cur[i0] : 0u, b = i0 + 1 < nbl ? cur[i0 + 1] : 0u;
+        const bool has_a = i0 < nbl, has_b = i0 + 1 < nbl && wide_local_populated(hf, i0 + 1);
         u32 btot;
         const u32 ex = base + block_scan_1024(a + b, sh, &btot);
         __syncthreads();
@@ -732,22 +739,22 @@
         if (i0 < nbl) toff[key0] = tex;
         if (i0 + 1 < nbl) toff[key0 + 1] = tex + nta;
         if (tid == 0) ptot[q] = btot;
-        if (i0 < nbl) atomicAdd(&lh[la], 1u);
-        if (i0 + 1 < nbl) atomicAdd(&lh[lb], 1u);
+        if (has_a) atomicAdd(&lh[la], 1u);
+        if (has_b) atomicAdd(&lh[lb], 1u);
         if (nta > 1) { const u32 sl = atomicAdd(&xl_n, 1u); xl_key[sl] = (u32)key0; xl_nt[sl] = nta; xl_base[sl] = atomicAdd(&xlist[0], nta - 1u); slist[atomicAdd(&xlist[1], 1u)] = (u32)key0; }
         if (ntb > 1) { const u32 sl = atomicAdd(&xl_n, 1u); xl_key[sl] = (u32)key0 + 1u; xl_nt[sl] = ntb; xl_base[sl] = atomicAdd(&xlist[0], ntb - 1u); slist[atomicAdd(&xlist[1], 1u)] = (u32)key0 + 1u; }
         if (nta > hot_nt) { const u32 sl = atomicAdd(&big[0], 1u); big[2 + sl] = (u32)key0; big[2 + bigcap + sl] = 0u; }
         if (ntb > hot_nt) { const u32 sl = atomicAdd(&big[0], 1u); big[2 + sl] = (u32)key0 + 1u; big[2 + bigcap + sl] = 0u; }
-        if (i0 < nbl && a == 0) { uint4* rec = (uint4*)(buckets29 + ((size_t)j * nb + ((size_t)i0 << 8 | pidx)) * B29_BYTES); _Pragma("unroll") for (int t = 0; t < 9; t++) rec[t] = make_uint4(0u, 0u, 0u, 0u); }
-        if (i0 + 1 < nbl && b == 0) { uint4* rec = (uint4*)(buckets29 + ((size_t)j * nb + ((size_t)(i0 + 1) << 8 | pidx)) * B29_BYTES); _Pragma("unroll") for (int t = 0; t < 9; t++) rec[t] = make_uint4(0u, 0u, 0u, 0u); }
+        if (has_a && a == 0) { uint4* rec = (uint4*)(buckets29 + (size_t)wide_true_bucket(wide_kind, (u32)key0, low) * B29_BYTES); _Pragma("unroll") for (int t = 0; t < 9; t++) rec[t] = make_uint4(0u, 0u, 0u, 0u); }
+        if (has_b && b == 0) { uint4* rec = (uint4*)(buckets29 + (size_t)wide_true_bucket(wide_kind, (u32)key0 + 1u, low) * B29_BYTES); _Pragma("unroll") for (int t = 0; t < 9; t++) rec[t] = make_uint4(0u, 0u, 0u, 0u); }
         __syncthreads();
         const u32 L = MAX_K - (tid <= MAX_K ? tid : MAX_K), hv = tid <= MAX_K ? lh[L] : 0u;
         const u32 above = block_scan_1024(hv, sh, &btot);
         __syncthreads();
         if (tid <= MAX_K) lh[L] = above;
         __syncthreads();
-        if (i0 < nbl) { const u32 r = atomicAdd(&lh[la], 1u); order[(size_t)(r / og) * nparts * og + q * og + (r % og)] = (u32)key0; }
-        if (i0 + 1 < nbl) { const u32 r = atomicAdd(&lh[lb], 1u); order[(size_t)(r / og) * nparts * og + q * og + (r % og)] = (u32)key0 + 1u; }
+        if (has_a) { const u32 r = atomicAdd(&lh[la], 1u); order[(size_t)(r / og) * nparts * og + q * og + (r % og)] = (u32)key0; }
+        if (has_b) { const u32 r = atomicAdd(&lh[lb], 1u); order[(size_t)(r / og) * nparts * og + q * og + (r % og)] = (u32)key0 + 1u; }
         const u32 nx = xl_n;
         for (u32 it = 0; it < nx; it++) {
             const u32 key = xl_key[it], ntx = xl_nt[it], xb = xl_base[it];
@@ -784,13 +791,13 @@
 #pragma unroll
                 for (int u = 0; u < 4; u++) {
                     if (x0 + u * 64 >= re) break;
-                    const u32 bk = m[u] >> 17;
+                    const u32 bk = (m[u] >> 17) & (nbl - 1u);
                     const bool live = x0 + u * 64 + lane < re && (!staged || bpass[bk] == pass);
                     const u32 pos = lds_inc_agg(cur, bk, live);
                     if (live) {
                         u32 w = w0, i = i0 + (m[u] & 0xffffu);
                         while (i >= n) { i -= n; w++; }
-                        const u32 val = (pb0 + (u32)(w * pt_stride) + i) | ((m[u] & (1u << 16)) << 15);
+                        const u32 val = (pb0 + (u32)((size_t)((w << tab_log) + (m[u] >> 28)) * pt_stride) + i) | ((m[u] & (1u << 16)) << 15);
                         if (staged && pos - p0 < stage_cap) stage[pos - p0] = val;
                         else entries[pos] = val;
                     }
@@ -884,13 +891,11 @@
     }
     r.store(partial + t * 128);
 }
-__device__ __forceinline__ u32 wide_true_bucket(u32 key, u32 low) {
-    const u32 nbl = 1u << low, grp = key >> (low + 8), kk = key & ((nbl << 8) - 1u);
-    return (grp << (low + 8)) | ((kk & (nbl - 1u)) << 8) | (kk >> low);
-}
+struct WideKey { u32 low; int kind; };
+__device__ __forceinline__ u32 wide_record_of(u32 key, WideKey wk) { return wide_true_bucket(wk.kind, key, wk.low); }
 template <class BF>
 __device__ __forceinline__ bool wide_task29(u32 key, u32 jt, const u32* __restrict__ entries, const u32* __restrict__ off, const u32* __restrict__ toff,
-                                            const uint8_t* __restrict__ pts, uint8_t* __restrict__ partial, uint8_t* __restrict__ buckets29, u32 low, u32* __restrict__ handed) {
+                                            const uint8_t* __restrict__ pts, uint8_t* __restrict__ partial, uint8_t* __restrict__ buckets29, WideKey wk, u32* __restrict__ handed) {
     const u32 o0 = off[key], cnt = off[key + 1] - o0;
     if (cnt == 0) return true;
     const u32 t0 = toff[key], nt = toff[key + 1] - t0;
@@ -923,7 +928,7 @@
         if (!ok) break;
     }
     if (!ok) { if (!handed) return false; const u32 slot = atomicAdd(&handed[0], 1u); handed[2 + 2 * slot] = key; handed[3 + 2 * slot] = jt; return true; }
-    if (nt == 1) { store_b29<BF>(buckets29 + (size_t)wide_true_bucket(key, low) * B29_BYTES, acc); return true; }
+    if (nt == 1) { store_b29<BF>(buckets29 + (size_t)wide_record_of(key, wk) * B29_BYTES, acc); return true; }
     Xyzz<BF> r;
     r.x = from29<BF>(acc.x); r.y = from29<BF>(acc.y); r.zz = from29<BF>(acc.zz); r.zzz = from29<BF>(acc.zzz);
     r.store(partial + (size_t)(t0 + jt) * 128);
@@ -931,7 +936,7 @@
 }
 template <class BF>
 __device__ __forceinline__ void wide_task_exact(u32 key, u32 jt, const u32* __restrict__ entries, const u32* __restrict__ off, const u32* __restrict__ toff,
-                                                const uint8_t* __restrict__ pts, uint8_t* __restrict__ partial, uint8_t* __restrict__ buckets29, u32 low) {
+                                                const uint8_t* __restrict__ pts, uint8_t* __restrict__ partial, uint8_t* __restrict__ buckets29, WideKey wk) {
     const u32 o0 = off[key], cnt = off[key + 1] - o0, t0 = toff[key], nt = toff[key + 1] - t0;
     if (cnt == 0) return;
     const u32 start = o0 + (u32)(((u64)jt * cnt) / nt), end = o0 + (u32)(((u64)(jt + 1) * cnt) / nt);
@@ -945,30 +950,30 @@
         acc = madd<BF>(acc, p, (e >> 31) != 0);
     }
     if (nt == 1) {
-        uint8_t* const rec = buckets29 + (size_t)wide_true_bucket(key, low) * B29_BYTES;
+        uint8_t* const rec = buckets29 + (size_t)wide_record_of(key, wk) * B29_BYTES;
         if (acc.is_identity()) store_b29_identity<BF>(rec); else store_b29<BF>(rec, xyzz_to29<BF>(acc));
     } else acc.store(partial + (size_t)(t0 + jt) * 128);
 }
 template <class BF>
 __global__ void __launch_bounds__(256) __attribute__((amdgpu_num_vgpr(112), amdgpu_waves_per_eu(4, 4)))
 k_acc_wide29(const u32* __restrict__ entries, const u32* __restrict__ off, const u32* __restrict__ toff, const u32* __restrict__ order, u32 nkeys,
-             const uint8_t* __restrict__ pts, uint8_t* __restrict__ partial, uint8_t* __restrict__ buckets29, u32 low, u32* __restrict__ handed) {
+             const uint8_t* __restrict__ pts, uint8_t* __restrict__ partial, uint8_t* __restrict__ buckets29, WideKey wk, u32* __restrict__ handed) {
     const u32 g = blockIdx.x * blockDim.x + threadIdx.x;
-    if (g < nkeys) (void)wide_task29<BF>(order[g], 0u, entries, off, toff, pts, partial, buckets29, low, handed);
+    if (g < nkeys) (void)wide_task29<BF>(order[g], 0u, entries, off, toff, pts, partial, buckets29, wk, handed);
 }
 template <class BF>
 __global__ void __launch_bounds__(256)
 k_acc_wide_rest(const u32* __restrict__ entries, const u32* __restrict__ off, const u32* __restrict__ toff, const u32* __restrict__ xlist, const u32* __restrict__ handed,
-                const uint8_t* __restrict__ pts, uint8_t* __restrict__ partial, uint8_t* __restrict__ buckets29, u32 low) {
+                const uint8_t* __restrict__ pts, uint8_t* __restrict__ partial, uint8_t* __restrict__ buckets29, WideKey wk) {
     KH_HIGH_PRIO();
     const u32 nx = xlist[0], nh = handed[0];
     for (u32 it = blockIdx.x * blockDim.x + threadIdx.x; it < nx; it += gridDim.x * blockDim.x) {
         const u32 key = xlist[2 + 2 * it], jt = xlist[3 + 2 * it];
-        if (!wide_task29<BF>(key, jt, entries, off, toff, pts, partial, buckets29, low, nullptr))
-            wide_task_exact<BF>(key, jt, entries, off, toff, pts, partial, buckets29, low);
+        if (!wide_task29<BF>(key, jt, entries, off, toff, pts, partial, buckets29, wk, nullptr))
+            wide_task_exact<BF>(key, jt, entries, off, toff, pts, partial, buckets29, wk);
     }
     for (u32 it = blockIdx.x * blockDim.x + threadIdx.x; it < nh; it += gridDim.x * blockDim.x)
-        wide_task_exact<BF>(handed[2 + 2 * it], handed[3 + 2 * it], entries, off, toff, pts, partial, buckets29, low);
+        wide_task_exact<BF>(handed[2 + 2 * it], handed[3 + 2 * it], entries, off, toff, pts, partial, buckets29, wk);
 }
 __device__ __forceinline__ size_t hot_key(u32 slot) { return 2 + (size_t)slot; }
 __device__ __forceinline__ size_t hot_cbase(size_t cap, u32 slot) { return 2 + cap + slot; }
@@ -1244,7 +1249,7 @@
 template <class BF>
 __global__ void __launch_bounds__(256)
 k_bucket_sum_wide(const u32* __restrict__ toff, const u32* __restrict__ xlist, const u32* __restrict__ slist, const uint8_t* __restrict__ partial,
-                  uint8_t* __restrict__ buckets29, u32 low, u32 SMALL_NT, u32* __restrict__ big, u32 cap, uint8_t* __restrict__ chunk_out) {
+                  uint8_t* __restrict__ buckets29, WideKey wk, u32 SMALL_NT, u32* __restrict__ big, u32 cap, uint8_t* __restrict__ chunk_out) {
     KH_HIGH_PRIO();
     __shared__ __attribute__((aligned(16))) uint8_t total[4 * 128];
     const u32 count = xlist[1], nhot = big[0];
@@ -1254,7 +1259,7 @@
         if (nt > SMALL_NT) continue;
         Xyzz<BF> acc = Xyzz<BF>::load(partial + (size_t)t0 * 128);
         for (u32 k = 1; k < nt; k++) acc = add<BF>(acc, Xyzz<BF>::load(partial + (size_t)(t0 + k) * 128));
-        uint8_t* const rec = buckets29 + (size_t)wide_true_bucket(key, low) * B29_BYTES;
+        uint8_t* const rec = buckets29 + (size_t)wide_record_of(key, wk) * B29_BYTES;
         if (acc.is_identity()) store_b29_identity<BF>(rec); else store_b29<BF>(rec, xyzz_to29<BF>(acc));
     }
     if (nhot == 0) return;
@@ -1279,7 +1284,7 @@
                 __builtin_amdgcn_wave_barrier();
                 if (lane == 0) {
                     const Xyzz<BF> v = Xyzz<BF>::load(total + 128 * wave);
-                    uint8_t* const rec = buckets29 + (size_t)wide_true_bucket(key, low) * B29_BYTES;
+                    uint8_t* const rec = buckets29 + (size_t)wide_record_of(key, wk) * B29_BYTES;
                     if (v.is_identity()) store_b29_identity<BF>(rec); else store_b29<BF>(rec, xyzz_to29<BF>(v));
                 }
                 __builtin_amdgcn_wave_barrier();
@@ -1313,26 +1318,26 @@
     const u32 gid = blockIdx.x * blockDim.x + threadIdx.x;
     if (gid >= items * ngroups) return;
     const u32 q = gid / items, u = gid - q * items;
-    u32 out = u;
-    if (u >= per) { const u32 v = u - per, b = v & ((1u << g.lo) - 1u), sc = v >> g.lo; out = per + b * ((1u << g.hi) >> g.rlog) + sc; }
-    u32 t0, ts;
-    wide_a1_item(g, out, t0, ts);
-    wide_sum29<BF>(buckets29 + ((size_t)q * g.nb + t0) * B29_BYTES, (size_t)ts * B29_BYTES, 1u << g.rlog, out29 + ((size_t)q * items + out) * B29_BYTES);
+    const u32 out = wide_a1_thread(g, u);
+    u32 t0, ts, n;
+    wide_a1_span(g, out, t0, ts, n);
+    wide_sum29<BF>(buckets29 + ((size_t)q * g.nb + t0) * B29_BYTES, (size_t)ts * B29_BYTES, n, out29 + ((size_t)q * items + out) * B29_BYTES);
 }
 template <class BF>
 __global__ void __launch_bounds__(256)
-k_wide_l2(const uint8_t* __restrict__ in29, u32 flog, u32 nrec, uint8_t* __restrict__ out29) {
+k_wide_l2(const uint8_t* __restrict__ in29, WideGeom g, u32 nrec, uint8_t* __restrict__ out29) {
     KH_HIGH_PRIO();
     const u32 gid = blockIdx.x * blockDim.x + threadIdx.x;
     if (gid >= nrec) return;
-    wide_sum29<BF>(in29 + ((size_t)gid << flog) * B29_BYTES, B29_BYTES, 1u << flog, out29 + (size_t)gid * B29_BYTES);
+    bool empty;
+    const u32 run = wide_l2_thread(g, gid, empty);
+    wide_sum29<BF>(in29 + ((size_t)run << g.flog) * B29_BYTES, B29_BYTES, empty ? 0u : 1u << g.flog, out29 + (size_t)run * B29_BYTES);
 }
 template <class BF>
 __device__ __attribute__((noinline)) Xyzz<BF> wide_chunk_exact(const uint8_t* __restrict__ buckets29g, WideGeom g, u32 out) {
-    u32 t0, ts;
-    wide_a1_item(g, out, t0, ts);
+    u32 t0, ts, r;
+    wide_a1_span(g, out, t0, ts, r);
     Xyzz<BF> acc = Xyzz<BF>::identity();
-    const u32 r = 1u << g.rlog;
     for (u32 i = 0; i < r; i++) {
         const Acc29<BF> b = load_b29<BF>(buckets29g + ((size_t)t0 + (size_t)i * ts) * B29_BYTES);
         if (!is_identity29<BF>(b)) acc = add<BF>(acc, xyzz_from29<BF>(b));
@@ -1384,7 +1389,7 @@
 
 template <class BF>
 __global__ void __launch_bounds__(256)
-k_precompute(uint8_t* __restrict__ tables, const uint8_t* __restrict__ inf, size_t n, int c, int W, uint8_t* __restrict__ scratch) {
+k_precompute(uint8_t* __restrict__ tables, const uint8_t* __restrict__ inf, size_t n, int c, int W, int sub, uint8_t* __restrict__ scratch) {
     size_t i = (size_t)blockIdx.x * blockDim.x + threadIdx.x;
     if (i >= n) return;
     if (inf && inf[i]) {
@@ -1394,7 +1399,8 @@
     Xyzz<BF> P = Xyzz<BF>::from_affine(Aff<BF>::load(tables + i * 64));
     Fe<BF> prod = Fe<BF>::one();
     for (int w = 1; w < W; w++) {
-        for (int k = 0; k < c; k++) P = dbl<BF>(P);
+        const int steps = (w % sub) ? 1 : c - (sub - 1);
+        for (int k = 0; k < steps; k++) P = dbl<BF>(P);
         P.store(scratch + ((size_t)(w - 1) * n + i) * 128);
         prod = mul<BF>(prod, P.zzz);
         prod.store(tables + ((size_t)w * n + i) * 64);
@@ -1426,6 +1432,9 @@
 void msm_set_sort_staging(unsigned entries, unsigned max_passes) { sort_staging_cell(0).store(entries); sort_staging_cell(1).store(max_passes); }
 size_t msm_wide_min_n() { const size_t v = wide_min_n_cell().load(); return v ? v : ~(size_t)0; }
 void msm_set_wide_min_n(size_t n) { wide_min_n_cell().store(n); }
+static std::atomic<size_t>& wide_table_limit_cell() { static std::atomic<size_t> v{0}; return v; }
+void msm_set_wide_table_limit(size_t bytes) { wide_table_limit_cell().store(bytes); }
+size_t msm_wide_table_limit() { return wide_table_limit_cell().load(); }
 static int msm_reserve(Context& Ctx, MsmSlot& C, const MsmPlan& P, bool& flag_on) {
     hipStream_t s = C.stream;
     const size_t nkeys = P.nkeys, M = P.M, max_tasks = P.max_tasks, ngroups = P.ngroups;
@@ -1591,17 +1600,17 @@
     } else if (P.sort == SORT_PARTITIONED) {
         const u32 tot_e = (u32)P.tot_e, part_nblk = P.part_nblk, part_low = P.part_low;
         const dim3 pgrid(part_nblk, (unsigned)k);
-        hipLaunchKernelGGL(k_part_hist, pgrid, dim3(PART_T), 0, s, C.ws_digits.as<int32_t>(), tot_e, part_nblk, wide ? 0u : part_low, C.ws_hist.as<u32>());
+        hipLaunchKernelGGL(k_part_hist, pgrid, dim3(PART_T), 0, s, C.ws_digits.as<int32_t>(), tot_e, part_nblk, wide ? 0u : part_low, P.wide_kind, C.ws_hist.as<u32>());
         C.timer.mark("histogram", s);
         if ((rc = exclusive_scan_u32(C.ws_hist.as<u32>(), C.ws_cnt.as<u32>(), P.part_size + 1, C.ws_scan_tmp, s))) return rc;
         C.timer.mark("scan", s);
         if (wide) {
-            hipLaunchKernelGGL(k_part2_scatter, pgrid, dim3(PART_T), 0, s, C.ws_digits.as<int32_t>(), tot_e, part_nblk, part_low, C.ws_cnt.as<u32>(), C.ws_mid.as<u32>(), C.ws_xlist.as<u32>(), C.ws_biglist.as<u32>());
+            hipLaunchKernelGGL(k_part2_scatter, pgrid, dim3(PART_T), 0, s, C.ws_digits.as<int32_t>(), tot_e, part_nblk, part_low, P.wide_kind, C.ws_cnt.as<u32>(), C.ws_mid.as<u32>(), C.ws_xlist.as<u32>(), C.ws_biglist.as<u32>());
             const WideTasks wt{P.room, P.kmin, (u32)nkeys, P.ktab};
             u32* const ptot = C.ws_ntask.as<u32>();
             hipLaunchKernelGGL(k_part2_sort, dim3(PART_P, (unsigned)k), dim3(PART_T), P.part2_lds, s, C.ws_mid.as<u32>(), C.ws_cnt.as<u32>(), part_nblk, part_low, P.nb, tot_e, (u32)n,
                                P.g.pt_stride, sh.offset, sh.batch_stride, (u32)(k - 1), P.part_size, wt, C.ws_off.as<u32>(), C.ws_entries.as<u32>(),
-                               C.ws_toff.as<u32>(), order, ptot, C.ws_xlist.as<u32>(), slist, C.ws_b29.as<uint8_t>(), wide_og, P.stage_now, P.part2_maxpass, C.ws_biglist.as<u32>(), (u32)P.bigcap, WIDE_HOT_NT);
+                               C.ws_toff.as<u32>(), order, ptot, C.ws_xlist.as<u32>(), slist, C.ws_b29.as<uint8_t>(), wide_og, P.stage_now, P.part2_maxpass, C.ws_biglist.as<u32>(), (u32)P.bigcap, WIDE_HOT_NT, P.wide_kind, P.wg.hf, P.tab_log);
             hipLaunchKernelGGL(k_wide_fixup, dim3((unsigned)(nkeys / 256 + 1)), dim3(256), 0, s, C.ws_toff.as<u32>(), ptot, (u32)(k * PART_P), part_low, (u32)nkeys,
                                C.ws_handed.as<u32>(), C.ws_biglist.as<u32>());
         } else {
@@ -1653,19 +1662,20 @@
     u32* const slist = sort_views(C, P).slist;
     const u32* abort_dev = fused ? C.ws_sync.as<u32>() + 2 + 2 * FUSED_B + 32 : nullptr;
     uint8_t* const b29 = wide ? C.ws_b29.as<uint8_t>() : nullptr;
+    const WideKey wk{P.part_low, P.wide_kind};
     if (wide) {
-        launch_timed(C.timer, "k_acc_wide29", k_acc_wide29<BF>, dim3(P.acc_blocks), dim3(256), P.wide_acc_lds, s, C.ws_entries.as<u32>(), C.ws_off.as<u32>(),
-                     C.ws_toff.as<u32>(), order, (u32)nkeys, (const uint8_t*)tab_pts, C.ws_partial.as<uint8_t>(), b29, P.part_low, C.ws_handed.as<u32>());
+        launch_timed(C.timer, "k_acc_wide29", k_acc_wide29<BF>, dim3(P.acc_blocks), dim3(P.acc_threads), P.wide_acc_lds, s, C.ws_entries.as<u32>(), C.ws_off.as<u32>(),
+                     C.ws_toff.as<u32>(), order, (u32)P.acc_keys, (const uint8_t*)tab_pts, C.ws_partial.as<uint8_t>(), b29, wk, C.ws_handed.as<u32>());
         const unsigned xgrid = P.M / nkeys >= 64 ? 2048u : WIDE_XB;
         hipLaunchKernelGGL((k_acc_wide_rest<BF>), dim3(xgrid), dim3(256), 0, s, C.ws_entries.as<u32>(), C.ws_off.as<u32>(), C.ws_toff.as<u32>(), C.ws_xlist.as<u32>(),
-                           C.ws_handed.as<u32>(), (const uint8_t*)tab_pts, C.ws_partial.as<uint8_t>(), b29, P.part_low);
+                           C.ws_handed.as<u32>(), (const uint8_t*)tab_pts, C.ws_partial.as<uint8_t>(), b29, wk);
     } else
         launch_timed(C.timer, "k_accumulate29", k_accumulate29<BF>, dim3(P.acc_blocks), dim3(256), 0, s, C.ws_entries.as<u32>(), C.ws_off.as<u32>(),
                      C.ws_toff.as<u32>(), roff, order, nkeys, (const uint8_t*)tab_pts, C.ws_partial.as<uint8_t>(), C.ws_handed.as<u32>(), abort_dev, P.acc_prio);
     C.timer.mark("accumulate", s);
     if (wide)
         hipLaunchKernelGGL((k_bucket_sum_wide<BF>), dim3(256), dim3(256), 0, s, C.ws_toff.as<u32>(), C.ws_xlist.as<u32>(), slist,
-                           C.ws_partial.as<uint8_t>(), b29, P.part_low, WIDE_HOT_NT, C.ws_biglist.as<u32>(), (u32)P.bigcap, C.ws_chunks.as<uint8_t>());
+                           C.ws_partial.as<uint8_t>(), b29, wk, WIDE_HOT_NT, C.ws_biglist.as<u32>(), (u32)P.bigcap, C.ws_chunks.as<uint8_t>());
     else
         launch_bucket_sums<BF>(s, P.quad_sum, P.quad_sum ? (P.spread ? SPREAD_MAX_NT : 16u) : (nkeys <= 16384 ? 4u : 16u), P.spread ? (u32*)C.spread_abort : nullptr,
                                C.ws_toff.as<u32>(), nkeys, C.ws_partial.as<uint8_t>(), C.ws_buckets.as<uint8_t>(), C.ws_biglist.as<u32>(), P.bigcap,
@@ -1677,7 +1687,7 @@
     if (wide) {
         hipLaunchKernelGGL((k_wide_a1<BF>), dim3((P.wide_items + 255) / 256), dim3(256), 0, s, b29, P.wg, (u32)ngroups, C.ws_a1.as<uint8_t>());
         C.timer.mark("reduce_a1", s);
-        hipLaunchKernelGGL((k_wide_l2<BF>), dim3((P.wide_runs + 63) / 64), dim3(64), 0, s, C.ws_a1.as<uint8_t>(), P.wg.flog, P.wide_runs, C.ws_l2.as<uint8_t>());
+        hipLaunchKernelGGL((k_wide_l2<BF>), dim3((P.wide_runs + 63) / 64), dim3(64), 0, s, C.ws_a1.as<uint8_t>(), P.wg, P.wide_runs, C.ws_l2.as<uint8_t>());
         hipLaunchKernelGGL((k_wide_a2<BF>), dim3(P.wide_runs / (u32)ngroups / 16u, (unsigned)ngroups), dim3(64), 0, s, C.ws_l2.as<uint8_t>(), C.ws_a1.as<uint8_t>(), b29, P.wg,
                            C.ws_a2.as<uint8_t>());
         hipLaunchKernelGGL((k_marginals_q<BF>), dim3(32, 3, (unsigned)P.tail_groups), dim3(256), 0, s, C.ws_a2.as<uint8_t>(), mg, C.ws_seg.as<uint8_t>());
@@ -1708,7 +1718,7 @@
     static const bool fused_off = env_flag("KH_NO_FUSED_SORT", false), flag_off = env_flag("KH_NO_DONE_FLAG", false), fin_quad = !env_flag("KH_NO_FIN_QUAD", false);
     MsmShape sh;
     sh.n = n; sh.k = k; sh.offset = offset; sh.flags = flags;
-    sh.precomp_c = basis.precomp_c; sh.has_wide = basis.wide_pts != nullptr; sh.wide_c = basis.wide_c; sh.glv = basis.glv;
+    sh.precomp_c = basis.precomp_c; sh.has_wide = basis.wide_pts != nullptr; sh.wide_c = basis.wide_c; sh.wide_kind = basis.wide_kind; sh.glv = basis.glv;
     sh.stride = basis.stride; sh.basis_n = basis.n; sh.batch_stride = basis.batch_stride;
     sh.num_cus = C.num_cus; sh.lds_per_cu = C.lds_per_cu; sh.lds_per_block = C.lds_per_block;
     sh.wide_min_n = msm_wide_min_n(); sh.stage_entries = sort_staging_cell(0).load(); sh.stage_maxpass = sort_staging_cell(1).load();
@@ -1828,12 +1838,12 @@
     return KH_OK;
 }
 
-int msm_precompute(Context& C, int curve, void* tables, const uint8_t* inf, size_t n, int c) {
-    const int W = windows_of(c);
+int msm_precompute(Context& C, int curve, void* tables, const uint8_t* inf, size_t n, int c, int sub) {
+    const int W = windows_of(c) * sub;
     DevBuf& scratch = C.scratch("precompute");
     int rc = scratch.reserve((size_t)(W - 1) * n * 128); if (rc) return rc;
     dim3 grid((unsigned)((n + 255) / 256));
-    KH_CURVE_LAUNCH(curve, k_precompute<F>, grid, dim3(256), 0, C.stream, (uint8_t*)tables, inf, n, c, W, scratch.as<uint8_t>());
+    KH_CURVE_LAUNCH(curve, k_precompute<F>, grid, dim3(256), 0, C.stream, (uint8_t*)tables, inf, n, c, W, sub, scratch.as<uint8_t>());
     KH_HIP(hipStreamSynchronize(C.stream));
     if (scratch.cap > ((size_t)1 << 30)) scratch.release();
     return KH_OK;
diff --git a/proof_systems_amd/csrc/msm.hpp b/proof_systems_amd/csrc/msm.hpp
--- a/proof_systems_amd/csrc/msm.hpp
+++ b/proof_systems_amd/csrc/msm.hpp
@@ -6,7 +6,7 @@
 
 namespace kh {
 
-int msm_precompute(Context& C, int curve, void* tables, const uint8_t* inf, size_t n, int c);
+int msm_precompute(Context& C, int curve, void* tables, const uint8_t* inf, size_t n, int c, int sub = 1);
 int rebase_points(hipStream_t s, int curve, const uint64_t* coef, size_t Q, const void* tables, size_t stride, size_t N, void* B, void* part, void* lists,
                   hipEvent_t after_plan = nullptr);
 int rebase_tables(hipStream_t s, int curve, const void* part, size_t N, const void* extra_affine_host, size_t extra, int c, void* scratch, void* tables, uint32_t* fail,
@@ -19,6 +19,8 @@
 static constexpr int MSM_PRECOMP_C = 16;
 static constexpr int MSM_WIDE_C = 20;
 void msm_set_wide_min_n(size_t n);
+void msm_set_wide_table_limit(size_t bytes);
+size_t msm_wide_table_limit();
 void msm_set_sort_staging(unsigned entries, unsigned max_passes);
 size_t msm_wide_min_n();
 static constexpr size_t MSM_PRECOMP_MIN_N = 1024;
diff --git a/proof_systems_amd/csrc/msm_api.cpp b/proof_systems_amd/csrc/msm_api.cpp
--- a/proof_systems_amd/csrc/msm_api.cpp
+++ b/proof_systems_amd/csrc/msm_api.cpp
@@ -208,6 +208,7 @@
 extern "C" {
 
 int kh_msm_set_wide_min_n(size_t n) { msm_set_wide_min_n(n); return KH_OK; }
+int kh_msm_set_wide_table_limit(size_t bytes) { msm_set_wide_table_limit(bytes); return KH_OK; }
 int kh_msm_set_sort_staging(unsigned entries, unsigned max_passes) {
     if (max_passes > 8) { set_error("kh_msm_set_sort_staging: at most 8 passes (got %u)", max_passes); return KH_E_INVALID; }
     msm_set_sort_staging(entries, max_passes); return KH_OK;
diff --git a/proof_systems_amd/csrc/msm_plan.hpp b/proof_systems_amd/csrc/msm_plan.hpp
--- a/proof_systems_amd/csrc/msm_plan.hpp
+++ b/proof_systems_amd/csrc/msm_plan.hpp
@@ -46,7 +46,7 @@
 };
 struct WideTasks { u32 room, kmin, nkeys; KTab ktab; };
 struct MargGeom { u32 nb; u32 sh[3]; u32 wd[3]; };
-struct WideGeom { u32 nb, lo, hi, rlog, flog; };
+struct WideGeom { u32 nb, lo, hi, rlog, flog, hf; };
 
 #if defined(__HIPCC__)
 #define KH_PLAN_FN __host__ __device__ inline __attribute__((always_inline))
@@ -64,18 +64,67 @@
     return mg;
 }
 inline size_t hot_list_cap(size_t nkeys, size_t max_tasks) { return nkeys + max_tasks / CHUNK + 2; }
+static constexpr u32 WIDE_SHIFT_J = 4, WIDE_SHIFT_LOG = 2, WIDE_SHIFT_MAX = WIDE_SHIFT_J - 1;
+enum WideKind { WIDE_PLAIN = 1, WIDE_SHIFTED = 2 };
+KH_PLAN_FN void wide_shift_digit(u32 d, u32& j, u32& dp) {
+    u32 z = 0;
+    while (z < WIDE_SHIFT_MAX && !((d >> z) & 1u)) z++;
+    j = z; dp = d >> z;
+}
+KH_PLAN_FN u32 wide_unshift_digit(u32 j, u32 dp) { return dp << j; }
+KH_PLAN_FN u32 wide_holes_from(int kind, u32 nb) { return kind == WIDE_SHIFTED ? nb >> WIDE_SHIFT_MAX : 0u; }
+KH_PLAN_FN bool wide_bucket_populated(u32 hf, u32 t) { return hf == 0u || !(t & 1u) || t < hf; }
+inline size_t wide_populated_count(int kind, u32 nb) { return kind == WIDE_SHIFTED ? (size_t)(nb >> 1) + (nb >> (WIDE_SHIFT_MAX + 1)) : (size_t)nb; }
+KH_PLAN_FN u32 wide_key_of_bucket(int kind, u32 low, u32 t) {
+    if (kind != WIDE_SHIFTED) return ((t & 255u) << low) | (t >> 8);
+    return (((t >> 1) & 255u) << low) | ((t >> 9) << 1) | (t & 1u);
+}
+KH_PLAN_FN u32 wide_true_bucket(int kind, u32 key, u32 low) {
+    const u32 nbl = 1u << low, grp = key >> (low + 8), kk = key & ((nbl << 8) - 1u), part = kk >> low, loc = kk & (nbl - 1u);
+    if (kind != WIDE_SHIFTED) return (grp << (low + 8)) | (loc << 8) | part;
+    return (grp << (low + 8)) | ((loc >> 1) << 9) | (part << 1) | (loc & 1u);
+}
+KH_PLAN_FN bool wide_local_populated(u32 hf, u32 loc) { return hf == 0u || !(loc & 1u) || (loc >> 1) < (hf >> 9); }
 KH_PLAN_FN void wide_a1_item(const WideGeom& g, u32 out, u32& t0, u32& tstride) {
     const u32 per = g.nb >> g.rlog;
     if (out < per) { t0 = out << g.rlog; tstride = 1u; return; }
     const u32 cpm = (1u << g.hi) >> g.rlog, v = out - per, b = v / cpm, s = v - b * cpm;
     t0 = ((s << g.rlog) << g.lo) + b; tstride = 1u << g.lo;
 }
+KH_PLAN_FN void wide_a1_span(const WideGeom& g, u32 out, u32& t0, u32& tstride, u32& cnt) {
+    wide_a1_item(g, out, t0, tstride);
+    cnt = 1u << g.rlog;
+    if (g.hf == 0u || t0 < g.hf) return;
+    if (tstride == 1u) { tstride = 2u; cnt >>= 1; }
+    else if (t0 & 1u) cnt = 0u;
+}
+KH_PLAN_FN u32 wide_a1_thread(const WideGeom& g, u32 u) {
+    const u32 per = g.nb >> g.rlog, cpm = (1u << g.hi) >> g.rlog;
+    if (u < per) return u;
+    u32 v = u - per, b, sc;
+    if (g.hf == 0u) { b = v & ((1u << g.lo) - 1u); sc = v >> g.lo; }
+    else { const u32 odd = v >= (per >> 1) ? 1u : 0u; v -= odd * (per >> 1); b = ((v & ((1u << (g.lo - 1)) - 1u)) << 1) | odd; sc = v >> (g.lo - 1); }
+    return per + b * cpm + sc;
+}
+KH_PLAN_FN u32 wide_l2_thread(const WideGeom& g, u32 u, bool& empty) {
+    empty = false;
+    if (g.hf == 0u) return u;
+    const u32 per2 = (g.nb >> g.rlog) >> g.flog, rpm = ((1u << g.hi) >> g.rlog) >> g.flog;
+    const u32 q = u / (2u * per2), w = u - q * 2u * per2;
+    if (w < per2) return u;
+    u32 v = w - per2;
+    const u32 odd = v >= (per2 >> 1) ? 1u : 0u; v -= odd * (per2 >> 1);
+    const u32 half = 1u << (g.lo - 1), b = ((v & (half - 1u)) << 1) | odd, r = v >> (g.lo - 1);
+    empty = odd && ((r << g.flog) << g.rlog) >= (g.hf >> g.lo);
+    return q * 2u * per2 + per2 + b * rpm + r;
+}
 
 struct MsmShape {
     size_t n = 0, k = 0, offset = 0;
     int flags = 0;
     int precomp_c = 0;
     bool has_wide = false; int wide_c = 0;
+    int wide_kind = WIDE_PLAIN;
     bool glv = false;
     size_t stride = 0, basis_n = 0, batch_stride = 0;
     int num_cus = 256;
@@ -108,6 +157,8 @@
     size_t wide_acc_lds = 0;
     u32 stage_now = 0, part2_maxpass = 0; size_t part2_lds = 0;
     u32 acc_blocks = 0, wide_items = 0, wide_runs = 0;
+    int wide_kind = 0; u32 tab_log = 0;
+    size_t acc_keys = 0; u32 acc_threads = 256;
     u32 m = 0, nseg = 0, nblk1 = 0, planes = 0;
     MargGeom mg{};
     size_t tail_groups = 0, nout = 0;
@@ -160,6 +211,8 @@
     const int W = P.W = P.glv ? 2 * ((128 + c - 1) / c) : windows_of(c);
     const u32 nb = P.nb = 1u << (c - 1);
     const int precomp = P.precomp = (wide || sh.precomp_c) ? 1 : 0;
+    P.wide_kind = wide ? (sh.wide_kind == WIDE_SHIFTED ? WIDE_SHIFTED : WIDE_PLAIN) : 0;
+    P.tab_log = P.wide_kind == WIDE_SHIFTED ? WIDE_SHIFT_LOG : 0u;
     int S = (int)(n / 32768); if (S < 1) S = 1; if (S > 16) S = 16;
     { int want = (int)(512 / ((size_t)W * k)); if (want < 1) want = 1; if (S > want) S = want; }
     P.S = S;
@@ -181,18 +234,24 @@
     P.kmin = 8;
     P.ktab = precomp ? task_length_table(nkeys, (u32)sh.num_cus) : KTab{};
     const size_t max_tasks = P.max_tasks = M / 4 + nkeys + 1;
-    if (!(M < ((size_t)1 << 31) && (tab_stride * (size_t)(precomp ? W : 1) + sh.batch_stride * k) < ((size_t)1 << 31))) {
+    if (!(M < ((size_t)1 << 31) && (tab_stride * ((size_t)(precomp ? W : 1) << P.tab_log) + sh.batch_stride * k) < ((size_t)1 << 31))) {
         *why = "MSM too large for 31-bit entry indices";
         return 1;
     }
     P.bigcap = hot_list_cap(nkeys, max_tasks);
     P.slist_off = 2 + 2 * max_tasks;
-    P.acc_blocks = wide ? (u32)(nkeys / 256) : (u32)((max_tasks + 255) / 256);
-    P.wide_acc_lds = (sh.lds_per_cu / (wide_acc_blocks + 1) + 1024) & ~(size_t)1023;
+    P.acc_keys = wide ? ngroups * wide_populated_count(P.wide_kind, nb) : 0;
+    P.acc_threads = 256;
+    u32 acc_per_cu = wide_acc_blocks;
+    if (P.wide_kind == WIDE_SHIFTED && (P.acc_keys + 255) / 256 < 2 * (size_t)sh.num_cus * wide_acc_blocks) { P.acc_threads = 128; acc_per_cu = 2 * wide_acc_blocks; }
+    P.acc_blocks = wide ? (u32)((P.acc_keys + P.acc_threads - 1) / P.acc_threads) : (u32)((max_tasks + 255) / 256);
+    P.wide_acc_lds = (sh.lds_per_cu / (acc_per_cu + 1) + 1024) & ~(size_t)1023;
     if (P.wide_acc_lds > sh.lds_per_block) P.wide_acc_lds = sh.lds_per_block & ~(size_t)1023;
     if (wide) {
         WideGeom& wg = P.wg;
         wg.nb = nb; wg.lo = (u32)c / 2; wg.hi = (u32)(c - 1) - wg.lo; wg.rlog = wide_rlog;
+        wg.hf = wide_holes_from(P.wide_kind, nb);
+        if (wg.hf && ((wg.hf & 511u) || ((wg.hf >> wg.lo) & ((1u << wg.rlog) - 1u)) || (wg.hf >> wg.lo) == 0u)) { *why = "wide window too narrow for the shifted table kind"; return 1; }
         wg.flog = wg.lo > wg.rlog + 5 ? wg.lo - wg.rlog - 4 : 1;
         P.wide_items = 2u * (nb >> wg.rlog) * (u32)ngroups;
         P.wide_runs = 2u * (nb >> (wg.rlog + wg.flog)) * (u32)ngroups;
diff --git a/proof_systems_amd/csrc/srs.cpp b/proof_systems_amd/csrc/srs.cpp
--- a/proof_systems_amd/csrc/srs.cpp
+++ b/proof_systems_amd/csrc/srs.cpp
@@ -10,7 +10,7 @@
     if (basis == KH_BASIS_G) {
         KH_REQUIRE(chunk == 0, "chunk must be 0 for the monomial basis");
         out.pts = srs->g.p; out.inf = nullptr; out.n = srs->n; out.stride = srs->g_stride; out.precomp_c = srs->g_precomp_c;
-        out.wide_pts = srs->g_wide_c ? srs->g_wide.p : nullptr; out.wide_c = srs->g_wide_c;
+        out.wide_pts = srs->g_wide_c ? srs->g_wide.p : nullptr; out.wide_c = srs->g_wide_c; out.wide_kind = srs->g_wide_c ? srs->g_wide_kind : 0;
         return KH_OK;
     }
     std::lock_guard<std::mutex> ml(srs->map_mu);
@@ -42,23 +42,28 @@
     }
 }
 
-static int build_wide_tables(Context& C, kh_srs* s, bool required) {
+static size_t wide_table_bytes(const kh_srs* s, int kind) { return s->g_stride * 64 * (size_t)windows_of(MSM_WIDE_C) * (kind == KH_WIDE_SHIFTED ? WIDE_SHIFT_J : 1u); }
+static int build_wide_tables(Context& C, kh_srs* s, bool required, int kind) {
     if (s->g_wide_c) return KH_OK;
     if (!s->g_precomp_c || (!required && s->n < msm_wide_min_n())) return KH_OK;
-    int rc = s->g_wide.reserve(s->g_stride * 64 * (size_t)windows_of(MSM_WIDE_C));
+    const size_t limit = msm_wide_table_limit();
+    int rc = KH_OK;
+    if (!required && limit && wide_table_bytes(s, kind) > limit) { set_error("the wide table set is above the limit of %zu bytes", limit); rc = KH_E_NOMEM; }
+    if (!rc) rc = s->g_wide.reserve(wide_table_bytes(s, kind));
     if (!rc) {
         hipError_t e = hipMemcpyAsync(s->g_wide.p, s->g.p, s->g_stride * 64, hipMemcpyDeviceToDevice, C.stream);
         if (e != hipSuccess) { set_error("hipMemcpyAsync failed: %s", hipGetErrorString(e)); rc = KH_E_DEVICE; }
     }
-    if (!rc) rc = msm_precompute(C, s->curve, s->g_wide.p, nullptr, s->g_stride, MSM_WIDE_C);
+    if (!rc) rc = msm_precompute(C, s->curve, s->g_wide.p, nullptr, s->g_stride, MSM_WIDE_C, kind == KH_WIDE_SHIFTED ? (int)WIDE_SHIFT_J : 1);
     if (rc) {
         (void)hipStreamSynchronize(C.stream);
         s->g_wide.release(); s->g_wide_c = 0;
         if (required || rc != KH_E_NOMEM) return rc;
         (void)hipGetLastError();
         set_error("");
-        return KH_OK;
-    }
+        return kind == KH_WIDE_SHIFTED ? build_wide_tables(C, s, false, KH_WIDE_PLAIN) : KH_OK;
+    }
+    s->g_wide_kind = kind;
     s->g_wide_c = MSM_WIDE_C;
     return KH_OK;
 }
@@ -84,7 +89,7 @@
     for (size_t i = n; i < s->g_stride; i++)
         KH_HIP(hipMemcpyAsync((char*)s->g.p + i * 64, s->g.p, 64, hipMemcpyDeviceToDevice, C.stream));
     if ((rc = build_tables(C, curve, s->g.p, nullptr, n, s->g_stride, &s->g_precomp_c))) return rc;
-    if ((rc = build_wide_tables(C, s.get(), false))) return rc;
+    if ((rc = build_wide_tables(C, s.get(), false, KH_WIDE_SHIFTED))) return rc;
     KH_HIP(hipStreamSynchronize(C.stream));
     if ((rc = kh_srs_h(curve, s->h))) return rc;
     *out = s.release();
@@ -94,17 +99,24 @@
 extern "C" {
 
 int kh_srs_has_wide_tables(const kh_srs_t* srs) { return srs && srs->g_wide_c ? 1 : 0; }
+int kh_srs_wide_tables_kind(const kh_srs_t* srs) { return srs && srs->g_wide_c ? srs->g_wide_kind : 0; }
 int kh_srs_set_wide_tables(kh_srs_t* srs, int on) {
     KH_ON_DEVICE_OF(srs);
     KH_REQUIRE(srs != nullptr, "null SRS handle");
+    KH_REQUIRE(on == 0 || on == KH_WIDE_PLAIN || on == KH_WIDE_SHIFTED, "kh_srs_set_wide_tables: %d is no table kind (0, KH_WIDE_PLAIN, KH_WIDE_SHIFTED)", on);
     int rc = ensure_init(); if (rc) return rc;
     Context& C = ctx();
     std::lock_guard<std::mutex> lk(C.mu);
     if (on) {
         KH_REQUIRE(srs->g_precomp_c, "kh_srs_set_wide_tables: the handle has no window tables (fewer than %d points)", (int)MSM_PRECOMP_MIN_N);
         std::lock_guard<std::mutex> wl(srs->wide_mu);
-        if (srs->g_wide_c) return KH_OK;
-        if ((rc = build_wide_tables(C, srs, true))) return rc;
+        if (srs->g_wide_c && srs->g_wide_kind == on) return KH_OK;
+        if (srs->g_wide_c) {
+            KH_REQUIRE(srs->jobs->load() == 0, "kh_srs_set_wide_tables: an MSM is in flight (kh_msm_wait first)");
+            srs->g_wide_c = 0;
+            srs->g_wide.release();
+        }
+        if ((rc = build_wide_tables(C, srs, true, on))) return rc;
         const int built = srs->g_wide_c;
         srs->g_wide_c = 0;
         const hipError_t e = hipStreamSynchronize(C.stream);
diff --git a/proof_systems_amd/khip.py b/proof_systems_amd/khip.py
--- a/proof_systems_amd/khip.py
+++ b/proof_systems_amd/khip.py
@@ -32,6 +32,7 @@
 VESTA, PALLAS = _CONSTANTS["KH_CURVE_VESTA"], _CONSTANTS["KH_CURVE_PALLAS"]
 FP, FQ = _CONSTANTS["KH_FIELD_FP"], _CONSTANTS["KH_FIELD_FQ"]
 BASIS_G = _CONSTANTS["KH_BASIS_G"]
+WIDE_PLAIN, WIDE_SHIFTED = _CONSTANTS["KH_WIDE_PLAIN"], _CONSTANTS["KH_WIDE_SHIFTED"]
 PROVE_CHECK = _CONSTANTS["KH_PROVE_CHECK"]
 WITNESS_GATES, WITNESS_WIRES, WITNESS_LOOKUPS = _CONSTANTS["KH_WITNESS_GATES"], _CONSTANTS["KH_WITNESS_WIRES"], _CONSTANTS["KH_WITNESS_LOOKUPS"]
 
@@ -160,6 +161,10 @@
     _check(_lib.kh_msm_set_wide_min_n(n))
 
 
+def set_wide_table_limit(nbytes: int = 0):
+    _check(_lib.kh_msm_set_wide_table_limit(nbytes))
+
+
 POINT_BYTES = _CONSTANTS["KH_POINT_BYTES"]
 POINT_OK, POINT_INFINITY, POINT_BAD_FLAGS, POINT_NOT_CANONICAL, POINT_NOT_ON_CURVE = (_CONSTANTS["KH_POINT_" + _n] for _n in (
     "OK", "INFINITY", "BAD_FLAGS", "NOT_CANONICAL", "NOT_ON_CURVE"))
@@ -272,8 +277,11 @@
     def has_wide_tables(self) -> bool:
         return bool(_lib.kh_srs_has_wide_tables(self._h))
 
-    def set_wide_tables(self, on: bool):
+    def set_wide_tables(self, on):
         _check(_lib.kh_srs_set_wide_tables(self._h, int(on)))
+
+    def wide_tables_kind(self) -> int:
+        return int(_lib.kh_srs_wide_tables_kind(self._h))
 
     def close(self):
         if self._h:
diff --git a/rust/kimchi-hip-sys/src/lib.rs b/rust/kimchi-hip-sys/src/lib.rs
--- a/rust/kimchi-hip-sys/src/lib.rs
+++ b/rust/kimchi-hip-sys/src/lib.rs
@@ -208,6 +208,8 @@
 pub const KH_FIELD_FP: c_int = 0;
 pub const KH_FIELD_FQ: c_int = 1;
 pub const KH_BASIS_G: c_int = -1;
+pub const KH_WIDE_PLAIN: c_int = 1;
+pub const KH_WIDE_SHIFTED: c_int = 2;
 pub const KH_REF_NONE: c_int = -2;
 pub const KH_REF_ARENA: c_int = -1;
 pub const KH_STEP_NO_FLAG: c_int = 255;
@@ -322,6 +324,8 @@
     pub fn kh_msm_set_sort_staging(entries: c_uint, max_passes: c_uint) -> c_int;
     pub fn kh_srs_set_wide_tables(srs: *mut kh_srs_t, on: c_int) -> c_int;
     pub fn kh_srs_has_wide_tables(srs: *const kh_srs_t) -> c_int;
+    pub fn kh_srs_wide_tables_kind(srs: *const kh_srs_t) -> c_int;
+    pub fn kh_msm_set_wide_table_limit(bytes: usize) -> c_int;
     pub fn kh_srs_free(srs: *mut kh_srs_t);
     pub fn kh_srs_size(srs: *const kh_srs_t) -> usize;
     pub fn kh_srs_curve(srs: *const kh_srs_t) -> c_int;
```
